# zhipeng-wei/Image-to-Video-I2V-attack

Hardware: AMD Instinct MI355X
Metric: adversarial frames/sec (10-step I2V, ResNet-50 layer3, 32x224^2 clips) (higher is better)
Workload: dtype f32

## Files before the change

### __graft_entry__.py

```python
import os
import subprocess
import sys

ROOT = os.path.dirname(os.path.abspath(__file__))
PKG_ROOT = os.path.join(ROOT, "image-to-video-i2v-attack_amd")
CSRC = os.path.join(PKG_ROOT, "csrc")
LIB = os.path.join(PKG_ROOT, "i2v_amd", "libi2v_hip.so")
for p in (PKG_ROOT, ROOT):
    if p not in sys.path:
        sys.path.insert(0, p)


def _stale(target, sources):
    return not os.path.exists(target) or any(os.path.getmtime(s) > os.path.getmtime(target) for s in sources)


ENGINE_UNITS = ["i2v_engine.cpp", "i2v_pack.cpp", "i2v_plan.cpp", "i2v_tune.cpp", "i2v_run.cpp", "i2v_loop_api.cpp"]
UNITS = ["i2v_kernels.hip", "i2v_conv_cfg0.hip", "i2v_conv_cfg1.hip", "i2v_conv_cfg2.hip", "i2v_conv_cfg3.hip", "i2v_conv_cfg4.hip",
         "i2v_conv_cfg5.hip", "i2v_conv_stems.hip", "i2v_fastblock.hip", "i2v_gconv.hip", "i2v_dwconv.hip", "i2v_se.hip", "i2v_loader.hip", "i2v_vit.hip", "i2v_vit.cpp", "i2v_swin.hip", "i2v_swin.cpp",
         "i2v_convnext.hip", "i2v_convnext.cpp", "i2v_mixer.hip", "i2v_mixer.cpp",
         ] + ENGINE_UNITS
HEADERS = ["i2v_kernels.h", "i2v_params.h", "i2v_be.h", "i2v_conv_tile.h", "i2v_conv_launch.h", "i2v_vit_kernels.h", "i2v_swin_kernels.h", "i2v_xf.h",
           "i2v_net.h", "i2v_se_host.h", "i2v_convnext_host.h", "i2v_xf_host.h", "i2v_hip_stub.h",
           "i2v_mixer_host.h", "i2v_gelu.h"]
FLAGS = ["--offload-arch=gfx950", "-O3", "-ffp-contract=off", "-std=c++20", "-fPIC", "-DI2V_SEPARATE_UNITS",
         "-DI2V_HAVE_GCONV", "-DI2V_HAVE_DWCONV",
         "-DI2V_HAVE_SE",
         "-DI2V_HAVE_CONVNEXT",
         "-DI2V_HAVE_MIXER"]


def build_lib(experimental: bool = False) -> str:
    from concurrent.futures import ThreadPoolExecutor
    hipcc = os.environ.get("HIPCC", "/opt/rocm/bin/hipcc")
    lib = LIB.replace(".so", "_exp.so") if experimental else LIB
    objdir = os.path.join(CSRC, "build", "exp" if experimental else "default")
    os.makedirs(objdir, exist_ok=True)
    units = UNITS + (["i2v_conv_exp.hip"] if experimental else [])
    hdrs = [os.path.join(CSRC, f) for f in HEADERS] + [os.path.join(ROOT, "include", h) for h in ("i2v_hip.h", "i2v_loader.h", "i2v_vit.h", "i2v_swin.h", "i2v_convnext.h", "i2v_mixer.h")]
    defs = ["-DI2V_EXPERIMENTAL"] if experimental else []
    if not _stale(lib, [os.path.join(CSRC, u) for u in units] + hdrs):
        return lib
    jobs = []
    for u in units:
        src, obj = os.path.join(CSRC, u), os.path.join(objdir, u + ".o")
        if _stale(obj, [src] + hdrs):
            jobs.append([hipcc] + FLAGS + defs + ["-c", "-x", "hip", src, "-o", obj])

    def run(cmd):
        print(" ".join(cmd), flush=True)
        subprocess.run(cmd, check=True)
    if jobs:
        with ThreadPoolExecutor(max_workers=min(len(jobs), max(1, (os.cpu_count() or 2)))) as ex:
            list(ex.map(run, jobs))
    objs = [os.path.join(objdir, u + ".o") for u in units]
    if jobs or _stale(lib, objs):
        run([hipcc, "--offload-arch=gfx950", "-shared", "-fPIC", "-o", lib] + objs)
    return lib


def build() -> None:
    build_lib(experimental=False)
    deps = [os.path.join(CSRC, f) for f in ENGINE_UNITS + ["i2v_net.h", "i2v_kernels.h", "i2v_params.h", "i2v_se_host.h", "i2v_convnext_host.h", "i2v_convnext.cpp", "i2v_mixer_host.h", "i2v_mixer.cpp", "i2v_gelu.h", "i2v_xf.h", "i2v_xf_host.h", "i2v_hip_stub.h",
                                                               "i2v_vit_kernels.h", "i2v_swin_kernels.h"]] + [os.path.join(ROOT, "include", "i2v_hip.h")]
    hs = os.path.join(ROOT, "tests", "hostsim")
    if _stale(os.path.join(hs, "libi2v_hostsim.so"), deps + [os.path.join(hs, "hostsim_backend.cpp")]):
        subprocess.run([os.path.join(hs, "build.sh")], check=True)
    import ctypes
    import i2v_amd
    from i2v_amd import lib
    cd = ctypes.CDLL(LIB) if not _has_gpu() else lib.load()
    missing = [n for n in lib.EXPORTS + lib.LOADER_EXPORTS + lib.VIT_EXPORTS + lib.SWIN_EXPORTS + lib.CONVNEXT_EXPORTS + lib.MIXER_EXPORTS if not hasattr(cd, n)]
    if missing:
        raise RuntimeError(f"libi2v_hip.so lacks symbols: {missing}")


def _has_gpu() -> bool:
    try:
        import torch
        return torch.cuda.is_available()
    except Exception:
        return False


def smoke() -> None:
    import numpy as np
    import torch
    build()
    from i2v_amd import attacks, graphs, weights
    from oracle import restate
    gen = torch.Generator().manual_seed(1234)
    u8 = torch.randint(0, 256, (1, 3, 4, 64, 64), generator=gen, dtype=torch.uint8)
    mean = torch.tensor(restate.MEAN).view(1, 3, 1, 1, 1)
    std = torch.tensor(restate.STD).view(1, 3, 1, 1, 1)
    vid = (u8.float() / 255 - mean) / std
    atk = attacks.ImageGuidedFMDirection_Adam(["resnet"], depth=3, step_size=0.005, steps=3,
                                              graph_builder=graphs.build_tiny, weight_seed=0)
    adv = atk(vid, torch.zeros(1, dtype=torch.long), ["smoke"])
    torch.cuda.synchronize()
    g = graphs.build_tiny("resnet", (64, 64))
    net = restate.OracleNet(g, weights.synthetic_state_dict(g, 0), [g.hooks[3]])
    ref = restate.run_attack([net], vid, steps=3, step_size=0.005)
    np.testing.assert_allclose(atk.last_costs, ref["costs"], rtol=2e-4)
    diff = (adv.cpu() - ref["adv"]).abs()
    assert float(diff.mean()) < 5e-3, float(diff.mean())
    print("smoke ok: costs", atk.last_costs, "mean|adv-oracle|", float(diff.mean()))


if __name__ == "__main__":
    if "--experimental" in sys.argv[1:]:
        print(build_lib(experimental=True))
    else:
        build()
        if _has_gpu():
            smoke()
```

### image-to-video-i2v-attack_amd/csrc/i2v_be.h

```cpp
#pragma once
#include <hip/hip_runtime.h>
#include <math.h>
#include <stdint.h>
#include <stdio.h>
#include <stdlib.h>
#include <string.h>

#include <type_traits>
#include <utility>

#include "i2v_kernels.h"

typedef float f32x16 __attribute__((ext_vector_type(16)));
typedef float f32x4 __attribute__((ext_vector_type(4)));

extern thread_local char g_be_err[256];
extern thread_local bool g_be_has_err;
int hip_fail(hipError_t e, const char* what);
#define HIPCHK(x) do { hipError_t e_ = (x); if (e_ != hipSuccess) return hip_fail(e_, #x); } while (0)
#define LAUNCH_CHECK(name) do { hipError_t e_ = hipGetLastError(); if (e_ != hipSuccess) return hip_fail(e_, name); } while (0)
extern long long g_stat_conv, g_stat_pws, g_stat_bf3, g_stat_igh, g_stat_sth, g_stat_fastblock, g_stat_vfma, g_stat_igv, g_stat_gconv, g_stat_dwconv, g_stat_se, g_stat_cndw, g_stat_mixtok;

__device__ __forceinline__ unsigned fastdiv(unsigned n, unsigned m, unsigned s) {
    return (unsigned)(((unsigned long long)n * m) >> s);
}
static inline void fastdiv_magic(unsigned d, uint32_t* m, uint32_t* s) {
    unsigned l = 0; while ((1ull << l) < d) ++l;
    *s = 31 + l;
    *m = (uint32_t)(((1ull << (31 + l)) / d) + 1);
}
typedef int i2v_v4i __attribute__((ext_vector_type(4)));
__device__ __forceinline__ I2VKEntry load_kentry(const I2VKEntry* tab, int k) {
#if defined(__HIP_DEVICE_COMPILE__)
    const i2v_v4i v = ((const __attribute__((address_space(4))) i2v_v4i*)tab)[k];
    return I2VKEntry{v.x, v.y, v.z, v.w};
#else
    return tab[k];
#endif
}

static inline void conv_magics(I2VConvParams& p) {
    fastdiv_magic((unsigned)(p.Hg * p.Wg), &p.dv_hw_m, &p.dv_hw_s);
    fastdiv_magic((unsigned)p.Wg, &p.dv_w_m, &p.dv_w_s);
    fastdiv_magic((unsigned)(p.Tg > 0 ? p.Tg : 1), &p.dv_t_m, &p.dv_t_s);
    fastdiv_magic((unsigned)(p.Wo > 0 ? p.Wo : 1), &p.dv_wo_m, &p.dv_wo_s);
}

static inline bool conv_wants_prefetch(const I2VConvParams& p) {
    return p.vec_epilogue && !p.gate_scale && !p.pre_scale && p.add0_stride == 1 && (p.add0 || p.add1 || p.mask || p.gate) && p.Kpad <= 256 && (p.pointwise || p.tap_uniform) && p.Cd > 32;
}

static inline int conv_tail_px_tiles(const I2VConvParams& p) {
    if (p.quad || p.pre_scale || p.temporal || !(p.pointwise || p.tap_uniform) || p.Cd % 16 != 0 || p.blk > 1) return 0;
    const int64_t P = (int64_t)p.N * p.Hg * p.Wg;
    const int64_t n_px = (P + 63) / 64; const int n_cd = (p.Cd + 63) / 64;
    const int64_t tiles = n_px * n_cd;
    if (tiles < 2 * 256) return 0;
    const int r = (int)(tiles % 256);
    if (r == 0 || r > 104) return 0;
    return r / n_cd;
}

static inline bool conv_halo_ok(const I2VConvParams& p) {
    return p.halo == 9 && p.tap_uniform && !p.temporal && !p.pre_scale && !p.quad && p.blk <= 1 && p.sh == 1 && p.sw == 1 && p.Hs == p.Hg &&
           p.Ws == p.Wg && (p.Ws == 14 || p.Ws == 28 || p.Ws == 56) && p.Kpad == p.K && (p.Kpad / I2V_KC) % 9 == 0;
}

static inline bool conv_dc_ok(const I2VConvParams& p) {
    return (p.pointwise || p.tap_uniform) && !p.temporal && !p.pre_scale && !p.quad && p.Cd > 32 && (p.Kpad / I2V_KC) % 2 == 0 && p.Kpad >= 4 * I2V_KC;
}

static inline bool conv_bf3_ok(const I2VConvParams& p) {
#ifdef I2V_EXPERIMENTAL
    return p.bf3 && p.wp3 && (p.pointwise || p.tap_uniform) && (!p.temporal || p.tap_uniform) && !p.pre_scale && !p.quad && p.blk <= 1 && p.blkt <= 1 && p.Cd > 32;
#else
    (void)p; return false;
#endif
}

int launch_conv_cfg0(const I2VConvParams& p, hipStream_t s);
int launch_conv_cfg1(const I2VConvParams& p, hipStream_t s);
int launch_conv_cfg2(const I2VConvParams& p, hipStream_t s);
int launch_conv_cfg3(const I2VConvParams& p, hipStream_t s);
int launch_conv_cfg4(const I2VConvParams& p, hipStream_t s);
int launch_conv_cfg5(const I2VConvParams& p, hipStream_t s);
bool conv_ighalo_ok(const I2VConvParams& p);
int launch_conv_ighalo(const I2VConvParams& p, hipStream_t s);
bool conv_igvfma_ok(const I2VConvParams& p);
int launch_conv_igvfma(const I2VConvParams& p, hipStream_t s);
bool conv_stemhalo_ok(const I2VConvParams& p);
int launch_conv_stemhalo(const I2VConvParams& p, hipStream_t s);
bool conv_vfma_ok(const I2VConvParams& p);
int launch_conv_vfma(const I2VConvParams& p, hipStream_t s);
#ifdef I2V_EXPERIMENTAL
#ifndef I2V_BF3_VARIANT
#define I2V_BF3_VARIANT 1
#endif
#endif
#ifdef I2V_EXPERIMENTAL
bool conv_stem64_ok(const I2VConvParams& p);
int launch_conv_stem64(const I2VConvParams& p, hipStream_t s);
int conv_pws_grid(const I2VConvParams& p);
int launch_conv_pws(const I2VConvParams& p, hipStream_t s);
int launch_conv_bf3(const I2VConvParams& p, hipStream_t s);
// ... 2 lines not shown
```

### image-to-video-i2v-attack_amd/csrc/i2v_conv_tile.h

```cpp
#pragma once
#include "i2v_be.h"

#ifndef I2V_PROBE_T
struct I2VNoProbe {
    __device__ __forceinline__ void entry() {}
    __device__ __forceinline__ void loop_begin() {}
    __device__ __forceinline__ void loop_end(int ) {}
    __device__ __forceinline__ void exit(int ) {}
};
#define I2V_PROBE_T I2VNoProbe
#endif

#ifndef I2V_PRIO_LEVELS
#define I2V_PRIO_LEVELS 3
#endif
#ifndef I2V_DEEP
#define I2V_DEEP 1
#endif
#ifndef I2V_DEEP_STAGES
#define I2V_DEEP_STAGES 3
#endif
#ifndef I2V_BF3_STAGES
#define I2V_BF3_STAGES 2
#endif
// ... 42 lines not shown
    const bool nt_store = true;
#else
    const bool nt_store = p.cfg > 0 && ((p.cfg - 1) & 128);
#endif
    constexpr int C4 = BP / 4, RSTEP = 1024 / BP, NQ = WD * FR / RSTEP;
    const int c4 = t % C4, rbase = t / C4;
    const int64_t pp = px0 + (int64_t)c4 * 4;
    const bool pok = pp < P;
    const int64_t n = pok ? fastdiv((unsigned)pp, p.dv_hw_m, p.dv_hw_s) : 0;
    const int64_t poff = pp - n * HWg;
    #pragma unroll
    for (int q = 0; q < NQ; ++q) {
        const int row = rbase + q * RSTEP;
        const int cd = cd0 + (row / FR) * (BD / WD) + i * FR + (row % FR);
        const bool valid = pok && cd < p.Cd;
        float4 v = make_float4(0.f, 0.f, 0.f, 0.f);
        if (valid) {
        v = *reinterpret_cast<const float4*>(&Cs[row][c4 * 4]);
        const int64_t o = (int64_t)cd * HoWo + poff;
        if (p.gate_scale) {
            const float4 m = *reinterpret_cast<const float4*>(p.mask + n * p.mask_nstride + o);
            const float gs = p.gate_scale[cd], gt = p.gate_shift[cd];
            if (!(fmaf(m.x, gs, gt) > 0.f)) v.x = 0.f;
            if (!(fmaf(m.y, gs, gt) > 0.f)) v.y = 0.f;
            if (!(fmaf(m.z, gs, gt) > 0.f)) v.z = 0.f;
            if (!(fmaf(m.w, gs, gt) > 0.f)) v.w = 0.f;
        }
        if (p.shift) { const float sh = p.shift[cd]; v.x += sh; v.y += sh; v.z += sh; v.w += sh; }
        if (PREF) {
            v.x += pre0[q].x; v.y += pre0[q].y; v.z += pre0[q].z; v.w += pre0[q].w;
        } else {
            if (p.add0 && p.add0_stride == 1) {
                const float4 a = *reinterpret_cast<const float4*>(p.add0 + n * p.add0_nstride + o);
                v.x += a.x; v.y += a.y; v.z += a.z; v.w += a.w;
            } else if (p.add0) {
                const int oh = (int)fastdiv((unsigned)poff, p.dv_wo_m, p.dv_wo_s), ow = (int)(poff - (int64_t)oh * p.Wo);
                if (!(oh & 1) && (oh >> 1) < p.add0_H) {
                    const float2 a = *reinterpret_cast<const float2*>(
                        p.add0 + n * p.add0_nstride + (int64_t)cd * p.add0_H * p.add0_W + (oh >> 1) * p.add0_W + (ow >> 1));
                    v.x += a.x; v.z += a.y;
                }
            }
        }
        if (p.add1) {
            const float4 a = *reinterpret_cast<const float4*>(p.add1 + n * p.add1_nstride + o);
            v.x += a.x; v.y += a.y; v.z += a.z; v.w += a.w;
        }
        if (p.relu) { v.x = fmaxf(v.x, 0.f); v.y = fmaxf(v.y, 0.f); v.z = fmaxf(v.z, 0.f); v.w = fmaxf(v.w, 0.f); }
        if (p.gate) {
            const unsigned w = PREF ? pregw[q] : p.gate[(int64_t)cd * p.gate_stride + ((p.gate_pix0 + pp) >> 5)];
            const unsigned g = w >> ((unsigned)(p.gate_pix0 + pp) & 31u);
            if (!(g & 1u)) v.x = 0.f;
            if (!(g & 2u)) v.y = 0.f;
            if (!(g & 4u)) v.z = 0.f;
            if (!(g & 8u)) v.w = 0.f;
        } else if (p.mask && !p.gate_scale) {
            const float4 m = *reinterpret_cast<const float4*>(p.mask + n * p.mask_nstride + o);
            if (!(m.x > 0.f)) v.x = 0.f;
            if (!(m.y > 0.f)) v.y = 0.f;
            if (!(m.z > 0.f)) v.z = 0.f;
            if (!(m.w > 0.f)) v.w = 0.f;
        }
        if constexpr (!FUSE) {
            if (nt_store) { typedef float nt4 __attribute__((ext_vector_type(4))); const nt4 w4 = {v.x, v.y, v.z, v.w};
                            __builtin_nontemporal_store(w4, reinterpret_cast<nt4*>(p.dst + n * p.dst_nstride + o)); }
            else *reinterpret_cast<float4*>(p.dst + n * p.dst_nstride + o) = v;
        }
        }
        if constexpr (FUSE)
            *reinterpret_cast<float4*>(mid + (cd - cd0) * BP + c4 * 4) = v;
        if (p.gate_out) {
            unsigned nib = valid ? ((v.x > 0.f ? 1u : 0u) | (v.y > 0.f ? 2u : 0u) | (v.z > 0.f ? 4u : 0u) | (v.w > 0.f ? 8u : 0u)) : 0u;
            nib <<= 4 * (lane & 7);
            nib |= (unsigned)__builtin_amdgcn_update_dpp(0, (int)nib, 0xB1, 0xF, 0xF, true);
            nib |= (unsigned)__builtin_amdgcn_update_dpp(0, (int)nib, 0x4E, 0xF, 0xF, true);
            nib |= (unsigned)__builtin_amdgcn_update_dpp(0, (int)nib, 0x141, 0xF, 0xF, true);
            if (valid && (lane & 7) == 0)
                p.gate_out[(int64_t)cd * p.gate_out_stride + ((p.gate_out_pix0 + pp) >> 5)] = nib;
        }
    }
}

#define I2V_FROW(r) (MF16 ? 4 * lk + (r) : ((r) & 3) + 8 * ((r) >> 2) + 4 * lk)
template <int BD, int BP, int WD, int WP, bool PREF, bool MF16, bool FUSE, typename ACC, typename PT>
__device__ __forceinline__ void conv_vec_epilogue(const PT& p, ACC (&acc)[BD / WD / (MF16 ? 16 : 32)][BP / WP / (MF16 ? 16 : 32)], const int cd0,
                                                  const int64_t px0, float* const smem, const float4* const pre0, const unsigned* const pregw,
                                                  float* const mid) {
    constexpr int FR = MF16 ? 16 : 32, NR = MF16 ? 4 : 16, TD = BD / WD / FR, TP = BP / WP / FR;
    const int t = threadIdx.x, lane = t & 63, wave = t >> 6;
    const int wd = wave / WP, wpx = wave % WP;
    const int l31 = MF16 ? (lane & 15) : (lane & 31), lk = MF16 ? (lane >> 4) : (lane >> 5);
    float (*Cs)[BP] = reinterpret_cast<float (*)[BP]>(smem);
#pragma unroll
    for (int i = 0; i < TD; ++i) {
        __syncthreads();
#pragma unroll
        for (int j = 0; j < TP; ++j)
#pragma unroll
            for (int r = 0; r < NR; ++r)
                Cs[wd * FR + I2V_FROW(r)][wpx * (BP / WP) + j * FR + l31] = acc[i][j][r];
        __syncthreads();
        conv_vec_rows<BD, BP, WD, PREF, MF16, FUSE>(p, i, cd0, px0, Cs, t, pre0, pregw, mid);
    }
}
#undef I2V_FROW

template <int BD, int BP, int WD, int WP, int MODE, bool PREF, bool PRE = false, bool VID = false, bool MF16 = false, int HWM = 0, int CPB = 1, int FUSE = 0, int BF3 = 0>
__device__ __forceinline__ void conv_tile(const I2VConvParams& p, const int n_cd_tiles, const int bid, const int nwg, const int64_t px_base,
                                          float* const smem, I2V_PROBE_T& probe, const int probe_slot, const int prio_arg = I2V_PRIO_LEVELS,
                                          float* const mid = nullptr) {
#if defined(__HIP_DEVICE_COMPILE__)
    constexpr int KC = I2V_KC;
    constexpr int FR = MF16 ? 16 : 32;
    constexpr int NR = MF16 ? 4 : 16;
    constexpr int TD = BD / WD / FR, TP = BP / WP / FR;
    static_assert(!(MF16 && (PRE || PREF)), "no pre-activation / prefetch variants of the 16x16 tile");
    constexpr bool DEEP = conv_deep(MODE, PREF) || (BF3 == 1 && I2V_BF3_STAGES > 2) || BF3 == 3;
    constexpr int NST = BF3 == 3 ? 3 : BF3 == 1 ? I2V_BF3_STAGES : DEEP ? I2V_DEEP_STAGES : 2, AHEAD = NST - 1;
    constexpr bool HALO = MODE == 5;
    constexpr int HS = HALO ? BP + 2 * HWM + 2 : 1, HQ = (HS + 63) / 64;
    static_assert(!HALO || (HWM > 0 && BD == 64 && BP == 64 && !PREF && !PRE && !VID && !MF16), "halo staging: the plain 64x64 image tile only");
    static_assert(CPB == 1 || (!HALO && !DEEP && !PREF && !PRE && MODE != 4 && MODE != 0), "several chunks per barrier: the plain pointwise / tap-uniform loops only");
    constexpr int KB = CPB * KC;
    static_assert(!BF3 || (!MF16 && !PRE && !PREF && !HALO && (MODE == 1 || MODE == 2) && FUSE == 0 && BD % 32 == 0), "split-bf16 K loop: the plain pointwise / tap-uniform tiles");
    constexpr int AF = BF3 == 2 ? 0 : BF3 ? CPB * (((BD / 32) * 3 + 3) / 4 * 4) * 256 : KB * BD;
    float (*As)[KB][BD] = reinterpret_cast<float (*)[KB][BD]>(smem);
    float* const As3 = smem;
    float (*Bs)[KB][BP] = reinterpret_cast<float (*)[KB][BP]>(smem + NST * AF);

    const int t = threadIdx.x, lane = t & 63, wave = t >> 6;
    const int wd = wave / WP, wpx = wave % WP;

    const int q8 = nwg >> 3, r8 = nwg & 7, xcd = bid & 7;
    const int lid = (xcd < r8 ? xcd * (q8 + 1) : r8 * (q8 + 1) + (xcd - r8) * q8) + (bid >> 3);
    const int cd_tile = lid % n_cd_tiles;
    const int64_t px0 = px_base + (int64_t)(lid / n_cd_tiles) * BP;
    const int cd0 = cd_tile * BD;

    const int HWg = p.Hg * p.Wg;
    const int64_t P = (int64_t)p.N * HWg;

    constexpr bool PW = MODE == 1;
    constexpr bool QUAD = MODE == 4;
    typedef __attribute__((address_space(3))) void* lds_ptr_t;
    constexpr unsigned OOB = 0x80000000u;
    const int wv = __builtin_amdgcn_readfirstlane(wave);
    const __amdgpu_buffer_rsrc_t rs_w = BF3 ? __builtin_amdgcn_make_buffer_rsrc((void*)p.wp3, 0, (p.Kpad / KC) * (p.Cdpad / 32) * 3072, 0x00020000)
                                            : __builtin_amdgcn_make_buffer_rsrc((void*)p.wp, 0, p.Kpad * p.Cdpad * 4, 0x00020000);
    constexpr unsigned XB = QUAD ? 64u : 0u;
    const __amdgpu_buffer_rsrc_t rs_x = __builtin_amdgcn_make_buffer_rsrc((void*)((const char*)p.src - XB), 0, p.src_span_bytes + 2 * XB, 0x00020000);
    constexpr int NA = BF3 == 2 ? 0 : BF3 ? (BD / 32) * 3 : KC * BD / 256, NAQ = (NA + 3) / 4;
    constexpr int BPER = (PW || QUAD) ? 256 : 64;
    constexpr int NB = HALO ? 0 : KC * BP / BPER, NBQ = (NB + 3) / 4;
    const int bcol = PW ? (lane * 4) % BP : (BP >= 64 ? ((wave * 64) % BP) + lane : lane % BP);
    const int64_t ppix = px0 + bcol;
    const bool pvalid = ppix < P;
    const int64_t pn = pvalid ? fastdiv((unsigned)ppix, p.dv_hw_m, p.dv_hw_s) : 0;
    const int prem = (int)(ppix - pn * HWg);
    const int HWs = p.Hs * p.Ws;
    int h0 = 0, w0 = 0, t0 = 0;
    int64_t pns = pn;
    if (VID) {
        const int64_t clip = fastdiv((unsigned)pn, p.dv_t_m, p.dv_t_s);
        t0 = (int)(pn - clip * p.Tg) * p.st;
        pns = clip * p.Ts + t0;
    }
    const int nstr = (int)p.src_nstride;
    unsigned xoff;
    if (PW) xoff = (unsigned)((pns * p.src_nstride + prem) * 4);
    else {
        const int gi = (int)fastdiv((unsigned)prem, p.dv_w_m, p.dv_w_s), gj = prem - gi * p.Wg;
        h0 = gi * p.sh; w0 = gj * p.sw;
        xoff = (unsigned)((pns * p.src_nstride + (int64_t)h0 * p.Ws + w0) * 4) + XB;
    }
    if (!pvalid) xoff = OOB;
    unsigned aoff[NAQ ? NAQ : 1];
#pragma unroll
    for (int q = 0; q < NAQ; ++q) {
        const int f = (wave + 4 * q) * 256 + lane * 4;
        aoff[q] = BF3 ? (unsigned)(((cd0 / 32) * 3 + wave + 4 * q) * 1024 + lane * 16) : (unsigned)(((f / BD) * p.Cdpad + f % BD + cd0) * 4);
    }
    unsigned boff[PW ? NBQ : 1];
    if (PW) {
#pragma unroll
        for (int q = 0; q < NBQ; ++q) boff[q] = pvalid ? xoff + (unsigned)((((wave + 4 * q) * 256 + lane * 4) / BP) * HWs * 4) : OOB;
    }

#define I2V_ISSUE_PIECE(j_, k0_, buf_, vb_) I2V_ISSUE_PIECE_SUB(j_, k0_, buf_, vb_, 0)
#define I2V_ISSUE_PIECE_SUB(j_, k0_, buf_, vb_, sub_)                                                     \
    {                                                                                                     \
        constexpr int jj = (j_);                                                                          \
        const int k0 = (k0_);                                                                             \
        if constexpr (jj < NAQ) {                                                                         \
            const int ins = wv + 4 * jj;                                                                  \
            if constexpr (BF3) {    \
                __builtin_amdgcn_raw_ptr_buffer_load_lds(rs_w, (lds_ptr_t)(As3 + (buf_) * AF + (sub_) * (AF / CPB) + ins * 256), 16, ins < NA ? aoff[jj] : OOB, \
                                                         (k0 / KC) * (p.Cdpad / 32) * 3072, 0, 0);       \
            } else if (NA % 4 == 0 || ins < NA) {                                                         \
                if constexpr (false)                                                                      \
                    ;                                                                                     \
                else                                                                                      \
                    __builtin_amdgcn_raw_ptr_buffer_load_lds(rs_w, (lds_ptr_t)(&As[buf_][(sub_) * KC][0] + ins * 256), 16, aoff[jj],  \
                                                             k0 * p.Cdpad * 4, 0, 0);                     \
            }                                                                                             \
        } else {                                                                                          \
            constexpr int q = jj - NAQ;                                                                   \
            const int ins = wv + 4 * q;                                                                   \
            float* const bbuf = &Bs[buf_][(sub_) * KC][0];                                                \
            if (NB % 4 == 0 || ins < NB) {                                                                \
                if constexpr (PW) {                                                                       \
                    unsigned v = boff[q];                                                                 \
                    if (k0 + KC > p.K)             \
                        v = (k0 + ((wave + 4 * q) * 256 + lane * 4) / BP < p.K) ? v : OOB;                \
                    __builtin_amdgcn_raw_ptr_buffer_load_lds(rs_x, (lds_ptr_t)(bbuf + ins * 256), 16, v,         \
                                                             k0 * HWs * 4, 0, 0);                         \
                } else if constexpr (QUAD) {                                                              \
                     \
                    const I2VKEntry e = load_kentry(p.ktab, k0 + 4 * ((ins * 64) / BP));                  \
                    const int hs = h0 + e.dh, dtk = VID ? (e.valid >> 1) : 0;                             \
                    const bool ok = pvalid && (unsigned)hs < (unsigned)p.Hs && (!VID || (unsigned)(t0 + dtk) < (unsigned)p.Ts); \
                    const unsigned v = ok ? xoff + (unsigned)((e.chan_off + dtk * nstr + e.dh * p.Ws + e.dw) * 4) : OOB; \
                    __builtin_amdgcn_raw_ptr_buffer_load_lds(rs_x, (lds_ptr_t)(bbuf + ins * 256), 16, v, 0, 0, 0); \
                } else if constexpr (MODE == 2) {                                                         \
                    __builtin_amdgcn_raw_ptr_buffer_load_lds(rs_x, (lds_ptr_t)(bbuf + ins * 64), 4, vb_,         \
                                                             ((ins * 64) / BP) * HWs * 4, 0, 0);          \
                } else {                                                                                  \
                    const I2VKEntry e = load_kentry(p.ktab, k0 + (ins * 64) / BP);                        \
                    const int hs = h0 + e.dh, ws = w0 + e.dw, dtk = VID ? (e.valid >> 1) : 0;             \
                    const bool ok = pvalid && (e.valid & 1) && (unsigned)hs < (unsigned)p.Hs &&           \
                                    (unsigned)ws < (unsigned)p.Ws && (!VID || (unsigned)(t0 + dtk) < (unsigned)p.Ts); \
                    const unsigned v = ok ? xoff + (unsigned)((e.chan_off + dtk * nstr + e.dh * p.Ws + e.dw) * 4) : OOB; \
                    __builtin_amdgcn_raw_ptr_buffer_load_lds(rs_x, (lds_ptr_t)(bbuf + ins * 64), 4, v, 0, 0, 0); \
                }                                                                                         \
            }                                                                                             \
        }                                                                                                 \
    }
#define I2V_CHUNK_VB(e_)                                                                                  \
    ([&]() -> unsigned {                                                                                  \
        const int hs = h0 + (e_).dh, ws = w0 + (e_).dw, dtk = VID ? ((e_).valid >> 1) : 0;                \
        const bool ok = pvalid && (unsigned)hs < (unsigned)p.Hs && (unsigned)ws < (unsigned)p.Ws &&       \
                        (!VID || (unsigned)(t0 + dtk) < (unsigned)p.Ts);                                  \
        return ok ? xoff + (unsigned)(((e_).chan_off + dtk * nstr + (e_).dh * p.Ws + (e_).dw) * 4) : OOB; \
    }())

    constexpr int E_C4 = BP / 4, E_RSTEP = 1024 / BP, E_NQ = WD * FR / E_RSTEP;
    static_assert(!PREF || TD == 1, "PREF needs a single epilogue pass");
    float4 pre0[PREF ? E_NQ : 1];
    unsigned pregw[PREF ? E_NQ : 1];
    if (PREF) {
        const int e_c4 = t % E_C4, e_rbase = t / E_C4;
        const int64_t e_pp = px0 + (int64_t)e_c4 * 4;
        const bool e_ok = e_pp < P;
        const int64_t e_n = e_ok ? fastdiv((unsigned)e_pp, p.dv_hw_m, p.dv_hw_s) : 0;
        const int64_t e_poff = e_pp - e_n * HWg;
        const int e_HoWo = p.Ho * p.Wo;
#pragma unroll
        for (int q = 0; q < E_NQ; ++q) {
            const int row = e_rbase + q * E_RSTEP;
            const int cd = cd0 + (row >> 5) * (BD / WD) + (row & 31);
            const bool ok = e_ok && cd < p.Cd;
            const int64_t o = (int64_t)cd * e_HoWo + e_poff;
            pre0[q] = (ok && p.add0) ? *reinterpret_cast<const float4*>(p.add0 + e_n * p.add0_nstride + o) : make_float4(0.f, 0.f, 0.f, 0.f);
            pregw[q] = (ok && p.gate) ? p.gate[(int64_t)cd * p.gate_stride + ((p.gate_pix0 + e_pp) >> 5)] : 0xffffffffu;
        }
    }

    probe.loop_begin();
    typedef short bf8 __attribute__((ext_vector_type(8)));
    typedef float f4 __attribute__((ext_vector_type(4)));
    constexpr int TD_ = BD / WD / (MF16 ? 16 : 32);
    bf8 wcur[BF3 == 2 ? CPB : 1][BF3 == 2 ? TD_ : 1][3];
    const char* const w3lane = BF3 ? (const char*)p.wp3 + (size_t)lane * 16 + (size_t)(cd0 / 32 + (wave / WP) * TD_) * 3072 : nullptr;
    const size_t w3chunk = BF3 ? (size_t)(p.Cdpad / 32) * 3072 : 0;
    auto load_w3 = [&](const int chunk, const int i, const int pl) {
        return __builtin_bit_cast(bf8, *reinterpret_cast<const f4*>(w3lane + (size_t)chunk * w3chunk + (i * 3 + pl) * 1024));
    };
    if constexpr (BF3 == 2) {
#pragma unroll
        for (int sb = 0; sb < CPB; ++sb)
#pragma unroll
            for (int i = 0; i < TD_; ++i)
#pragma unroll
                for (int pl = 0; pl < 3; ++pl) wcur[sb][i][pl] = load_w3(sb, i, pl);
    }
    (void)wcur; (void)w3lane; (void)w3chunk;
    constexpr int TP_ = BP / WP / (MF16 ? 16 : 32);
    bf8 xcur[BF3 == 3 ? TP_ : 1][3];
    (void)xcur;
    auto bf3_split2 = [](const float lo, const float hi, unsigned& p1, unsigned& p2, unsigned& p3) {
        typedef __bf16 bf2 __attribute__((ext_vector_type(2)));
        typedef float f2 __attribute__((ext_vector_type(2)));
        const unsigned a = __builtin_bit_cast(unsigned, __builtin_convertvector((f2){lo, hi}, bf2));
        const float rl = lo - __builtin_bit_cast(float, a << 16), rh = hi - __builtin_bit_cast(float, a & 0xffff0000u);
        const unsigned b = __builtin_bit_cast(unsigned, __builtin_convertvector((f2){rl, rh}, bf2));
        const float sl = rl - __builtin_bit_cast(float, b << 16), sh = rh - __builtin_bit_cast(float, b & 0xffff0000u);
        const unsigned c = __builtin_bit_cast(unsigned, __builtin_convertvector((f2){sl, sh}, bf2));
        p1 = a; p2 = b; p3 = c;
    };
    auto bf3_split_frag = [&](const float (&x)[8], bf8 (&out)[3]) {
        typedef unsigned u4 __attribute__((ext_vector_type(4)));
        unsigned q1[4], q2[4], q3[4];
#pragma unroll
        for (int e = 0; e < 4; ++e) bf3_split2(x[2 * e], x[2 * e + 1], q1[e], q2[e], q3[e]);
        out[0] = __builtin_bit_cast(bf8, (u4){q1[0], q1[1], q1[2], q1[3]});
        out[1] = __builtin_bit_cast(bf8, (u4){q2[0], q2[1], q2[2], q2[3]});
        out[2] = __builtin_bit_cast(bf8, (u4){q3[0], q3[1], q3[2], q3[3]});
    };
    (void)bf3_split_frag;
    typedef typename std::conditional<MF16, f32x4, f32x16>::type acc_t;
    acc_t acc[TD][TP];
#pragma unroll
    for (int a = 0; a < TD; ++a)
#pragma unroll
        for (int b = 0; b < TP; ++b)
#pragma unroll
            for (int r = 0; r < NR; ++r) acc[a][b][r] = 0.f;

    const int nchunks = p.Kpad / KC;
    const int l31 = MF16 ? (lane & 15) : (lane & 31), lk = MF16 ? (lane >> 4) : (lane >> 5);
#define I2V_FROW(r) (MF16 ? 4 * lk + (r) : ((r) & 3) + 8 * ((r) >> 2) + 4 * lk)
    constexpr int NL = NAQ + NBQ;
    constexpr int KR = MF16 ? 4 : 2;
    constexpr int KS = KC / KR;
    constexpr int PPS = (NL + KS - 1) / KS;
    I2VKEntry e_next[CPB];
#pragma unroll
    for (int h = 0; h < CPB; ++h) e_next[h] = I2VKEntry{0, 0, 0, 0};
    const int nsuper = nchunks / CPB;
    bool qok[QUAD ? TP : 1][2][MF16 ? 1 : 2];
    if constexpr (QUAD) {
#pragma unroll
        for (int j = 0; j < TP; ++j) {
            const int64_t fp = px0 + wpx * (BP / WP) + j * FR + l31;
            const unsigned fr = fp < P ? (unsigned)fp - fastdiv((unsigned)fp, p.dv_hw_m, p.dv_hw_s) * (unsigned)HWg : 0u;
            const int fj = (int)(fr - fastdiv(fr, p.dv_w_m, p.dv_w_s) * (unsigned)p.Wg);
#pragma unroll
            for (int qi = 0; qi < 2; ++qi)
#pragma unroll
                for (int hf = 0; hf < (MF16 ? 1 : 2); ++hf) {
                    const int el = MF16 ? lk : 2 * hf + lk;
                    qok[j][qi][hf] = 4 * qi + el < p.quad_kw && (unsigned)(fj * p.sw + p.quad_dw0 + 4 * qi + el) < (unsigned)p.Ws;
                }
        }
    }
    if constexpr (HALO) {
        constexpr int NT = 9, HPW = 4 * HQ, PPC = (HPW + NT - 1) / NT;
        float* const Hb = smem + NST * KC * BD;
        const int W_ = HWM;
        int tsh[NT], tdh[NT], tdw[NT];
#pragma unroll
        for (int t = 0; t < NT; ++t) {
            const I2VKEntry e = load_kentry(p.ktab, t * KC);
            tdh[t] = e.dh; tdw[t] = e.dw; tsh[t] = e.dh * W_ + e.dw + W_ + 1;
        }
        const int chan0 = load_kentry(p.ktab, 0).chan_off;
        const int ngroups = nchunks / NT;
        const int gstride = ngroups > 1 ? load_kentry(p.ktab, NT * KC).chan_off - chan0 : 0;
        const int64_t fp = px0 + wpx * (BP / WP) + l31;
        const bool fpv = fp < P;
        const unsigned fr = fpv ? (unsigned)fp - fastdiv((unsigned)fp, p.dv_hw_m, p.dv_hw_s) * (unsigned)HWg : 0u;
        const int fh = (int)fastdiv(fr, p.dv_w_m, p.dv_w_s), fw = (int)fr - fh * p.Wg;
        unsigned tmask = 0;
#pragma unroll
        for (int t = 0; t < NT; ++t)
            tmask |= (fpv && (unsigned)(fh + tdh[t]) < (unsigned)p.Hs && (unsigned)(fw + tdw[t]) < (unsigned)p.Ws) ? (1u << t) : 0u;
        const int lbase = lk * HS + wpx * (BP / WP) + l31;
        unsigned hoff[HQ];
#pragma unroll
        for (int q = 0; q < HQ; ++q) {
            const int64_t vp = px0 - (W_ + 1) + 64 * q + lane;
            const bool ok = vp >= 0 && vp < P;
            const int64_t vn = ok ? fastdiv((unsigned)vp, p.dv_hw_m, p.dv_hw_s) : 0;
            hoff[q] = ok ? (unsigned)((vn * p.src_nstride + (vp - vn * HWg)) * 4) : OOB;
        }
        auto halo_piece = [&]<int IDX>(std::integral_constant<int, IDX>, const int gb, const int chan_off) {
            constexpr int chl = IDX / HQ, q = IDX % HQ;
            float* const dst = Hb + ((gb * KC + wv * 4 + chl) * HS + 64 * q);
            const int so = (chan_off + (wv * 4 + chl) * HWs) * 4;
            if constexpr (chl == 3 && q == HQ - 1) {
                if (lane < HS - 64 * q) __builtin_amdgcn_raw_ptr_buffer_load_lds(rs_x, (lds_ptr_t)dst, 4, hoff[q], so, 0, 0);
            } else
                __builtin_amdgcn_raw_ptr_buffer_load_lds(rs_x, (lds_ptr_t)dst, 4, hoff[q], so, 0, 0);
        };
        if (ngroups > 0) {
            [&]<int... I>(std::integer_sequence<int, I...>) { ((halo_piece(std::integral_constant<int, I>{}, 0, chan0)), ...); }
            (std::make_integer_sequence<int, HPW>{});
            I2V_ISSUE_PIECE(0, 0, 0, OOB);
        }
        int gbuf = 0;
        for (int g = 0; g < ngroups; ++g) {
            const bool more_g = g + 1 < ngroups;
            const int chan_next = chan0 + (g + 1) * gstride;
            [&]<int... T>(std::integer_sequence<int, T...>) {
                (([&] {
                    constexpr int t = T;
                    const int abuf = (g + t) & 1;
                    asm volatile("s_waitcnt vmcnt(0)" ::: "memory");
                    asm volatile("s_waitcnt lgkmcnt(0)" ::: "memory");
                    __builtin_amdgcn_s_barrier();
                    const int hidx = lbase + gbuf * KC * HS + tsh[t];
                    const bool ok = (tmask >> t) & 1u;
                    float fa[2], fb[2];
                    auto rd = [&](const int s_, const int set) {
// ... 192 lines not shown
#pragma unroll
                    for (int i = 0; i < TD; ++i)
#pragma unroll
                        for (int pl = 0; pl < 3; ++pl) wcur[sb][i][pl] = wnxt[sb][i][pl];
            }
            return;
        }
        float fa[2][TD], fb[2][TP];
        auto read_frags = [&](const int s, const int set) {
#pragma unroll
            for (int i = 0; i < TD; ++i) fa[set][i] = As[buf][KR * s + lk][wd * (BD / WD) + i * FR + l31];
            if constexpr (QUAD) {
                const float* const bq = &Bs[buf][0][0];
#pragma unroll
                for (int j = 0; j < TP; ++j) {
                    const int px = wpx * (BP / WP) + j * FR + l31;
                    const int qd = MF16 ? s : (s >> 1), el = MF16 ? lk : 2 * (s & 1) + lk;
                    const float v = bq[(qd * BP + px) * 4 + el];
                    const bool m = ((qd & 1) && p.quad == 2) ? qok[j][1][MF16 ? 0 : (s & 1)] : qok[j][0][MF16 ? 0 : (s & 1)];
                    fb[set][j] = m ? v : 0.f;
                }
            } else {
#pragma unroll
                for (int j = 0; j < TP; ++j) fb[set][j] = Bs[buf][KR * s + lk][wpx * (BP / WP) + j * FR + l31];
            }
        };
        read_frags(0, 0);
        [&]<int... S>(std::integer_sequence<int, S...>) {
            (([&] {
                constexpr int s = S, set = S & 1;
                if constexpr (s + 1 < CPB * KS) read_frags(s + 1, set ^ 1);
                __builtin_amdgcn_sched_barrier(0);
                if constexpr (PRE) {
                    typedef const __attribute__((address_space(4))) float* cfp;
                    const int kr = c * KB + 2 * s;
                    const float sc = lk ? ((cfp)p.pre_scale)[kr + 1] : ((cfp)p.pre_scale)[kr];
                    const float sh = lk ? ((cfp)p.pre_shift)[kr + 1] : ((cfp)p.pre_shift)[kr];
#pragma unroll
                    for (int j = 0; j < TP; ++j) fb[set][j] = fmaxf(fmaf(fb[set][j], sc, sh), 0.f);
                }
#pragma unroll
                for (int i = 0; i < TD; ++i)
#pragma unroll
                    for (int j = 0; j < TP; ++j) {
                        if constexpr (MF16) acc[i][j] = __builtin_amdgcn_mfma_f32_16x16x4f32(fa[set][i], fb[set][j], acc[i][j], 0, 0, 0);
                        else acc[i][j] = __builtin_amdgcn_mfma_f32_32x32x2f32(fa[set][i], fb[set][j], acc[i][j], 0, 0, 0);
                    }
                if constexpr (MORE) {
                    [&]<int... Q>(std::integer_sequence<int, Q...>) {
                        (([&] {
                            constexpr int jp = s * PPS + Q;
                            if constexpr (jp < CPB * NL) {
                                constexpr int sub = jp / NL;
                                I2V_ISSUE_PIECE_SUB(jp % NL, ((c + AHEAD) * CPB + sub) * KC, DEEP ? (buf + AHEAD) % NST : (buf ^ 1), vb[sub], sub);
                            }
                        }()), ...);
                    }(std::make_integer_sequence<int, PPS>{});
                }
            }()), ...);
        }(std::make_integer_sequence<int, CPB * KS>{});
    };
    if constexpr (BF3 == 3) {
        asm volatile("s_waitcnt vmcnt(0)" ::: "memory");
        __builtin_amdgcn_s_barrier();
        const int l31_ = lane & 31, lk_ = lane >> 5;
#pragma unroll
        for (int j = 0; j < TP_; ++j) {
            float x[8];
#pragma unroll
            for (int e = 0; e < 8; ++e) x[e] = Bs[0][8 * lk_ + e][(wave % WP) * (BP / WP) + j * 32 + l31_];
            bf3_split_frag(x, xcur[j]);
        }
    }
    if constexpr (!HALO) {
        int c = 0, buf = 0;
        for (; c + AHEAD < nsuper; ++c) { chunk_body(c, buf, std::true_type{}); buf = buf + 1 == NST ? 0 : buf + 1; }
        for (; c < nsuper; ++c) { chunk_body(c, buf, std::false_type{}); buf = buf + 1 == NST ? 0 : buf + 1; }
    }
#undef I2V_ISSUE_PIECE
#undef I2V_ISSUE_PIECE_SUB
#undef I2V_CHUNK_VB
    if (prio_hi > 0) __builtin_amdgcn_s_setprio(0);
    probe.loop_end(probe_slot);

    const int HoWo = p.Ho * p.Wo;
    if (p.vec_epilogue) {
        conv_vec_epilogue<BD, BP, WD, WP, PREF, MF16, FUSE != 0>(p, acc, cd0, px0, smem, pre0, pregw, mid);
        return;
    }
    if (p.blk > 1 || (VID && p.blkt > 1)) {
        const int bb = p.blk * p.blk, Creal = p.Cd / ((VID ? p.blkt : 1) * bb);
#pragma unroll
        for (int j = 0; j < TP; ++j) {
            const int64_t pp = px0 + wpx * (BP / WP) + j * FR + l31;
            if (pp >= P) continue;
            const int64_t ng = fastdiv((unsigned)pp, p.dv_hw_m, p.dv_hw_s);
            const int rem = (int)(pp - ng * HWg);
            const int gi = (int)fastdiv((unsigned)rem, p.dv_w_m, p.dv_w_s), gj = rem - gi * p.Wg;
            const int64_t clip = VID ? fastdiv((unsigned)ng, p.dv_t_m, p.dv_t_s) : ng;
            const int otb = VID ? (int)(ng - clip * p.Tg) * p.ost + p.ot0 : 0;
#pragma unroll
            for (int i = 0; i < TD; ++i)
#pragma unroll
                for (int r = 0; r < NR; ++r) {
                    const int cd = cd0 + wd * (BD / WD) + i * FR + I2V_FROW(r);
                    if (cd >= p.Cd) continue;
                    const int cls3 = cd / Creal, c = cd - cls3 * Creal;
                    const int ct = VID ? cls3 / bb : 0, cls = cls3 - ct * bb;
                    const int oh = gi * p.osh + cls / p.blk + p.oh0, ow = gj * p.osw + cls % p.blk + p.ow0;
                    if (oh >= p.Ho || ow >= p.Wo || (VID && otb + ct * p.oct >= p.To)) continue;
                    const int64_t n = VID ? clip * p.To + otb + ct * p.oct : ng;
                    const int64_t o = (int64_t)c * HoWo + oh * p.Wo + ow;
                    float v = acc[i][j][r];
                    if (p.shift) v += p.shift[c];
                    if (p.add1) v += p.add1[n * p.add1_nstride + o];
                    if (p.relu) v = fmaxf(v, 0.f);
                    if (p.mask && !(p.mask[n * p.mask_nstride + o] > 0.f)) v = 0.f;
                    p.dst[n * p.dst_nstride + o] = v;
                }
        }
        return;
    }
#pragma unroll
    for (int j = 0; j < TP; ++j) {
        const int64_t pp = px0 + wpx * (BP / WP) + j * FR + l31;
        const bool pin = pp < P;
        const int64_t ng = pin ? fastdiv((unsigned)pp, p.dv_hw_m, p.dv_hw_s) : 0;
        const int rem = (int)(pin ? pp - ng * HWg : 0);
        const int gi = (int)fastdiv((unsigned)rem, p.dv_w_m, p.dv_w_s), gj = rem - gi * p.Wg;
        const int oh = gi * p.osh + p.oh0, ow = gj * p.osw + p.ow0;
        bool ok = pin && oh < p.Ho && ow < p.Wo;
        int64_t n = ng;
        if (VID) {
            const int64_t clip = fastdiv((unsigned)ng, p.dv_t_m, p.dv_t_s);
            const int ot = (int)(ng - clip * p.Tg) * p.ost + p.ot0;
            if (ot >= p.To) ok = false;
            n = clip * p.To + ot;
        }
        const int opix = oh * p.Wo + ow;
        float* dstn = p.dst + n * p.dst_nstride + opix;
        const float* a0 = nullptr; int a0_plane = HoWo;
        if (p.add0 && ok) {
            if (p.add0_stride == 1) a0 = p.add0 + n * p.add0_nstride + opix;
            else {
                const int s = p.add0_stride, qh = oh / s, qw = ow / s;
                if (qh * s == oh && qw * s == ow && qh < p.add0_H && qw < p.add0_W) {
                    a0 = p.add0 + n * p.add0_nstride + qh * p.add0_W + qw;
                    a0_plane = p.add0_H * p.add0_W;
                }
            }
        }
        const float* a1 = p.add1 ? p.add1 + n * p.add1_nstride + opix : nullptr;
        const float* mk = p.mask ? p.mask + n * p.mask_nstride + opix : nullptr;
        const int64_t gidx = (int64_t)p.gate_pix0 + n * HoWo + opix;
#pragma unroll
        for (int i = 0; i < TD; ++i) {
#pragma unroll
            for (int r = 0; r < NR; ++r) {
                const int cd = cd0 + wd * (BD / WD) + i * FR + I2V_FROW(r);
                const bool okc = ok && cd < p.Cd;
                float v = 0.f;
                if (okc) {
                    v = acc[i][j][r];
                    if (p.gate_scale && !(fmaf(mk[(int64_t)cd * HoWo], p.gate_scale[cd], p.gate_shift[cd]) > 0.f)) v = 0.f;
                    if (p.shift) v += p.shift[cd];
                    if (a0) v += a0[(int64_t)cd * a0_plane];
                    if (a1) v += a1[(int64_t)cd * HoWo];
// ... 72 lines not shown
```

### image-to-video-i2v-attack_amd/csrc/i2v_engine.cpp

```cpp
#include "i2v_net.h"

#include <math.h>
#include <stdarg.h>
#include <stdio.h>
#include <stdlib.h>
#include <string.h>

using namespace eng;

#define I2V_MAX_NETS 4096
thread_local std::string eng::g_err;

int eng::fail(const char* fmt, ...) {
    char buf[512];
    va_list ap;
    va_start(ap, fmt);
    vsnprintf(buf, sizeof buf, fmt, ap);
    va_end(ap);
    g_err = buf;
    return 1;
}

int i2v_api_fail(const char* msg) { return fail("%s", msg); }

// ... 331 lines not shown
            if (pack_gconv(n, nd)) return 1;
            continue;
        }
        if (nd.groups > 1 || nd.dw) expand_grouped(nd);
        if (pack_fwd(n, nd)) return 1;
        if (nd.preact()) {
            std::vector<float> ps(nd.fwd.Kpad > nd.fwd.Cdpad ? nd.fwd.Kpad : nd.fwd.Cdpad, 0.f), pt(ps.size(), 0.f);
            for (int c = 0; c < nd.cd.cin; ++c) { ps[c] = nd.pre_scale[c]; pt[c] = nd.pre_shift[c]; }
            if (upload(n, ps, &nd.pre_scale_d) || upload(n, pt, &nd.pre_shift_d)) return 1;
        }
        if (nd.cd.src == n.input) { if (pack_img(n, nd)) return 1; }
        else if (pack_bwd(n, nd)) return 1;
        if (nd.groups > 1 || nd.dw) std::vector<float>().swap(nd.w);
    }
    size_t off = 64;
    for (const Node& nd : n.nodes) if (nd.type == 0 && nd.cd.src == n.input && nd.fwd.quad) n.stage_input = true;
    if (n.stage_input) {
        const Buffer& ib = n.bufs[n.tens[n.input].buf];
        n.in_stage_off = off; off = align_up(off + N * ib.C * ib.H * ib.W, 64) + 64;
    }
    for (Buffer& b : n.bufs) {
        if (b.is_input) continue;
        size_t sz = N / Tin * b.T * b.C * b.H * b.W;
        b.act_off = off; off = align_up(off + sz, 64);
        b.grad_off = off; off = align_up(off + sz, 64);
    }
    const char* gates_env = getenv("I2V_GATES");
    const bool use_gates = !(gates_env && gates_env[0] == '0');
    for (const Node& nd : n.nodes)
        if (use_gates && nd.type == 0 && nd.cd.relu && !nd.fwd.tpair) n.bufs[n.tens[nd.cd.dst].buf].gated = true;
    for (const Node& nd : n.nodes)
        if (use_gates && nd.type == 4 && nd.sd.relu) n.bufs[n.tens[nd.sd.dst].buf].gated = true;
    for (Buffer& b : n.bufs) {
        if (!b.gated) continue;
        const size_t pix = N / Tin * b.T * b.H * b.W;
        if (pix + 64 >= (1ull << 31)) return fail("gate rows of more than 2^31 bits are not supported");
        b.gate_words = (int)((pix + 31) / 32 + 2);
        b.gate_off = off; off = align_up(off + (size_t)b.C * b.gate_words, 64);
    }
    for (Node& nd : n.nodes)
        if (nd.type == 1) {
            const Buffer& db = n.bufs[n.tens[nd.pd.dst].buf];
            nd.idx_off = off; off = align_up(off + (N / Tin * db.T * n.tens[nd.pd.dst].C * db.H * db.W + 3) / 4, 64);
        }
    for (Node& nd : n.nodes)
        if (nd.type == 3) {
            const Buffer& tb = n.bufs[n.tens[nd.ad.theta].buf]; const Buffer& pb = n.bufs[n.tens[nd.ad.phi].buf];
            nd.p_off = off; off = align_up(off + N / Tin * ((size_t)tb.T * tb.H * tb.W) * ((size_t)pb.T * pb.H * pb.W), 64);
        }
    for (Node& nd : n.nodes)
        if (nd.type == 4) {
            const size_t C = (size_t)nd.sd.C, rd = (size_t)nd.sd.rd;
            nd.se_off = off; nd.se_floats = 4 * align_up(N * C, 64) + align_up(N * rd, 64);
            off += nd.se_floats;
        }
    std::string err;
    size_t end = 0;
    if (!plan_pass(n, true, off, N, &end, &err)) return fail("plan: %s", err.c_str());
    n.arena_floats = end + 64;
    n.arena = (float*)be_malloc(n.arena_floats * sizeof(float));
    if (!n.arena) return fail("arena allocation of %zu bytes failed", n.arena_floats * sizeof(float));
    CHECK_BE(be_memset0(n.arena, n.arena_floats * sizeof(float), nullptr));
    if (!plan_pass(n, false, off, N, &end, &err)) return fail("plan: %s", err.c_str());
    mark_fusable(n);
    if (autotune(n)) return 1;
    mark_overlap(n);
    CHECK_BE(be_stream_sync(nullptr));
    n.planned = true;
    return 0;
}

extern "C" int i2v_net_fusion_info(i2v_handle h, int net, int32_t out[4]) {
    Net* n = get_net(h, net); if (!n) return 1;
    if (!n->planned || !out) return fail("i2v_net_fusion_info: net not planned");
    out[0] = out[1] = out[2] = out[3] = 0;
    int k = 0;
    for (const std::vector<Launch>* L : {&n->fwd, &n->bwd}) {
        for (const Launch& l : *L) { out[k] += l.fuse_ok ? 1 : 0; out[2 + k] += (l.fuse_ok && l.fuse_b[0]) ? 1 : 0; }
        ++k;
    }
    return 0;
}

extern "C" size_t i2v_net_workspace_bytes(i2v_handle h, int net) {
    Net* n = get_net(h, net); if (!n) return 0;
    return n->arena_floats * sizeof(float) + n->weight_bytes;
}

#ifndef I2V_SEPARATE_UNITS
#include "i2v_pack.cpp"
#include "i2v_plan.cpp"
#include "i2v_tune.cpp"
#include "i2v_run.cpp"
#include "i2v_loop_api.cpp"
#define fail xf_fail
#include "i2v_convnext.cpp"
#include "i2v_mixer.cpp"
#undef fail
#endif
```

### image-to-video-i2v-attack_amd/csrc/i2v_kernels.h

```cpp
#pragma once
#include <initializer_list>
#include "i2v_params.h"

typedef void* i2v_stream_t;

const char* be_name();
long long be_stat(const char* name);
int  be_set_device(int device);
void* be_malloc(size_t bytes);
void be_free(void* p);
int  be_h2d(void* dst, const void* src, size_t bytes);
int  be_d2d_2d(void* dst, size_t dpitch, const void* src, size_t spitch, size_t width, size_t rows,
               i2v_stream_t s);
int  be_memset0(void* p, size_t bytes, i2v_stream_t s);
const char* be_error();
int  i2v_api_fail(const char* msg);
void* be_event_create();
void be_event_destroy(void* ev);
int  be_event_record(void* ev, i2v_stream_t s);
int  be_event_elapsed_ms(void* start, void* stop, float* ms);
int  be_stream_sync(i2v_stream_t s);
i2v_stream_t be_stream_create();
void be_stream_destroy(i2v_stream_t s);
int  be_stream_wait_event(i2v_stream_t s, void* ev);
int  be_device_sync();

int k_conv(const I2VConvParams& p, i2v_stream_t s);
int k_conv_fusable(const I2VConvParams& a, const I2VConvParams& b);
inline bool i2v_conv_pair_fusable(const I2VConvParams& a, const I2VConvParams& b) {
    if (a.pointwise || !a.tap_uniform || a.temporal || a.quad || a.pre_scale || a.gate_scale || a.blk > 1 || a.blkt > 1) return false;
    for (const I2VConvParams* q : {&a, &b})
        if (!(q->Tg == q->Ts && q->Ts == q->To && q->st == 1 && q->ost == 1 && q->ot0 == 0 && q->blkt <= 1)) return false;
    if (a.sh != 1 || a.sw != 1 || a.Hs != a.Hg || a.Ws != a.Wg || a.Hg != a.Ho || a.Wg != a.Wo || a.osh != 1 || a.osw != 1 || a.oh0 || a.ow0) return false;
    if ((a.Cd != 64 && a.Cd != 128) || a.Kpad != a.K || a.add0_stride > 1) return false;
    if (!b.pointwise || b.temporal || b.quad || b.pre_scale || b.gate_scale || b.blk > 1 || b.blkt > 1 || b.add0_stride > 1) return false;
    if (b.K != a.Cd || b.Kpad != b.K || b.Cs != a.Cd || b.src != a.dst || b.src_nstride != a.dst_nstride) return false;
    if (b.Hs != a.Ho || b.Ws != a.Wo || b.Hg != a.Hg || b.Wg != a.Wg || b.Ho != a.Ho || b.Wo != a.Wo || b.sh != 1 || b.sw != 1 || b.osh != 1 || b.osw != 1 ||
        b.oh0 || b.ow0 || b.Cd < 64 || b.Tg != a.Tg) return false;
    return true;
}
int k_conv_fused(const I2VConvParams& a, const I2VConvParams& b, int halo, i2v_stream_t s);
int k_conv_candidates(const I2VConvParams& p, int* out);
inline int i2v_fastblock_rows(const I2VConvParams& a, const I2VConvParams& b, const I2VConvParams* c, const I2VConvParams* d) {
    auto plain = [](const I2VConvParams& q) {
        return !q.pre_scale && !q.gate_scale && q.blk <= 1 && q.blkt <= 1 && q.sh == 1 && q.sw == 1 && q.osh == 1 && q.osw == 1 && q.oh0 == 0 &&
               q.ow0 == 0 && q.Hs == q.Hg && q.Hg == q.Ho && q.Ws == q.Wg && q.Wg == q.Wo && q.Tg == q.Ts && q.Ts == q.To && q.st == 1 && q.ost == 1 && q.ot0 == 0 &&
               !q.add1 && !q.mask && q.Kpad % 8 == 0 && q.Kpad <= 512 && q.gate_pix0 == 0 && q.gate_out_pix0 == 0;
    };
    if (!plain(a) || !plain(b) || a.quad || a.add0 || b.add0) return 0;
    const int CM = a.Cd;
    if ((CM != 4 && CM != 8) || b.Cd != CM || b.Cs != CM || b.src != a.dst || b.src_nstride != a.dst_nstride) return 0;
    if (b.Hg != a.Hg || b.Wg != a.Wg || b.Tg != a.Tg || b.N != a.N) return 0;
    const int H = a.Hg, W = a.Wg;
    if ((H * W) % 32 != 0 || (int64_t)a.N * a.src_nstride * 4 >= (1ll << 31)) return 0;
    if (c) {
        if (!plain(*c) || c->quad || !a.relu || !b.relu || a.gate || b.gate || c->gate || !c->relu || !a.shift || !b.shift || !c->shift || !a.gate_out || !b.gate_out || !c->gate_out) return 0;
        if (c->src != b.dst || c->src_nstride != b.dst_nstride || c->Cs != CM || c->K != CM || c->Cd != 4 * CM || c->Hg != H || c->Wg != W || c->Tg != a.Tg || c->N != a.N) return 0;
        if (!c->add0 || c->add0_stride != 1) return 0;
        if (d) {
            if (!plain(*d) || d->quad || d->relu || d->add0 || d->gate || d->gate_out || !d->shift || d->src != a.src || d->src_nstride != a.src_nstride || d->Cs != a.Cs ||
                d->K != a.Cs || d->K != CM || d->Cd != c->Cd || d->Hg != H || d->Wg != W || d->Tg != a.Tg || d->N != a.N || c->add0 != d->dst || c->add0_nstride != d->dst_nstride) return 0;
        }
    } else {
        if (d || a.relu || b.relu || a.gate_out || b.gate_out || a.shift || b.shift || !a.gate || !b.gate || a.K != a.Cs || a.K > 64) return 0;
    }
    int g = W, r32 = 32; while (r32) { const int t = g % r32; g = r32; r32 = t; }
    const int Rq = 32 / g;
    if (H % Rq != 0) return 0;
    int R = Rq;
    while (R * W < 192 && R * 2 <= H && H % (R * 2) == 0) R *= 2;
    if ((size_t)CM * (R + 2) * (W + 2) * 4 > 60 * 1024) return 0;
    return R;
}
int k_fastblock(const I2VConvParams& a, const I2VConvParams& b, const I2VConvParams* c, const I2VConvParams* d, i2v_stream_t s);
int k_gconv_plan(I2VGConvParams* p);
int k_gconv(const I2VGConvParams& p, i2v_stream_t s);
int k_dwconv_plan(I2VDwConvParams* p);
int k_dwconv(const I2VDwConvParams& p, i2v_stream_t s);
int k_se_plan(I2VSeParams* p);
int k_se_squeeze(const I2VSeParams& p, i2v_stream_t s);
int k_se_excite(const I2VSeParams& p, i2v_stream_t s);
int k_se_scale(const I2VSeParams& p, i2v_stream_t s);
int k_convnext_dw_plan(I2VCnDwParams* p);
int k_convnext_dw(const I2VCnDwParams& p, i2v_stream_t s);
int k_mixer_tokens_plan(I2VMixTokParams* p);
int k_mixer_tokens(const I2VMixTokParams& p, i2v_stream_t s);
int k_pool_fwd(const I2VPoolParams& p, i2v_stream_t s);
int k_pool_bwd(const I2VPoolParams& p, i2v_stream_t s);
int k_pool3d_fwd(const I2VPoolParams& p, i2v_stream_t s);
int k_pool3d_bwd(const I2VPoolParams& p, i2v_stream_t s);
int k_avgpool_fwd(const I2VPoolParams& p, i2v_stream_t s);
int k_avgpool_bwd(const I2VPoolParams& p, i2v_stream_t s);
int k_addmask(const I2VAddMaskParams& p, i2v_stream_t s);
int k_cos(const I2VCosParams& p, i2v_stream_t s);
int k_std_reduce(const I2VStdParams& p, i2v_stream_t s);
int k_std_grad(const I2VStdParams& p, i2v_stream_t s);
int k_ilaf_reduce(const I2VIlafParams& p, i2v_stream_t s);
int k_ilaf_grad(const I2VIlafParams& p, i2v_stream_t s);
int k_head_ce(const I2VHeadParams& p, i2v_stream_t s);
int k_clip_from_u8(const uint8_t* frames, float* video, int b, int t, int h, int w, i2v_stream_t s);
int k_clip_resize_crop(const uint8_t* frames, float* video, const int32_t* xtab, const int32_t* ytab, int b, int t, int H, int W,
                       int cy, int cx, int oh, int ow, i2v_stream_t s);
int k_frames_from_video(const float* video, float* x, float* u, int b, int f, int h, int w, i2v_stream_t s);
int k_compose(const float* u, const float* delta, float* x, int b, int f, int h, int w, float eps,
              int video_layout, i2v_stream_t s);
int k_adam(float* delta, float* m, float* v, const float* gx, const float* u, int64_t n, int hw,
           float eps, float step_size, float bc2_sqrt, float w1, float beta2, float w2, float adam_eps,
           i2v_stream_t s);
int k_sign_bim(float* adv, const float* u, const float* grad, int64_t n, int64_t chan_stride,
               float step, float eps, i2v_stream_t s);
int k_sign_delta(float* delta, const float* grad, int64_t n, float step, i2v_stream_t s);
int k_sign_delta_gx(float* delta, const float* gx, const float* u, int64_t n, float eps, float step,
                    i2v_stream_t s);
int k_clip_resample_crop(const uint8_t* frames, float* video, const int32_t* xb, const int32_t* xk, int kx, const int32_t* yb, const int32_t* yk,
                         int ky, int b, int t, int H, int W, int cy, int cx, int oh, int ow, i2v_stream_t s);
int k_tt_grad_mix(const float* grads, float* out, const float* kern , const int* moves , int D, int64_t NC, int T,
                  int HW, float w1, float w, i2v_stream_t s);
int k_attn_gemm(const I2VAttnGemm& p, i2v_stream_t s);
int k_softmax_rows(const I2VSoftmaxRows& p, i2v_stream_t s);
int k_resample_nearest(const float* src, float* dst, int64_t planes, int Hs, int Ws, int Hd, int Wd, const int32_t* map_y,
                       const int32_t* map_x, i2v_stream_t s);
int k_resample_nearest_bwd(const float* g, float* gsrc, int64_t planes, int Hd, int Wd, int Hs, int Ws, const int32_t* ylo,
                           const int32_t* yhi, const int32_t* xlo, const int32_t* xhi, i2v_stream_t s);
int k_grad_post_groups(int b, int c, int f, int h, int w, int mode, int64_t* group_elems);
// ... 12 lines not shown
```

### image-to-video-i2v-attack_amd/csrc/i2v_kernels.hip

```cpp
#include "i2v_be.h"

thread_local char g_be_err[256];
thread_local bool g_be_has_err = false;

int hip_fail(hipError_t e, const char* what) {
    snprintf(g_be_err, sizeof g_be_err, "%s: %s", what, hipGetErrorString(e));
    g_be_has_err = true;
    return 1;
}

const char* be_name() { return "hip:gfx950"; }
long long g_stat_conv = 0, g_stat_pws = 0, g_stat_bf3 = 0, g_stat_igh = 0, g_stat_sth = 0;
long long be_stat(const char* name) {
    if (!strcmp(name, "conv_launches")) return __atomic_load_n(&g_stat_conv, __ATOMIC_RELAXED);
    if (!strcmp(name, "pws_launches")) return __atomic_load_n(&g_stat_pws, __ATOMIC_RELAXED);
    if (!strcmp(name, "bf3_launches")) return __atomic_load_n(&g_stat_bf3, __ATOMIC_RELAXED);
    if (!strcmp(name, "ighalo_launches")) return __atomic_load_n(&g_stat_igh, __ATOMIC_RELAXED);
    if (!strcmp(name, "stemhalo_launches")) return __atomic_load_n(&g_stat_sth, __ATOMIC_RELAXED);
    if (!strcmp(name, "fastblock_launches")) return __atomic_load_n(&g_stat_fastblock, __ATOMIC_RELAXED);
    if (!strcmp(name, "vfma_launches")) return __atomic_load_n(&g_stat_vfma, __ATOMIC_RELAXED);
    if (!strcmp(name, "igvfma_launches")) return __atomic_load_n(&g_stat_igv, __ATOMIC_RELAXED);
    if (!strcmp(name, "gconv_launches")) return __atomic_load_n(&g_stat_gconv, __ATOMIC_RELAXED);
    if (!strcmp(name, "dwconv_launches")) return __atomic_load_n(&g_stat_dwconv, __ATOMIC_RELAXED);
    if (!strcmp(name, "se_launches")) return __atomic_load_n(&g_stat_se, __ATOMIC_RELAXED);
    if (!strcmp(name, "convnext_dw_launches")) return __atomic_load_n(&g_stat_cndw, __ATOMIC_RELAXED);
    if (!strcmp(name, "mixer_tokens_launches")) return __atomic_load_n(&g_stat_mixtok, __ATOMIC_RELAXED);
#ifdef I2V_EXPERIMENTAL
    if (!strcmp(name, "experimental")) return 1;
#else
    if (!strcmp(name, "experimental")) return 0;
#endif
    return -1;
}
const char* be_error() { return g_be_has_err ? g_be_err : nullptr; }
int be_set_device(int device) { HIPCHK(hipSetDevice(device)); return 0; }
void* be_malloc(size_t bytes) { void* p = nullptr; if (hipMalloc(&p, bytes) != hipSuccess) return nullptr; return p; }
void be_free(void* p) { (void)hipFree(p); }
int be_h2d(void* dst, const void* src, size_t bytes) { HIPCHK(hipMemcpy(dst, src, bytes, hipMemcpyHostToDevice)); return 0; }
int be_d2d_2d(void* dst, size_t dpitch, const void* src, size_t spitch, size_t width, size_t rows, i2v_stream_t s) {
    HIPCHK(hipMemcpy2DAsync(dst, dpitch, src, spitch, width, rows, hipMemcpyDeviceToDevice, (hipStream_t)s));
    return 0;
}
int be_memset0(void* p, size_t bytes, i2v_stream_t s) { HIPCHK(hipMemsetAsync(p, 0, bytes, (hipStream_t)s)); return 0; }

void* be_event_create() { hipEvent_t e = nullptr; if (hipEventCreate(&e) != hipSuccess) return nullptr; return (void*)e; }
void be_event_destroy(void* ev) { (void)hipEventDestroy((hipEvent_t)ev); }
int be_event_record(void* ev, i2v_stream_t s) { HIPCHK(hipEventRecord((hipEvent_t)ev, (hipStream_t)s)); return 0; }
int be_event_elapsed_ms(void* a, void* b, float* ms) { HIPCHK(hipEventElapsedTime(ms, (hipEvent_t)a, (hipEvent_t)b)); return 0; }
int be_stream_sync(i2v_stream_t s) { HIPCHK(hipStreamSynchronize((hipStream_t)s)); return 0; }
int be_device_sync() { HIPCHK(hipDeviceSynchronize()); return 0; }
i2v_stream_t be_stream_create() { hipStream_t s = nullptr; if (hipStreamCreateWithFlags(&s, hipStreamNonBlocking) != hipSuccess) return nullptr; return (i2v_stream_t)s; }
void be_stream_destroy(i2v_stream_t s) { if (s) (void)hipStreamDestroy((hipStream_t)s); }
int be_stream_wait_event(i2v_stream_t s, void* ev) { HIPCHK(hipStreamWaitEvent((hipStream_t)s, (hipEvent_t)ev, 0)); return 0; }

__constant__ float c_mean[3] = {0.485f, 0.456f, 0.406f};
__constant__ float c_std[3] = {0.229f, 0.224f, 0.225f};

static int conv_pick(const I2VConvParams& p) {
    const char* force = getenv("I2V_FORCE_CFG");
    if (force && *force) { const int f = atoi(force); return (p.pre_scale && f != 0 && f != 3) ? 3 : f; }
    if (p.Cd <= 16 && !p.pre_scale) return 5;
    if (conv_bf3_ok(p)) return p.Cd > 64 ? 2 : 3;
    if (conv_wants_prefetch(p)) return 3;
    if (p.pre_scale) {
        const double blocks128 = ceil(p.Cd / 128.0) * ceil((double)p.N * p.Hg * p.Wg / 128.0);
        return (p.Cd > 64 && blocks128 >= 256.0 * 6) ? 0 : 3;
    }
    static const struct { int BD, BP, occ; double ineff; } C[5] = {
        {128, 128, 3, 1.00}, {64, 128, 5, 1.05}, {128, 64, 5, 1.04}, {64, 64, 7, 1.10}, {32, 256, 4, 1.08}};
    const double P = (double)p.N * p.Hg * p.Wg;
    const int nchunks = p.Kpad / I2V_KC;
    int best = 0; double best_t = 1e300;
    for (int i = 0; i < 5; ++i) {
        if (C[i].BD > 32 && p.Cd <= C[i].BD / 2) continue;
        if (C[i].BD == 32 && p.Cd > 32) continue;
        const double blocks = ceil(p.Cd / (double)C[i].BD) * ceil(P / C[i].BP);
        const double rounds = ceil(blocks / 256.0);
        const double fill = blocks / (256.0 * C[i].occ);
        const double mfma = (double)nchunks * (C[i].BD / 32) * (C[i].BP / 32) / 4 * 8 * 64 * C[i].ineff *
                            (1.0 + 0.15 * (fill < 1.0 ? 1.0 - fill : 0.0));
        const double overhead = 1500.0 + (C[i].BD * C[i].BP / 256) * 10.0;
        const double t = rounds * mfma + ceil(rounds / C[i].occ) * overhead;
        if (t < best_t) { best_t = t; best = i; }
    }
    return best;
}

int k_conv_candidates(const I2VConvParams& p, int* out) {
    int n = 0;
    if (p.pre_scale) { if (p.Cd > 64) out[n++] = 0; out[n++] = 3; return n; }
#ifdef I2V_EXPERIMENTAL
    if (conv_bf3_ok(p)) {
        static const int BD3[4] = {128, 64, 128, 64};
        for (int i = 0; i < 4; ++i) {
            if (p.Cd <= BD3[i] / 2) continue;
            out[n++] = i;
            if (I2V_BF3_VARIANT == 2 && (p.Kpad / I2V_KC) % 2 == 0) out[n++] = i | 64;
            if (I2V_BF3_VARIANT == 1 && i == 0 && !p.temporal) out[n++] = 0 | 64;
        }
        return n;
    }
#endif
    static const int BD[5] = {128, 64, 128, 64, 32};
    for (int i = 0; i < 5; ++i) {
        if (BD[i] > 32 && p.Cd <= BD[i] / 2) continue;
        if (BD[i] == 32 && p.Cd > 32) continue;
        out[n++] = i;
    }
    if (conv_wants_prefetch(p)) out[n++] = 3 | 8;
// ... 1306 lines not shown
```

### image-to-video-i2v-attack_amd/csrc/i2v_net.h

```cpp
#pragma once
#include "../../include/i2v_hip.h"
#include "i2v_kernels.h"

#include <stdint.h>

#include <deque>
#include <mutex>
#include <string>
#include <vector>

namespace eng {

#pragma GCC visibility push(hidden)
extern thread_local std::string g_err;
int fail(const char* fmt, ...);
#pragma GCC visibility pop

#define CHECK_BE(expr)                                                            \
    do {                                                                          \
        if ((expr) != 0) return fail("%s: %s", #expr, be_error() ? be_error() : "backend error"); \
    } while (0)

struct Buffer { int C, H, W; int T = 1; size_t act_off = 0, grad_off = 0; bool is_input = false;
                size_t gate_off = 0; int gate_words = 0; bool gated = false; };
struct Tensor { int buf, c_off, C; bool post_relu; float bwd_gain = 1.f; };

struct Packed {
    float* wp = nullptr; I2VKEntry* ktab = nullptr;
    float* wpc = nullptr;
    uint16_t* wp3 = nullptr;
    int K = 0, Kpad = 0, Cd = 0, Cdpad = 0, tap_uniform = 0;
    int halo = 0;
    int ph = 0, pw = 0, Hg = 0, Wg = 0;
    int pt = 0, Tg = 1;
    int has_dt = 0;
    int quad = 0, quad_kw = 0, quad_dw0 = 0;
    int tpair = 0;
    int ig_tt = 0, ig_th = 0, ig_tw = 0;
    int ig_p77 = 0;
};

struct Node {
    int type;
    i2v_se_desc sd{};
    std::vector<float> se_w1, se_b1, se_w2t, se_b2;
    float* se_w1_d = nullptr; float* se_b1_d = nullptr; float* se_w2t_d = nullptr; float* se_b2_d = nullptr;
    size_t se_off = 0, se_floats = 0;
    i2v_attn_desc ad{};
    size_t p_off = 0;
    int src0() const { return type == 0 ? cd.src : type == 3 ? ad.theta : type == 4 ? sd.src : pd.src; }
    int dst0() const { return type == 0 ? cd.dst : type == 3 ? ad.dst : type == 4 ? sd.dst : pd.dst; }
    int residual0() const { return type == 0 ? cd.residual : type == 4 ? sd.residual : -1; }
    i2v_conv3d_desc cd; i2v_pool3d_desc pd;
    std::vector<float> w;
    std::vector<float> shift;
    std::vector<float> pre_scale, pre_shift;
    float* shift_d = nullptr; float* pre_scale_d = nullptr; float* pre_shift_d = nullptr;
    bool preact() const { return !pre_scale.empty(); }
    Packed fwd; std::vector<Packed> bwd;
    int groups = 1; std::vector<float> wg; bool gconv = false;
    float* gw_fwd = nullptr; float* gw_bwd = nullptr; int gw_tapmask[4] = {0, 0, 0, 0};
    int dw = 0; bool dwconv = false;
    struct ImgGrad {
        Packed P; int blk = 0, sh = 1, blkt = 1;
        int ost = 1, ot0 = 0;
        int st = 1, oct = 1; bool skips = false;
        double flop_share = 1.0;
    };
    std::vector<ImgGrad> imgs;
    size_t idx_off = 0;
};

enum Kind { L_CONV, L_IMGGRAD, L_POOLF, L_POOLB, L_ADDMASK, L_AVGF, L_AVGB, L_MEMSET, L_POOL3F, L_POOL3B, L_AGEMM, L_SOFTMAX, L_GCONV, L_DWCONV,
            L_SE_SQUEEZE, L_SE_EXCITE, L_SE_SCALE };
struct Launch {
    Kind kind;
    I2VConvParams conv; I2VPoolParams pool; I2VAddMaskParams am; I2VGConvParams gc; I2VDwConvParams dc; I2VSeParams se;
    I2VAttnGemm ag; I2VSoftmaxRows sm; int sm_rows_per_clip = 0;
    int T = 1;
    bool src_is_input = false;
    bool img_accumulate = false;
    float* ms_ptr = nullptr; size_t ms_floats_per_frame = 0;
    float* se_vec = nullptr; size_t se_vec_floats = 0;
    double se_bytes_per_frame = 0;
    bool ms_gx = false;
    double alg_flops_per_frame = 0;
    int cfg_b[4] = {0, 0, 0, 0};
    int fuse_ok = 0;
    int fuse_b[4] = {0, 0, 0, 0};
    int node = -1;
    int fb_ok = 0;
    int fb_b[4] = {0, 0, 0, 0};
    int ov_after = -2, ov_join = -1;
};
inline int cfg_bucket(int clips, int max_clips) {
    int b = 0;
    while (b < 3 && (max_clips >> (b + 1)) >= clips && (max_clips >> (b + 1)) >= 1) ++b;
    return b;
}

struct Addend { const float* p; int64_t nstride; int stride, H, W; };

struct Net {
    std::vector<Buffer> bufs; std::vector<Tensor> tens; std::vector<Node> nodes;
    int input = -1; std::vector<int> hooks; int maxN = 0; bool planned = false;
    float* arena = nullptr; size_t arena_floats = 0; std::vector<void*> dev_allocs;
    std::vector<Launch> fwd, bwd;
    int frames = 0;
    int Tin() const { return bufs[tens[input].buf].T; }
    size_t weight_bytes = 0;
    std::vector<float*> hook_tmp;
    size_t in_stage_off = 0; bool stage_input = false;
    i2v_stream_t side = nullptr; std::vector<void*> ov_ev; size_t ov_used = 0;
    std::vector<std::vector<int>> ov_at[2]; int ov_max_frames = 0;
};

struct TimedLaunch { void* start; void* stop; int kind; double flops; int Cd, K, HWg, frames, pw; void* chain_from; double bytes; int count = 1; };

}

struct i2v_ctx {
    int device; std::vector<eng::Net*> nets; std::mutex nets_mu;
    int timing = 0;
    std::deque<eng::TimedLaunch> timed; size_t timed_used = 0; std::mutex timing_mu;
};

namespace eng {
#pragma GCC visibility push(hidden)

inline size_t align_up(size_t v, size_t a) { return (v + a - 1) / a * a; }

inline Net* get_net(i2v_handle h, int id) {
    if (!h || id < 0 || id >= (int)h->nets.size() || !h->nets[id]) { fail("bad net id %d", id); return nullptr; }
    return h->nets[id];
}

template <typename T>
int upload(Net& n, const std::vector<T>& host, T** dev) {
    size_t bytes = host.size() * sizeof(T);
    void* d = be_malloc(bytes ? bytes : 16);
    if (!d) return fail("device allocation of %zu bytes failed", bytes);
    n.dev_allocs.push_back(d);
    n.weight_bytes += bytes;
    if (bytes) CHECK_BE(be_h2d(d, host.data(), bytes));
    *dev = (T*)d;
    return 0;
}

bool math_bf16x3();
int pack_fwd(Net& n, Node& nd);
int pack_bwd(Net& n, Node& nd);
int pack_img(Net& n, Node& nd);
bool gconv_enabled();
int pack_gconv(Net& n, Node& nd);
bool dwconv_enabled();
int pack_dwconv(Net& n, Node& nd);

struct View { float* p; int64_t nstride; int C, H, W; int T = 1; };
View view_of(Net& n, int t, bool grad);
bool plan_pass(Net& n, bool dry, size_t off, size_t N, size_t* end, std::string* err);

void mark_fusable(Net& n);
void mark_overlap(Net& n);
int autotune(Net& n);

I2VConvParams conv_prep(const Launch& l, const float* x, float* gx, int accumulate);
int conv_run(const Launch& l, int frames, const float* x, float* gx, int accumulate, i2v_stream_t s);
bool fused_fits(const Launch& a, const Launch& b, int frames);
int fused_run(const Launch& a, const Launch& b, int frames, const float* x, int halo, i2v_stream_t s);
int fast_run(const std::vector<Launch>& L, size_t li, int frames, const float* x, i2v_stream_t s);
extern long long g_overlap_launches;

#pragma GCC visibility pop
}
```

### image-to-video-i2v-attack_amd/csrc/i2v_run.cpp

```cpp
#include "i2v_net.h"
#ifndef I2V_HAVE_SE
#include "i2v_se_host.h"
#endif

#include <stdio.h>
#include <stdlib.h>

#include <algorithm>

using namespace eng;

namespace eng {

I2VConvParams conv_prep(const Launch& l, const float* x, float* gx, int accumulate) {
    I2VConvParams p = l.conv;
    if (l.src_is_input) p.src = x;
    if (l.kind == L_IMGGRAD) { p.dst = gx; if (accumulate || l.img_accumulate) { p.add1 = gx; p.add1_nstride = p.dst_nstride; } }
    p.vec_epilogue = (p.blk <= 1 && p.osh == 1 && p.osw == 1 && p.oh0 == 0 && p.ow0 == 0 && p.Hg == p.Ho &&
                      p.Wg == p.Wo && p.Tg == p.To && p.ost == 1 && p.ot0 == 0 &&
                      (p.Ho * p.Wo) % 4 == 0 && p.dst_nstride % 4 == 0 &&
                      (p.add0_stride == 1 || (p.add0_stride == 2 && p.Wo % 4 == 0 && p.add0_W * 2 == p.Wo &&
                                              p.add0_W % 2 == 0 && (p.add0_H * p.add0_W) % 2 == 0)) &&
                      p.add0_nstride % 4 == 0 && p.add1_nstride % 4 == 0 && p.mask_nstride % 4 == 0 &&
                      (((uintptr_t)p.dst | (uintptr_t)p.add0 | (uintptr_t)p.add1 | (uintptr_t)p.mask) & 15) == 0)
                         ? 1 : 0;
    if (!(p.Tg == p.Ts && p.Ts == p.To && p.st == 1 && p.ost == 1 && p.ot0 == 0 && p.blkt == 1)) p.temporal = 1;
    return p;
}

bool fused_fits(const Launch& a, const Launch& b, int frames) {
    for (const Launch* l : {&a, &b}) {
        const I2VConvParams& p = l->conv;
        const int64_t span = ((int64_t)frames * p.Ts / p.Tg - 1) * p.src_nstride * 4 + (int64_t)p.Cs * p.Hs * p.Ws * 4;
        if (span >= (1ll << 31)) return false;
    }
    return true;
}
int fused_run(const Launch& a, const Launch& b, int frames, const float* x, int halo, i2v_stream_t s) {
    I2VConvParams pa = conv_prep(a, x, nullptr, 0), pb = conv_prep(b, x, nullptr, 0);
    for (I2VConvParams* p : {&pa, &pb}) {
        p->N = frames;
        p->src_span_bytes = (int32_t)(((int64_t)frames * p->Ts / p->Tg - 1) * p->src_nstride * 4 + (int64_t)p->Cs * p->Hs * p->Ws * 4);
    }
    CHECK_BE(k_conv_fused(pa, pb, halo, s));
    return 0;
}

int fast_run(const std::vector<Launch>& L, size_t li, int frames, const float* x, i2v_stream_t s) {
    const int g = L[li].fb_ok;
    I2VConvParams q[4];
    for (int j = 0; j < g; ++j) { q[j] = conv_prep(L[li + j], x, nullptr, 0); q[j].N = frames; }
    const I2VConvParams* c = g == 3 ? &q[2] : g == 4 ? &q[3] : nullptr;
    const I2VConvParams* d = g == 4 ? &q[2] : nullptr;
    if (i2v_fastblock_rows(q[0], q[1], c, d) <= 0) return 2;
    if (k_fastblock(q[0], q[1], c, d, s)) { fail("k_fastblock: %s", be_error() ? be_error() : "backend error"); return 1; }
    return 0;
}

int conv_run(const Launch& l, int frames, const float* x, float* gx, int accumulate, i2v_stream_t s) {
    I2VConvParams p = conv_prep(l, x, gx, accumulate);
    const int clips = frames / p.Tg;
    const int64_t plane_bytes = (int64_t)p.Cs * p.Hs * p.Ws * 4, stride_bytes = p.src_nstride * 4;
    const int64_t clip_bytes = (int64_t)(p.Ts - 1) * stride_bytes + plane_bytes;
    int64_t per = clip_bytes >= (1ll << 31) ? 0 : 1 + ((1ll << 31) - 1 - clip_bytes) / (stride_bytes * p.Ts);
    if (per < 1) return fail("one clip of a convolution input exceeds 2 GiB");
    if (per < clips && (p.gate || p.gate_out)) {
        per -= per % 32;
        if (per < 1) return fail("a sliced convolution launch cannot keep its gate rows word-aligned");
    }
    for (int c0 = 0; c0 < clips; c0 += (int)per) {
        I2VConvParams q = p;
        const int nc = clips - c0 < per ? clips - c0 : (int)per;
        q.N = nc * p.Tg;
        q.src += (int64_t)c0 * p.Ts * p.src_nstride; q.dst += (int64_t)c0 * p.To * p.dst_nstride;
        if (q.add0) q.add0 += (int64_t)c0 * p.To * p.add0_nstride;
        if (q.add1) q.add1 += (int64_t)c0 * p.To * p.add1_nstride;
        if (q.mask) q.mask += (int64_t)c0 * p.To * p.mask_nstride;
        q.gate_pix0 = p.gate_pix0 + (int32_t)((int64_t)c0 * p.To * p.Ho * p.Wo);
        q.gate_out_pix0 = p.gate_out_pix0 + (int32_t)((int64_t)c0 * p.To * p.Ho * p.Wo);
        q.src_span_bytes = (int32_t)((int64_t)(nc * p.Ts - 1) * stride_bytes + plane_bytes);
        CHECK_BE(k_conv(q, s));
    }
    return 0;
}

}

long long eng::g_overlap_launches = 0;

static TimedLaunch* timing_begin(i2v_ctx* h, int kind, double flops, i2v_stream_t s, TimedLaunch* prev) {
    if (!h->timing) return nullptr;
    TimedLaunch* t;
    {
        std::lock_guard<std::mutex> lock(h->timing_mu);
        if (h->timed_used == h->timed.size()) {
            TimedLaunch fresh{be_event_create(), be_event_create(), 0, 0.0, 0, 0, 0, 0, 0, nullptr, 0.0, 1};
            if (!fresh.start || !fresh.stop) return nullptr;
            h->timed.push_back(fresh);
        }
        t = &h->timed[h->timed_used++];
    }
    t->kind = kind; t->flops = flops; t->Cd = t->K = t->HWg = t->frames = t->pw = 0; t->bytes = 0.0; t->count = 1;
    t->chain_from = prev ? prev->stop : nullptr;
    if (!t->chain_from) be_event_record(t->start, s);
    return t;
}

static double launch_flops(const std::vector<Launch>& L, size_t li, int fb, int fuse, int frames, int clips) {
    const Launch& l = L[li];
    double flops = 0.0;
    if (fb) { for (int j = 0; j < fb; ++j) { const Launch& m = L[li + j]; flops += m.alg_flops_per_frame > 0 ? m.alg_flops_per_frame * frames : 2.0 * frames * m.conv.Hg * m.conv.Wg * (double)m.conv.Cd * m.conv.K; } }
    else if ((l.kind == L_CONV || l.kind == L_GCONV || l.kind == L_DWCONV) && l.alg_flops_per_frame > 0) flops = l.alg_flops_per_frame * frames;
    else if (l.kind == L_CONV) flops = 2.0 * frames * l.conv.Hg * l.conv.Wg * ((double)l.conv.Cd * l.conv.K + (fuse ? (double)L[li + 1].conv.Cd * L[li + 1].conv.K : 0.0));
    else if (l.kind == L_IMGGRAD) flops = l.alg_flops_per_frame * frames;
    else if (l.kind == L_AGEMM) flops = 2.0 * clips * (double)l.ag.Cc * l.ag.M * l.ag.N;
    else if (l.kind == L_SE_SQUEEZE || l.kind == L_SE_EXCITE || l.kind == L_SE_SCALE) flops = l.alg_flops_per_frame * frames;
    return flops;
}

static int launch_timing_kind(const Launch& l, bool backward_pass) {
    switch (l.kind) {
        case L_CONV: case L_AGEMM: case L_GCONV: case L_DWCONV: return backward_pass ? 5 : 0;
        case L_IMGGRAD: return 1;
        case L_POOLF: case L_AVGF: case L_POOL3F: return 2;
        case L_POOLB: case L_AVGB: case L_POOL3B: return 3;
        case L_ADDMASK: case L_MEMSET: case L_SOFTMAX: return 4;
        case L_SE_SQUEEZE: case L_SE_EXCITE: case L_SE_SCALE: return 4;
    }
    return 4;
}

static double launch_bytes(const std::vector<Launch>& L, size_t li, int fb, int fuse, int frames, int clips, int accumulate) {
    const Launch& l = L[li];
    const I2VConvParams& q = l.conv;
    const double out = (double)frames * q.Hg * q.Wg * q.Cd;
    const double src = (double)clips * q.Ts * q.Cs * q.Hs * q.Ws;
    double b = 4.0 * (src + (double)q.K * q.Cd + out);
    if (q.add0) b += 4.0 * out / (q.add0_stride * q.add0_stride);
    if (q.add1 || l.kind == L_IMGGRAD) b += (q.add1 || accumulate || l.img_accumulate) ? 4.0 * out : 0.0;
    if (q.mask) b += 4.0 * out;
    if (q.gate) b += out / 8.0;
    if (q.gate_out) b += out / 8.0;
    if (fb) {
        const I2VConvParams& last = L[li + fb - 1].conv;
        const double outl = (double)frames * last.Hg * last.Wg * last.Cd;
        b = 4.0 * (src + outl);
        for (int j = 0; j < fb; ++j) {
            const I2VConvParams& r = L[li + j].conv;
            const double o = (double)frames * r.Hg * r.Wg * r.Cd;
            b += 4.0 * (double)r.K * r.Cd + (r.gate ? o / 8.0 : 0.0) + (r.gate_out ? o / 8.0 : 0.0);
        }
        if (fb == 3) b += 4.0 * outl;
    }
    if (fuse) {
        const I2VConvParams& r = L[li + 1].conv;
        const double out2 = (double)frames * r.Hg * r.Wg * r.Cd;
        b += 4.0 * ((double)r.K * r.Cd + out2) - 4.0 * out;
        if (r.add0) b += 4.0 * out2;
        if (r.add1) b += 4.0 * out2;
        if (r.mask) b += 4.0 * out2;
        if (r.gate) b += out2 / 8.0;
        if (r.gate_out) b += out2 / 8.0;
    }
    return b;
}

namespace {

struct ListTiming {
    i2v_ctx* h; i2v_stream_t s; bool backward_pass;
    TimedLaunch* prev = nullptr;
    TimedLaunch* seg = nullptr;

    TimedLaunch* open(const std::vector<Launch>& L, size_t li, int fb, int fuse, int frames, int clips, int accumulate) {
        const Launch& l = L[li];
        const int kind = launch_timing_kind(l, backward_pass);
        const double flops = launch_flops(L, li, fb, fuse, frames, clips);
        const bool conv = l.kind == L_CONV || l.kind == L_IMGGRAD || l.kind == L_GCONV || l.kind == L_DWCONV;
        if (h->timing == 2) {
            if (!seg || seg->kind != kind) {
                close();
                seg = timing_begin(h, kind, 0.0, s, seg);
                if (seg) seg->count = 0;
            }
            if (seg) { seg->flops += flops; seg->count += 1; if (conv) seg->bytes += launch_bytes(L, li, fb, fuse, frames, clips, accumulate); else seg->bytes += l.se_bytes_per_frame * frames; }
            return prev = nullptr;
        }
        TimedLaunch* const tl = prev = timing_begin(h, kind, flops, s, prev);
        if (tl && conv) {
            tl->Cd = l.conv.Cd; tl->K = l.conv.K; tl->HWg = l.conv.Hg * l.conv.Wg; tl->frames = frames; tl->pw = l.conv.pointwise;
            tl->bytes = launch_bytes(L, li, fb, fuse, frames, clips, accumulate);
        }
        if (tl && l.kind == L_AGEMM) {
            const I2VAttnGemm& q = l.ag;
            tl->Cd = q.Cc; tl->K = q.form == 1 ? q.Cc : (q.form == 2 ? q.N : q.M); tl->HWg = q.form == 2 ? q.M : q.N; tl->frames = frames; tl->pw = 10 + q.form;
            tl->bytes = 4.0 * clips * ((double)q.M * q.N + (double)q.Cc * q.M + (double)q.Cc * q.N);
        }
        if (tl && (l.kind == L_SE_SQUEEZE || l.kind == L_SE_EXCITE || l.kind == L_SE_SCALE)) {
            tl->Cd = l.se.C; tl->K = l.se.rd; tl->HWg = l.se.HW; tl->frames = frames;
            tl->pw = 20 + (l.kind == L_SE_SQUEEZE ? 0 : l.kind == L_SE_EXCITE ? 1 : 2) + 3 * l.se.backward;
            tl->bytes = l.se_bytes_per_frame * frames;
        }
        return tl;
    }
    void close() { if (seg) be_event_record(seg->stop, s); }
};

struct SideStream {
    Net& n; std::vector<Launch>& L; const std::vector<std::vector<int>>& at; i2v_stream_t main;
    int clips; const float* x; float* gx; int accumulate;
    struct Pending { int join; void* done; };
    std::vector<Pending> pending;

    void* event() {
        if (n.ov_used == n.ov_ev.size()) { void* e = be_event_create(); if (!e) return nullptr; n.ov_ev.push_back(e); }
        return n.ov_ev[n.ov_used++];
    }
    int issue(int p) {
        for (int i : at[p + 1]) {
            void* ready = event(); void* done = event();
            if (!ready || !done) return fail("launch overlap: event creation failed");
            CHECK_BE(be_event_record(ready, main)); CHECK_BE(be_stream_wait_event(n.side, ready));
            Launch& m = L[i];
            const int fr = clips * m.T;
            if (fr * m.conv.Hg * m.conv.Wg != 0) {
                const int cb = m.cfg_b[cfg_bucket(clips, n.maxN / n.Tin())];
                if (cb) m.conv.cfg = cb;
                if (conv_run(m, fr, x, gx, accumulate, n.side)) return 1;
                __atomic_fetch_add(&g_overlap_launches, 1, __ATOMIC_RELAXED);
            }
            CHECK_BE(be_event_record(done, n.side));
            pending.push_back(Pending{m.ov_join, done});
        }
        return 0;
    }
    int join(int upto) {
        for (size_t i = 0; i < pending.size();) {
            if (pending[i].join <= upto) { CHECK_BE(be_stream_wait_event(main, pending[i].done)); pending[i] = pending.back(); pending.pop_back(); }
            else ++i;
        }
        return 0;
    }
};

}

static int run_list(i2v_ctx* h, Net& n, std::vector<Launch>& L, int in_frames, const float* x, float* gx, int accumulate,
                    i2v_stream_t s, bool backward_pass) {
    const int clips = in_frames / n.Tin();
    const int bucket = cfg_bucket(clips, n.maxN / n.Tin());
    ListTiming timing{h, s, backward_pass};
    SideStream side{n, L, n.ov_at[backward_pass ? 1 : 0], s, clips, x, gx, accumulate};
    const bool overlap = !h->timing && n.side && !side.at.empty() && in_frames <= n.ov_max_frames;
    if (overlap) n.ov_used = 0;
    if (overlap && side.issue(-1)) return 1;
    for (size_t li = 0; li < L.size(); ++li) {
        Launch& l = L[li];
        const int frames = clips * l.T;
        const size_t li0 = li;
        if (overlap && l.ov_after != -2) continue;
        const int fuse = (l.kind == L_CONV && l.fuse_ok && li + 1 < L.size() && frames * l.conv.Hg * l.conv.Wg > 0 && fused_fits(l, L[li + 1], frames))
                             ? l.fuse_b[bucket] : 0;
        const int fb = (l.kind == L_CONV && l.fb_ok && li + l.fb_ok <= L.size() && frames * l.conv.Hg * l.conv.Wg > 0) ? l.fb_b[bucket] * l.fb_ok : 0;
        if (overlap && side.join((int)li + (fb ? fb - 1 : fuse ? 1 : 0))) return 1;
        TimedLaunch* const tl = h->timing ? timing.open(L, li, fb, fuse, frames, clips, accumulate) : nullptr;
        struct Stop { TimedLaunch* t; i2v_stream_t s; ~Stop() { if (t) be_event_record(t->stop, s); } } stop{tl, s};
        switch (l.kind) {
            case L_CONV:
            case L_IMGGRAD: {
                if (frames * l.conv.Hg * l.conv.Wg == 0) break;
                if (fuse) { if (fused_run(l, L[li + 1], frames, x, fuse == 2, s)) return 1; ++li; break; }
                if (fb) {
                    const int rc = fast_run(L, li, frames, x, s);
                    if (rc == 1) return 1;
                    if (rc == 0) { li += fb - 1; break; }
                }
                const int cb = l.cfg_b[bucket];
                if (cb) l.conv.cfg = cb;
                if (conv_run(l, frames, x, gx, accumulate, s)) return 1;
            } break;
            case L_GCONV: {
#ifdef I2V_HAVE_GCONV
                I2VGConvParams p = l.gc; p.N = frames; CHECK_BE(k_gconv(p, s));
#else
                return fail("this build has no grouped-convolution kernel");
#endif
            } break;
            case L_DWCONV: {
#ifdef I2V_HAVE_DWCONV
                I2VDwConvParams p = l.dc; p.N = frames; CHECK_BE(k_dwconv(p, s));
#else
                return fail("this build has no depthwise-convolution kernel");
#endif
            } break;
#ifdef I2V_HAVE_SE
            case L_SE_SQUEEZE: { I2VSeParams p = l.se; p.N = frames; CHECK_BE(k_se_squeeze(p, s)); } break;
            case L_SE_EXCITE: { I2VSeParams p = l.se; p.N = frames; CHECK_BE(k_se_excite(p, s)); } break;
            case L_SE_SCALE: { I2VSeParams p = l.se; p.N = frames; CHECK_BE(k_se_scale(p, s)); } break;
#else
            case L_SE_SQUEEZE: { I2VSeParams p = l.se; p.N = frames; if (se_host::squeeze(p)) return fail("squeeze-and-excitation: squeeze failed"); } break;
            case L_SE_EXCITE: { I2VSeParams p = l.se; p.N = frames; if (se_host::excite(p)) return fail("squeeze-and-excitation: excite failed"); } break;
            case L_SE_SCALE: { I2VSeParams p = l.se; p.N = frames; if (se_host::scale(p)) return fail("squeeze-and-excitation: scale failed"); } break;
#endif
            case L_POOLF: { I2VPoolParams p = l.pool; p.N = frames; CHECK_BE(k_pool_fwd(p, s)); } break;
            case L_POOL3F: {
                I2VPoolParams p = l.pool; p.N = frames;
                if (p.kt == 1 && p.pad_t == 0 && p.Ts == p.stride_t * p.To) { p.x_nstride *= p.stride_t; CHECK_BE(k_pool_fwd(p, s)); }
                else CHECK_BE(k_pool3d_fwd(p, s));
            } break;
            case L_POOL3B: {
                I2VPoolParams p = l.pool; p.N = frames;
                if (p.kt == 1 && p.pad_t == 0 && p.Ts == p.stride_t * p.To && p.gx_nstride == (int64_t)p.C * p.Hs * p.Ws) {
                    CHECK_BE(be_memset0(p.gx, (size_t)frames * p.stride_t * p.gx_nstride * sizeof(float), s));
                    p.x_nstride *= p.stride_t; p.gx_nstride *= p.stride_t;
                    CHECK_BE(k_pool_bwd(p, s));
                } else CHECK_BE(k_pool3d_bwd(p, s));
            } break;
            case L_AVGF: { I2VPoolParams p = l.pool; p.N = frames; CHECK_BE(k_avgpool_fwd(p, s)); } break;
            case L_AVGB: { I2VPoolParams p = l.pool; p.N = frames; CHECK_BE(k_avgpool_bwd(p, s)); } break;
            case L_MEMSET:
                if (!l.ms_gx) CHECK_BE(be_memset0(l.ms_ptr, l.ms_floats_per_frame * frames * sizeof(float), s));
                else if (!accumulate) CHECK_BE(be_memset0(gx, l.ms_floats_per_frame * frames * sizeof(float), s));
                break;
            case L_POOLB: { I2VPoolParams p = l.pool; p.N = frames; CHECK_BE(k_pool_bwd(p, s)); } break;
            case L_ADDMASK: { I2VAddMaskParams p = l.am; p.N = frames; CHECK_BE(k_addmask(p, s)); } break;
            case L_AGEMM: { I2VAttnGemm p = l.ag; p.clips = clips; CHECK_BE(k_attn_gemm(p, s)); } break;
            case L_SOFTMAX: { I2VSoftmaxRows p = l.sm; p.rows = (int64_t)clips * l.sm_rows_per_clip; CHECK_BE(k_softmax_rows(p, s)); } break;
        }
        if (overlap) for (size_t p = li0; p <= li; ++p) if (side.issue((int)p)) return 1;
    }
    if (overlap && side.join((int)L.size())) return 1;
    timing.close();
    return 0;
}

extern "C" int i2v_net_forward(i2v_handle h, int net, const float* x, int frames, void* stream) {
    Net* n = get_net(h, net); if (!n) return 1;
    if (!n->planned) return fail("net not planned");
    if (frames <= 0 || frames > n->maxN) return fail("frames=%d outside 1..%d", frames, n->maxN);
    if (frames % n->Tin()) return fail("frames=%d is not a multiple of the input's %d frames per clip", frames, n->Tin());
    if (!x) return fail("null input");
    n->frames = frames;
    if (n->stage_input) {
        static const bool always = [] { const char* e = getenv("I2V_STAGE_COPY"); return e && e[0] == '1'; }();
        bool need = always || ((uintptr_t)x & 15) != 0;
        const int bucket = cfg_bucket(frames / n->Tin(), n->maxN / n->Tin());
        for (const Launch& l : n->fwd)
            if (l.kind == L_CONV && l.src_is_input && l.conv.quad && !(l.cfg_b[bucket] > 0 && ((l.cfg_b[bucket] - 1) & 1024))) need = true;
        if (need) {
            const Buffer& ib = n->bufs[n->tens[n->input].buf];
            const size_t bytes = (size_t)frames * ib.C * ib.H * ib.W * sizeof(float);
            float* staged = n->arena + n->in_stage_off;
            CHECK_BE(be_d2d_2d(staged, bytes, x, bytes, bytes, 1, stream));
// ... 16 lines not shown
    return 0;
}

#define I2V_TIMING_FIELDS 8
extern "C" int i2v_timing_collect_ex(i2v_handle h, double* out, int n_kinds, int n_fields) {
    if (!h || !out || n_kinds < 6 || n_fields < I2V_TIMING_FIELDS) return fail("i2v_timing_collect_ex: bad argument");
    for (int i = 0; i < n_kinds * n_fields; ++i) out[i] = 0.0;
    if (h->timed_used) CHECK_BE(be_device_sync());
    const char* dump_path = getenv("I2V_TIMING_DUMP");
    FILE* dump = dump_path ? fopen(dump_path, "a") : nullptr;
    for (size_t i = 0; i < h->timed_used; ++i) {
        const TimedLaunch& t = h->timed[i];
        float ms = 0.f;
        CHECK_BE(be_event_elapsed_ms(t.chain_from ? t.chain_from : t.start, t.stop, &ms));
        if (dump && h->timing != 2) fprintf(dump, "%d %d %d %d %d %d %.4f %.3f %.3f\n", t.kind, t.Cd, t.K, t.HWg, t.frames, t.pw, ms, t.flops * 1e-9, t.bytes * 1e-6);
        if (t.kind < 0 || t.kind >= n_kinds) continue;
        double* o = out + (size_t)t.kind * n_fields;
        o[0] += ms; o[1] += t.flops; o[2] += t.count; o[3] += t.bytes;
        if (h->timing != 2 && t.bytes > 0 && t.flops < 19.7 * t.bytes) { o[4] += ms; o[5] += t.bytes; o[6] += 1; o[7] += t.flops; }
    }
    if (dump) fclose(dump);
    h->timed_used = 0;
    return 0;
}

extern "C" int i2v_timing_collect(i2v_handle h, double* ms_by_kind, double* flops_by_kind, int64_t* launches_by_kind,
                                  int n_kinds) {
    if (!h || !ms_by_kind || !flops_by_kind || !launches_by_kind || n_kinds < 6 || n_kinds > 16) return fail("i2v_timing_collect: bad argument");
    double tmp[16 * I2V_TIMING_FIELDS];
    if (i2v_timing_collect_ex(h, tmp, n_kinds, I2V_TIMING_FIELDS)) return 1;
    for (int i = 0; i < n_kinds; ++i) {
        ms_by_kind[i] = tmp[i * I2V_TIMING_FIELDS]; flops_by_kind[i] = tmp[i * I2V_TIMING_FIELDS + 1];
        launches_by_kind[i] = (int64_t)tmp[i * I2V_TIMING_FIELDS + 2];
    }
    return 0;
}

extern "C" int i2v_net_hook_info(i2v_handle h, int net, int hook, float** act, int64_t* act_stride,
                                 float** grad, int64_t* grad_stride, int64_t* D, int32_t* post_relu) {
    Net* n = get_net(h, net); if (!n) return 1;
    if (!n->planned) return fail("net not planned");
    if (hook < 0 || hook >= (int)n->hooks.size()) return fail("bad hook index");
    int t = n->hooks[hook];
    View a = view_of(*n, t, false), g = view_of(*n, t, true);
    int64_t d = (int64_t)a.C * a.H * a.W;
    if (act) *act = a.p;
    if (act_stride) *act_stride = a.nstride;
    if (grad_stride) *grad_stride = n->hook_tmp[hook] ? d : g.nstride;
    if (grad) *grad = n->hook_tmp[hook] ? n->hook_tmp[hook] : g.p;
    if (D) *D = d;
    if (post_relu) *post_relu = n->tens[t].post_relu ? 1 : 0;
    return 0;
}

extern "C" int i2v_net_read_tensor(i2v_handle h, int net, int tensor, int which, float* out, int frames,
                                   void* stream) {
    Net* n = get_net(h, net); if (!n) return 1;
    if (!n->planned) return fail("net not planned");
    if (tensor < 0 || tensor >= (int)n->tens.size() || tensor == n->input) return fail("bad tensor id");
    View v = view_of(*n, tensor, which != 0);
    if (frames <= 0 || frames > n->maxN / n->Tin() * v.T) return fail("bad frame count");
    for (const std::vector<Launch>* L : {&n->fwd, &n->bwd})
        for (const Launch& l : *L) {
            if (l.kind != L_CONV || !l.fuse_ok || !(l.fuse_b[0] | l.fuse_b[1] | l.fuse_b[2] | l.fuse_b[3])) continue;
            const float* lo = l.conv.dst; const float* hi = lo + (int64_t)(n->maxN / n->Tin() * std::max(1, l.conv.To) - 1) * l.conv.dst_nstride + (int64_t)l.conv.Cd * l.conv.Ho * l.conv.Wo;
            const float* vlo = v.p; const float* vhi = v.p + (int64_t)(frames - 1) * v.nstride + (int64_t)v.C * v.H * v.W;
            if (vlo < hi && lo < vhi)
                return fail("i2v_net_read_tensor: this tensor is the intermediate of a fused 3x3 -> pointwise pair and is never stored "
                            "(plan without I2V_FUSE / I2V_FORCE_FUSE to read it)");
        }
    for (const std::vector<Launch>* L : {&n->fwd, &n->bwd})
        for (size_t i = 0; i < L->size(); ++i) {
            const Launch& l = (*L)[i];
            if (l.kind != L_CONV || !l.fb_ok || !(l.fb_b[0] | l.fb_b[1] | l.fb_b[2] | l.fb_b[3])) continue;
            for (int j = 0; j + 1 < l.fb_ok && i + j < L->size(); ++j) {
                const I2VConvParams& q = (*L)[i + j].conv;
                const float* lo = q.dst; const float* hi = lo + (int64_t)(n->maxN / n->Tin() * std::max(1, q.To) - 1) * q.dst_nstride + (int64_t)q.Cd * q.Ho * q.Wo;
                const float* vlo = v.p; const float* vhi = v.p + (int64_t)(frames - 1) * v.nstride + (int64_t)v.C * v.H * v.W;
                if (vlo < hi && lo < vhi)
                    return fail("i2v_net_read_tensor: this tensor is an intermediate of a fused fast-pathway block and is never stored "
                                "(plan with I2V_FASTBLOCK=0 to read it)");
            }
        }
    size_t row = (size_t)v.C * v.H * v.W * sizeof(float);
    CHECK_BE(be_d2d_2d(out, row, v.p, (size_t)v.nstride * sizeof(float), row, frames, stream));
    return 0;
}
```

### image-to-video-i2v-attack_amd/csrc/i2v_tune.cpp

```cpp
#include "i2v_net.h"

#include <stdio.h>
#include <stdlib.h>
#include <string.h>

#include <algorithm>

namespace eng {

void mark_fusable(Net& n) {
    const int64_t frames = n.maxN, clips = n.maxN / n.Tin();
    typedef std::pair<const float*, const float*> Range;
    auto rng = [](const void* q, int64_t fr, int64_t ns, int64_t plane) {
        const float* f = (const float*)q;
        return f ? Range(f, f + (fr > 0 ? (fr - 1) * ns : 0) + std::max<int64_t>(plane, 1)) : Range(nullptr, nullptr);
    };
    auto meet = [](const Range& a, const Range& b) { return a.first && b.first && a.first < b.second && b.first < a.second; };
    auto touches = [&](const Launch& c, const Range& w, bool skip_src, bool skip_dst) {
        if (c.kind == L_CONV || c.kind == L_IMGGRAD || c.kind == L_GCONV || c.kind == L_DWCONV) {
            const I2VConvParams& q = c.conv;
            const int64_t fs = clips * std::max(1, q.Ts), fo = clips * std::max(1, q.To), dplane = (int64_t)(q.blk > 1 ? q.Cd / (q.blk * q.blk) : q.Cd) * q.Ho * q.Wo;
            return (!skip_src && meet(w, rng(q.src, fs, q.src_nstride, (int64_t)q.Cs * q.Hs * q.Ws))) ||
                   meet(w, rng(q.add0, fo, q.add0_nstride, dplane)) || meet(w, rng(q.add1, fo, q.add1_nstride, dplane)) ||
                   meet(w, rng(q.mask, fo, q.mask_nstride, dplane)) || (!skip_dst && meet(w, rng(q.dst, fo, q.dst_nstride, dplane)));
// ... 39 lines not shown
    for (std::vector<Launch>* L : {&n.fwd, &n.bwd})
        for (size_t i = 0; i + 1 < L->size(); ++i) {
            Launch& a = (*L)[i]; Launch& b = (*L)[i + 1];
            a.fuse_ok = 0;
            if (a.kind != L_CONV || b.kind != L_CONV || a.src_is_input || b.src_is_input || a.T != b.T) continue;
            const int ok = k_conv_fusable(a.conv, b.conv);
            if (!ok) continue;
            const Range w = dst_of(a);
            bool other = false;
            for (auto& hk : hooked) other |= meet(hk, w);
            for (std::vector<Launch>* M : {&n.fwd, &n.bwd})
                for (size_t j = 0; j < M->size() && !other; ++j)
                    other |= touches((*M)[j], w, M == L && j == i + 1, M == L && j == i);
            if (!other) a.fuse_ok = ok;
            if (getenv("I2V_FUSE_DEBUG"))
                fprintf(stderr, "[i2v fuse] %s pair %zu: 3x3 Cd=%d K=%d %dx%d -> 1x1 Cd=%d K=%d: eligible=%d other_reader=%d\n", L == &n.fwd ? "fwd" : "bwd", i,
                        a.conv.Cd, a.conv.K, a.conv.Hg, a.conv.Wg, b.conv.Cd, b.conv.K, ok, (int)other);
        }
    {
        const bool fb_off = [] { const char* e = getenv("I2V_FASTBLOCK"); return e && e[0] == '0'; }();
        auto cd_of = [&](const Launch& l) -> const i2v_conv3d_desc* { return (l.kind == L_CONV && l.node >= 0 && n.nodes[l.node].type == 0 && !n.nodes[l.node].preact()) ? &n.nodes[l.node].cd : nullptr; };
        auto unit = [](const i2v_conv3d_desc& c) { return c.stride == 1 && c.stride_t == 1 && c.dil_t == 1; };
        auto is_pw = [&](const i2v_conv3d_desc& c) { return unit(c) && c.kt == 1 && c.kh == 1 && c.kw == 1 && c.pad == 0 && c.pad_t == 0; };
        auto is_t = [&](const i2v_conv3d_desc& c) { return unit(c) && c.kh == 1 && c.kw == 1 && c.pad == 0 && (c.kt & 1) && 2 * c.pad_t == c.kt - 1; };
        auto is_33 = [&](const i2v_conv3d_desc& c) { return unit(c) && c.kt == 1 && c.kh == 3 && c.kw == 3 && c.pad == 1 && c.pad_t == 0; };
        auto private_to = [&](std::vector<Launch>* L, size_t first, size_t last, const Launch& w) {
            const Range r = dst_of(w);
            for (auto& hk : hooked) if (meet(hk, r)) return false;
            for (std::vector<Launch>* M : {&n.fwd, &n.bwd})
                for (size_t j = 0; j < M->size(); ++j) {
                    if (M == L && j >= first && j <= last) continue;
                    if (touches((*M)[j], r, false, false)) return false;
                }
            return true;
        };
        for (Launch& l : n.fwd) l.fb_ok = 0;
        for (Launch& l : n.bwd) l.fb_ok = 0;
        for (size_t i = 0; !fb_off && i + 2 < n.bwd.size(); ++i) {
            Launch& a = n.bwd[i]; Launch& x = n.bwd[i + 1]; Launch& b = n.bwd[i + 2];
            const i2v_conv3d_desc* ca = cd_of(a); const i2v_conv3d_desc* cb = cd_of(b);
            if (!ca || !cb || !is_pw(*ca) || !is_33(*cb) || b.conv.src != a.conv.dst || x.kind != L_CONV) continue;
            const I2VConvParams& px = x.conv;
            const bool dep = touches(x, dst_of(a), false, false) || touches(a, dst_of(x), false, false) || touches(x, dst_of(b), false, false) || touches(b, dst_of(x), false, false) ||
                             (px.gate_out && (px.gate_out == a.conv.gate || px.gate_out == b.conv.gate));
            if (!dep) { Launch t = x; n.bwd[i + 1] = n.bwd[i]; n.bwd[i] = t; }
        }
        for (size_t i = 0; !fb_off && i + 1 < n.bwd.size(); ++i) {
            Launch& a = n.bwd[i]; Launch& b = n.bwd[i + 1];
            const i2v_conv3d_desc* ca = cd_of(a); const i2v_conv3d_desc* cb = cd_of(b);
            if (!ca || !cb || !is_pw(*ca) || !is_33(*cb) || a.T != b.T || b.conv.src != a.conv.dst) continue;
            if (i2v_fastblock_rows(a.conv, b.conv, nullptr, nullptr) <= 0) continue;
            if (!private_to(&n.bwd, i, i + 1, a)) continue;
            a.fb_ok = 2;
        }
        for (size_t i = 0; !fb_off && i + 2 < n.fwd.size(); ++i) {
            Launch& a = n.fwd[i]; Launch& b = n.fwd[i + 1];
            const i2v_conv3d_desc* ca = cd_of(a); const i2v_conv3d_desc* cb = cd_of(b);
            if (!ca || !cb || a.src_is_input || !(is_t(*ca) || is_pw(*ca)) || !is_33(*cb) || !ca->relu || !cb->relu || ca->residual >= 0 || cb->residual >= 0 || cb->src != ca->dst) continue;
            Launch& c3 = n.fwd[i + 2];
            const i2v_conv3d_desc* cc = cd_of(c3);
            if (!cc || !is_pw(*cc)) continue;
            if (cc->src == cb->dst && cc->residual >= 0 && cc->relu && a.T == b.T && a.T == c3.T) {
                if (i2v_fastblock_rows(a.conv, b.conv, &c3.conv, nullptr) <= 0) continue;
                if (!private_to(&n.fwd, i, i + 2, a) || !private_to(&n.fwd, i, i + 2, b)) continue;
                a.fb_ok = 3;
            } else if (i + 3 < n.fwd.size() && cc->src == ca->src && !cc->relu && cc->residual < 0) {
                Launch& c4 = n.fwd[i + 3];
                const i2v_conv3d_desc* c4d = cd_of(c4);
                if (!c4d || !is_pw(*c4d) || c4d->src != cb->dst || c4d->residual != cc->dst || !c4d->relu || a.T != b.T || a.T != c3.T || a.T != c4.T) continue;
                if (i2v_fastblock_rows(a.conv, b.conv, &c4.conv, &c3.conv) <= 0) continue;
                if (!private_to(&n.fwd, i, i + 3, a) || !private_to(&n.fwd, i, i + 3, b) || !private_to(&n.fwd, i, i + 3, c3)) continue;
                a.fb_ok = 4;
            }
        }
        const bool fb_force = [] { const char* e = getenv("I2V_FORCE_FASTBLOCK"); return e && e[0] == '1'; }();
        for (std::vector<Launch>* L : {&n.fwd, &n.bwd})
            for (Launch& a : *L)
                for (int bk = 0; bk < 4; ++bk) a.fb_b[bk] = (a.fb_ok && fb_force) ? 1 : 0;
        if (getenv("I2V_FUSE_DEBUG"))
            for (std::vector<Launch>* L : {&n.fwd, &n.bwd})
                for (size_t i = 0; i < L->size(); ++i)
                    if ((*L)[i].fb_ok) fprintf(stderr, "[i2v fastblock] %s launch %zu: group of %d (Cs %d -> %d mid channels, %dx%d)\n", L == &n.fwd ? "fwd" : "bwd", i, (*L)[i].fb_ok,
                                               (*L)[i].conv.Cs, (*L)[i].conv.Cd, (*L)[i].conv.Hg, (*L)[i].conv.Wg);
    }
    const char* force = getenv("I2V_FORCE_FUSE");
    const int f = force ? atoi(force) : 0;
    for (std::vector<Launch>* L : {&n.fwd, &n.bwd})
        for (Launch& a : *L)
            for (int b = 0; b < 4; ++b) a.fuse_b[b] = (a.fuse_ok && f) ? ((f == 2 && (a.fuse_ok & 2)) ? 2 : 1) : 0;
}

void mark_overlap(Net& n) {
    for (int k = 0; k < 2; ++k) n.ov_at[k].clear();
    for (std::vector<Launch>* L : {&n.fwd, &n.bwd}) for (Launch& l : *L) { l.ov_after = -2; l.ov_join = -1; }
    const char* e = getenv("I2V_OVERLAP_MAX_FRAMES");
    n.ov_max_frames = e ? atoi(e) : 0;
    if (n.ov_max_frames <= 0) return;
    const int64_t clips = n.maxN / n.Tin();
    typedef std::pair<const char*, const char*> Range;
    struct RW { std::vector<Range> r, w; bool barrier = false; };
    static const char gx_tag[16] = {0};
    const Range GX(gx_tag, gx_tag + 16);
    auto rng = [](const void* q, int64_t fr, int64_t stride_bytes, int64_t plane_bytes) {
        const char* f = (const char*)q;
        return f ? Range(f, f + (fr > 0 ? (fr - 1) * stride_bytes : 0) + std::max<int64_t>(plane_bytes, 1)) : Range(nullptr, nullptr);
    };
    auto rw_of = [&](const Launch& c) {
        RW o;
        auto rd = [&](const Range& x) { if (x.first) o.r.push_back(x); };
        auto wr = [&](const Range& x) { if (x.first) o.w.push_back(x); };
        if (c.kind == L_CONV || c.kind == L_IMGGRAD || c.kind == L_GCONV || c.kind == L_DWCONV) {
            const I2VConvParams& q = c.conv;
            const int64_t fs = clips * std::max(1, q.Ts), fo = clips * std::max(1, q.To);
            const int64_t dplane = 4ll * (q.blk > 1 ? q.Cd / (q.blk * q.blk) : q.Cd) * q.Ho * q.Wo;
            if (!c.src_is_input) rd(rng(q.src, fs, 4 * q.src_nstride, 4ll * q.Cs * q.Hs * q.Ws));
            rd(rng(q.add0, fo, 4 * q.add0_nstride, dplane)); rd(rng(q.add1, fo, 4 * q.add1_nstride, dplane)); rd(rng(q.mask, fo, 4 * q.mask_nstride, dplane));
            rd(rng(q.gate, 1, 0, 4ll * q.Cd * q.gate_stride)); wr(rng(q.gate_out, 1, 0, 4ll * q.Cd * q.gate_out_stride));
            if (c.kind == L_IMGGRAD) { wr(GX); rd(GX); } else wr(rng(q.dst, fo, 4 * q.dst_nstride, dplane));
        } else if (c.kind == L_ADDMASK) {
            const int64_t fr = clips * std::max(1, c.T), pl = 4ll * c.am.C * c.am.HW;
            wr(rng(c.am.out, fr, 4 * c.am.out_nstride, pl));
            for (int i = 0; i < 3; ++i) rd(rng(c.am.a[i], fr, 4 * c.am.a_nstride[i], pl));
            rd(rng(c.am.mask, fr, 4 * c.am.mask_nstride, pl)); rd(rng(c.am.gate, 1, 0, 4ll * c.am.C * c.am.gate_stride));
        } else if (c.kind == L_MEMSET) {
            if (c.ms_gx) wr(GX); else wr(rng(c.ms_ptr, 1, 0, 4ll * (int64_t)c.ms_floats_per_frame * clips * std::max(1, c.T)));
        } else if (c.kind == L_AGEMM || c.kind == L_SOFTMAX) {
            o.barrier = true;
        } else if (c.kind == L_SE_SQUEEZE || c.kind == L_SE_EXCITE || c.kind == L_SE_SCALE) {
            const I2VSeParams& q = c.se;
            const int64_t fr = clips * std::max(1, c.T), pl = 4ll * q.C * q.HW;
            const Range vec = rng(c.se_vec, 1, 0, 4ll * (int64_t)c.se_vec_floats);
            rd(vec); wr(vec);
            if (c.kind != L_SE_EXCITE) { rd(rng(q.x, fr, 4 * q.x_nstride, pl)); rd(rng(q.g, fr, 4 * q.g_nstride, pl)); }
            if (c.kind == L_SE_SCALE) {
                rd(rng(q.r, fr, 4 * q.r_nstride, pl)); wr(rng(q.dst, fr, 4 * q.dst_nstride, pl));
                wr(rng(q.gate_out, 1, 0, 4ll * q.C * q.gate_out_stride));
            }
        } else {
            const I2VPoolParams& q = c.pool;
            const int64_t fr = clips * std::max(std::max(1, c.T), std::max(q.Ts, q.To)), pin = 4ll * q.C * q.Hs * q.Ws, pout = 4ll * q.C * q.Ho * q.Wo;
            const Range idx = rng(q.idx, 1, 0, fr * (int64_t)q.C * q.Ho * q.Wo);
            const bool fwd = c.kind == L_POOLF || c.kind == L_POOL3F || c.kind == L_AVGF;
            if (fwd) { rd(rng(q.x, fr, 4 * q.x_nstride, pin)); wr(rng(q.y, fr, 4 * q.y_nstride, pout)); wr(idx); }
            else { rd(rng(q.x, fr, 4 * q.x_nstride, pin)); rd(rng(q.y, fr, 4 * q.y_nstride, pout)); rd(rng(q.yact, fr, 4 * q.yact_nstride, pout)); rd(idx);
                   wr(rng(q.gx, fr * std::max(1, q.stride_t), 4 * q.gx_nstride, pin)); }
        }
        return o;
    };
    auto meet = [](const std::vector<Range>& A, const std::vector<Range>& B) {
        for (const Range& a : A) for (const Range& b : B) if (a.first < b.second && b.first < a.second) return true;
        return false;
    };
    auto conflict = [&](const RW& a, const RW& b) { return a.barrier || b.barrier || meet(a.r, b.w) || meet(a.w, b.w) || meet(a.w, b.r); };
    int k = 0;
    for (std::vector<Launch>* L : {&n.fwd, &n.bwd}) {
        const int M = (int)L->size();
        std::vector<RW> rw; rw.reserve(M);
        for (const Launch& l : *L) rw.push_back(rw_of(l));
        std::vector<char> member(M, 0);
        for (int i = 0; i < M; ++i) {
            const Launch& l = (*L)[i];
            for (int j = 0; j < l.fb_ok && i + j < M; ++j) member[i + j] = 1;
            if (l.fuse_ok) { member[i] = 1; if (i + 1 < M) member[i + 1] = 1; }
        }
        n.ov_at[k].assign(M + 1, {});
        int hoisted = 0;
// ... 85 lines not shown
                for (int ci = 0; ci < nc; ++ci) {
                    float ms = 0.f;
                    if (time_cfg(cand[ci] + 1, &ms)) return 1;
                    if ((cand[ci] & 2048) && getenv("I2V_FUSE_DEBUG"))
                        fprintf(stderr, "[i2v vfma] %s launch Cd %d K %d (%dx%d) at %d frames: conv_vfma %.1f us, best tile so far %.1f us\n", list_name(n, L),
                                l.conv.Cd, l.conv.K, l.conv.Hg, l.conv.Wg, lf, 1e3f * ms, 1e3f * best);
                    if (ms < best) { best = ms; best_c = cand[ci]; }
                }
                static const bool no_nt = [] { const char* e = getenv("I2V_NT"); return e && e[0] == '0'; }();
                if (best_c >= 0 && l.kind == L_CONV && !no_nt) {
                    float ms = 0.f;
                    if (time_cfg((best_c | 128) + 1, &ms)) return 1;
                    if (ms < 0.98f * best) { best = ms; best_c |= 128; }
                }
                l.cfg_b[b] = best_c >= 0 ? best_c + 1 : 0;
                return 0;
            });
            l.conv.cfg = l.cfg_b[0] ? l.cfg_b[0] : planned_cfg;
            if (rc) return 1;
        }
    return 0;
}

int tune_fastblocks(Net& n, Probe& pr, int max_clips) {
    const bool fb_force = [] { const char* e = getenv("I2V_FORCE_FASTBLOCK"); return e && e[0] == '1'; }();
    for (std::vector<Launch>* L : {&n.fwd, &n.bwd})
        for (size_t i = 0; i < L->size(); ++i) {
            Launch& a = (*L)[i];
            if (!a.fb_ok || i + a.fb_ok > L->size()) continue;
            for (int bk = 0; bk < 4; ++bk) a.fb_b[bk] = 0;
            const int rc = for_each_bucket(max_clips, a.conv.Tg, [&](int bk, int lf) -> int {
                auto run_sep = [&]() { for (int j = 0; j < a.fb_ok; ++j) { Launch& m = (*L)[i + j]; if (m.cfg_b[bk]) m.conv.cfg = m.cfg_b[bk]; if (conv_run(m, lf, pr.x, pr.gx, 0, nullptr)) return 1; } return 0; };
                auto run_fb = [&]() { return fast_run(*L, i, lf, pr.x, nullptr); };
                float t_sep = 0.f, t_fb = 0.f;
                if (run_fb() != 0) return 0;
                if (pr.time(run_sep, 3, &t_sep) || pr.time(run_fb, 3, &t_fb)) return 1;
                a.fb_b[bk] = (fb_force || t_fb < 0.97f * t_sep) ? 1 : 0;
                if (getenv("I2V_FUSE_DEBUG"))
                    fprintf(stderr, "[i2v fastblock] %s group %zu (%d launches, %d -> %d mid channels) at %d frames: separate %.1f us, fused %.1f us -> %s\n",
                            list_name(n, L), i, a.fb_ok, a.conv.Cs, a.conv.Cd, lf, 1e3f * t_sep, 1e3f * t_fb, a.fb_b[bk] ? "fused" : "separate");
                return 0;
            });
            for (int j = 0; j < a.fb_ok; ++j) { Launch& m = (*L)[i + j]; m.conv.cfg = m.cfg_b[0] ? m.cfg_b[0] : m.conv.cfg; }
            if (rc) return 1;
        }
    return 0;
}

int tune_pairs(Net& n, Probe& pr, int max_clips) {
    for (std::vector<Launch>* L : {&n.fwd, &n.bwd})
        for (size_t i = 0; i + 1 < L->size(); ++i) {
            Launch& a = (*L)[i]; Launch& b = (*L)[i + 1];
            if (!a.fuse_ok) continue;
            for (int bk = 0; bk < 4; ++bk) a.fuse_b[bk] = 0;
            const int rc = for_each_bucket(max_clips, a.conv.Tg, [&](int bk, int lf) -> int {
                if (!fused_fits(a, b, lf)) return 0;
                const int ca = a.conv.cfg, cb = b.conv.cfg;
                if (a.cfg_b[bk]) a.conv.cfg = a.cfg_b[bk];
                if (b.cfg_b[bk]) b.conv.cfg = b.cfg_b[bk];
                float best = 1e30f; int best_v = 0, rc = 0;
                for (int v = 0; v <= ((a.fuse_ok & 2) ? 2 : 1); ++v) {
                    auto once = [&]() { return v == 0 ? (conv_run(a, lf, pr.x, pr.gx, 0, nullptr) || conv_run(b, lf, pr.x, pr.gx, 0, nullptr))
                                                      : fused_run(a, b, lf, pr.x, v == 2, nullptr); };
                    if (v > 0 && once()) {
                        if (getenv("I2V_FUSE_DEBUG")) fprintf(stderr, "[i2v fuse] pair %zu variant %d does not launch: %s\n", i, v, g_err.c_str());
                        g_err.clear(); continue;
                    }
                    float ms = 0.f;
                    if (pr.time(once, 2, &ms, v == 0)) { rc = 1; break; }
                    if ((v == 0 ? ms : ms * 1.03f) < best) { best = v == 0 ? ms : ms * 1.03f; best_v = v; }
                    if (getenv("I2V_FUSE_DEBUG"))
                        fprintf(stderr, "[i2v fuse] %s pair %zu (Cd %d -> %d, %dx%d) at %d frames: variant %d = %.1f us\n", list_name(n, L), i,
                                a.conv.Cd, b.conv.Cd, a.conv.Hg, a.conv.Wg, lf, v, 1e3f * ms);
                }
                a.fuse_b[bk] = best_v;
                a.conv.cfg = ca; b.conv.cfg = cb;
                return rc;
            });
            if (rc) return 1;
        }
    return 0;
}

}

int autotune(Net& n) {
    const char* off = getenv("I2V_AUTOTUNE");
    if (off && off[0] == '0') return 0;
    int rc;
    {
        Probe pr;
        if (pr.init(n)) return 1;
        const int max_clips = n.maxN / n.Tin();
        const bool on_device = strncmp(be_name(), "hip", 3) == 0;
        rc = tune_tiles(n, pr, max_clips);
        if (!rc && on_device) rc = tune_fastblocks(n, pr, max_clips);
        static const bool fuse_on = [] { const char* e = getenv("I2V_FUSE"); return e && e[0] == '1'; }();
        if (!rc && fuse_on && on_device) rc = tune_pairs(n, pr, max_clips);
    }
    if (rc) return g_err.empty() ? fail("autotune failed") : 1;
    CHECK_BE(be_memset0(n.arena, n.arena_floats * sizeof(float), nullptr));
    return 0;
}

}
```

### image-to-video-i2v-attack_amd/i2v_amd/engine.py

```python
import ctypes as C
import sys
import threading
import time
from typing import List, Sequence

import torch

from . import lib as _lib
from .graphs import ConvNextSpec, Graph, MixerSpec, SwinSpec, VitSpec
from .weights import fold_affine, fold_pre_affine


_DEVICE_TYPES = {}


def _ptr(t: torch.Tensor, eng: "Engine" = None):
    assert t.is_contiguous() and t.dtype == torch.float32, (t.dtype, t.is_contiguous())
    ok = t.device.type == eng.device.type if eng is not None else _DEVICE_TYPES.get(t.device.type, 0) > 0
    if not ok:
        where = eng.device if eng is not None else sorted(k for k, v in _DEVICE_TYPES.items() if v > 0)
        raise _lib.I2VError(f"tensor on {t.device} passed to an engine on {where}: move it to the engine's device")
    return C.c_void_p(t.data_ptr())


# ... 312 lines not shown
            if nd.op == "conv":
                w = sd[nd.weight].float().cpu().contiguous()
                scale, shift = fold_affine(nd, sd)
                scale, shift = scale.contiguous(), shift.contiguous()
                if g.video:
                    d = _lib.Conv3dDesc(self.ten_id[nd.src], self.ten_id[nd.dst], nd.cin, nd.cout, nd.kt, nd.kh, nd.kw,
                                        nd.stride_t, nd.stride, nd.pad_t, nd.pad, nd.dil_t, 1 if nd.relu else 0,
                                        -1 if nd.residual is None else self.ten_id[nd.residual])
                    _lib.check(capi, capi.i2v_net_add_conv3d(h, self.id, C.byref(d), _hptr(w), _hptr(scale), _hptr(shift)))
                    continue
                d = _lib.ConvDesc(self.ten_id[nd.src], self.ten_id[nd.dst], nd.cin, nd.cout, nd.kh, nd.kw,
                                  nd.stride, nd.pad, 1 if nd.relu else 0,
                                  -1 if nd.residual is None else self.ten_id[nd.residual])
                if nd.pre_bn:
                    ps, pt = fold_pre_affine(nd, sd)
                    ps, pt = ps.contiguous(), pt.contiguous()
                    _lib.check(capi, capi.i2v_net_add_conv_preact(h, self.id, C.byref(d), _hptr(w), _hptr(scale), _hptr(shift),
                                                                  _hptr(ps), _hptr(pt)))
                elif getattr(nd, "groups", 1) > 1 and nd.groups == nd.cin == nd.cout:
                    _lib.check(capi, capi.i2v_net_add_conv_depthwise(h, self.id, C.byref(d), _hptr(w), _hptr(scale), _hptr(shift)))
                elif getattr(nd, "groups", 1) > 1:
                    _lib.check(capi, capi.i2v_net_add_conv_grouped(h, self.id, C.byref(d), nd.groups, _hptr(w), _hptr(scale), _hptr(shift)))
                else:
                    _lib.check(capi, capi.i2v_net_add_conv(h, self.id, C.byref(d), _hptr(w), _hptr(scale), _hptr(shift)))
            elif nd.op == "se":
                w1 = sd[nd.fc1 + ".weight"].float().cpu().reshape(nd.rd, nd.C).contiguous()
                w2 = sd[nd.fc2 + ".weight"].float().cpu().reshape(nd.C, nd.rd).contiguous()
                b1, b2 = sd[nd.fc1 + ".bias"].float().cpu().contiguous(), sd[nd.fc2 + ".bias"].float().cpu().contiguous()
                d = _lib.SeDesc(self.ten_id[nd.src], self.ten_id[nd.dst], -1 if nd.residual is None else self.ten_id[nd.residual],
                                nd.C, nd.rd, 1 if nd.relu else 0)
                _lib.check(capi, capi.i2v_net_add_se(h, self.id, C.byref(d), _hptr(w1), _hptr(b1), _hptr(w2), _hptr(b2)))
            elif nd.op == "attention":
                d = _lib.AttnDesc(self.ten_id[nd.src], self.ten_id[nd.phi], self.ten_id[nd.g], self.ten_id[nd.dst], float(nd.scale))
                _lib.check(capi, capi.i2v_net_add_attention(h, self.id, C.byref(d)))
            elif g.video:
                d = _lib.Pool3dDesc(self.ten_id[nd.src], self.ten_id[nd.dst], nd.kt, nd.k, nd.stride_t, nd.stride, nd.pad_t, nd.pad)
                _lib.check(capi, capi.i2v_net_add_maxpool3d(h, self.id, C.byref(d)))
            else:
                d = _lib.PoolDesc(self.ten_id[nd.src], self.ten_id[nd.dst], nd.k, nd.stride, nd.pad)
                add = capi.i2v_net_add_avgpool if nd.op == "avgpool" else capi.i2v_net_add_maxpool
                _lib.check(capi, add(h, self.id, C.byref(d)))
        for t, gain in (relu_gain or {}).items():
            if t in self.ten_id:
                _lib.check(capi, capi.i2v_net_set_relu_gain(h, self.id, self.ten_id[t], float(gain)))
        hooks = (C.c_int * len(hook_tensors))(*[self.ten_id[t] for t in hook_tensors])
        _lib.check(capi, capi.i2v_net_plan(h, self.id, hooks, len(hook_tensors), max_frames))
        self.hook_tensors = hook_tensors
        self.hooks = [self._hook_info(i) for i in range(len(hook_tensors))]

    def _hook_info(self, i) -> HookInfo:
        act, grad = C.c_void_p(), C.c_void_p()
        a_s, g_s, D, pr = C.c_int64(), C.c_int64(), C.c_int64(), C.c_int32()
        _lib.check(self.eng.capi, self.eng.capi.i2v_net_hook_info(
            self.eng.h, self.id, i, C.byref(act), C.byref(a_s), C.byref(grad), C.byref(g_s), C.byref(D), C.byref(pr)))
        hi = HookInfo()
        hi.act, hi.act_stride, hi.grad, hi.grad_stride = act.value, a_s.value, grad.value, g_s.value
        hi.D, hi.post_relu = D.value, pr.value
        ts = self.graph.tensors[self.hook_tensors[i]]
        hi.shape = (ts.C, ts.H, ts.W)
        hi.T = ts.T
        return hi

    def close(self):
        if self.id is not None and self.eng.h:
            with self.eng.plan_lock:
                self.eng.capi.i2v_net_destroy(self.eng.h, self.id)
        self.id = None

    def __del__(self):
        try:
            if not sys.is_finalizing():
                self.close()
        except Exception:
            pass

    def workspace_bytes(self) -> int:
        return self.eng.capi.i2v_net_workspace_bytes(self.eng.h, self.id)

    def fusion_info(self):
        out = (C.c_int32 * 4)()
        _lib.check(self.eng.capi, self.eng.capi.i2v_net_fusion_info(self.eng.h, self.id, out))
        return tuple(int(v) for v in out)

    def forward(self, x: torch.Tensor):
        _lib.check(self.eng.capi, self.eng.capi.i2v_net_forward(self.eng.h, self.id, _ptr(x, self.eng), x.shape[0], self.eng.stream()))

    def backward(self, gx: torch.Tensor, accumulate=False):
        _lib.check(self.eng.capi, self.eng.capi.i2v_net_backward(self.eng.h, self.id, _ptr(gx, self.eng), 1 if accumulate else 0,
                                                                 self.eng.stream()))

    def read_tensor(self, tid: int, frames: int, grad=False) -> torch.Tensor:
        ts = self.graph.tensors[tid]
        out = torch.empty(frames, ts.C, ts.H, ts.W, dtype=torch.float32, device=self.eng.device)
        _lib.check(self.eng.capi, self.eng.capi.i2v_net_read_tensor(self.eng.h, self.id, self.ten_id[tid], 1 if grad else 0,
                                                                    _ptr(out, self.eng), frames, self.eng.stream()))
        return out

    def save_hook(self, i: int, frames: int) -> torch.Tensor:
        return self.read_tensor(self.hook_tensors[i], frames)

    def cossim(self, i: int, init: torch.Tensor, cos_out: torch.Tensor, scratch: torch.Tensor, frames: int,
               coef_dev=None, coef_index=0, coef_host=1.0):
        hi = self.hooks[i]
        capi = self.eng.capi
        _lib.check(capi, capi.i2v_cossim_fwd_bwd_f32(
            C.c_void_p(hi.act), hi.act_stride, _ptr(init, self.eng), hi.D, hi.D, frames,
            C.c_void_p(coef_dev.data_ptr()) if coef_dev is not None else C.c_void_p(0), coef_index, coef_host,
            hi.post_relu, 0, C.c_void_p(cos_out.data_ptr()), C.c_void_p(hi.grad), hi.grad_stride,
            C.c_void_p(scratch.data_ptr()), self.eng.stream()))

    def stdloss(self, i: int, std_out: torch.Tensor, scratch: torch.Tensor, frames: int, exchange=None):
        hi = self.hooks[i]
        capi = self.eng.capi
        _lib.check(capi, capi.i2v_std_reduce_f32(C.c_void_p(hi.act), hi.act_stride, hi.D, frames,
                                                 C.c_void_p(scratch.data_ptr()), self.eng.stream()))
        total = frames * hi.D
        if exchange is not None:
            total = exchange(scratch[:16].view(torch.float64), total)
        _lib.check(capi, capi.i2v_std_grad_f32(
            C.c_void_p(hi.act), hi.act_stride, hi.D, frames, total, hi.post_relu, 0, C.c_void_p(std_out.data_ptr()),
            C.c_void_p(hi.grad), hi.grad_stride, C.c_void_p(scratch.data_ptr()), self.eng.stream()))

    def hook_frames(self, i: int, in_frames: int) -> int:
        return in_frames // self.graph.tensors[self.graph.input].T * self.hooks[i].T

    def ilaf_scratch_bytes(self, i: int, frames: int, frames_per_seg: int = 0) -> int:
        return self.eng.capi.i2v_ilaf_scratch_bytes(self.hooks[i].D, frames, frames_per_seg)

    def ilaf_reduce(self, i: int, ori: torch.Tensor, adv0: torch.Tensor, scratch: torch.Tensor, frames: int, act=None,
                    frames_per_seg: int = 0):
        hi = self.hooks[i]
        capi = self.eng.capi
        a, a_s = (C.c_void_p(hi.act), hi.act_stride) if act is None else (_ptr(act, self.eng), hi.D)
        if frames_per_seg:
            _lib.check(capi, capi.i2v_ilaf_reduce_seg_f32(a, a_s, _ptr(ori, self.eng), _ptr(adv0, self.eng), hi.D, frames, frames_per_seg,
                                                          C.c_void_p(scratch.data_ptr()), self.eng.stream()))
            return
        _lib.check(capi, capi.i2v_ilaf_reduce_f32(a, a_s, _ptr(ori, self.eng), _ptr(adv0, self.eng), hi.D, frames,
                                                  C.c_void_p(scratch.data_ptr()), self.eng.stream()))

    def ilaf_grad(self, i: int, ori, adv0, init_norm, loss_out: torch.Tensor, scratch: torch.Tensor, frames: int,
                  frames_per_seg: int = 0):
        hi = self.hooks[i]
        capi = self.eng.capi
        if frames_per_seg:
            assert init_norm.dtype == torch.float64 and init_norm.numel() == frames // frames_per_seg
            _lib.check(capi, capi.i2v_ilaf_grad_seg_f32(C.c_void_p(hi.act), hi.act_stride, _ptr(ori, self.eng), _ptr(adv0, self.eng), hi.D, frames,
                                                        frames_per_seg, C.c_void_p(init_norm.data_ptr()), hi.post_relu, 0,
                                                        C.c_void_p(loss_out.data_ptr()), C.c_void_p(hi.grad), hi.grad_stride,
                                                        C.c_void_p(scratch.data_ptr()), self.eng.stream()))
            return
        _lib.check(capi, capi.i2v_ilaf_grad_f32(C.c_void_p(hi.act), hi.act_stride, _ptr(ori, self.eng), _ptr(adv0, self.eng), hi.D, frames,
                                                init_norm, hi.post_relu, 0, C.c_void_p(loss_out.data_ptr()),
                                                C.c_void_p(hi.grad), hi.grad_stride, C.c_void_p(scratch.data_ptr()),
                                                self.eng.stream()))

    def tap_distance(self, i: int, clean: torch.Tensor, coef: float, dist_out: torch.Tensor, scratch: torch.Tensor, frames: int,
                     frames_per_seg: int):
        hi = self.hooks[i]
        _lib.check(self.eng.capi, self.eng.capi.i2v_tap_distance_f32(
            C.c_void_p(hi.act), hi.act_stride, _ptr(clean, self.eng), hi.D, frames, frames_per_seg, float(coef), hi.post_relu, 0,
            C.c_void_p(dist_out.data_ptr()), C.c_void_p(hi.grad), hi.grad_stride, C.c_void_p(scratch.data_ptr()), self.eng.stream()))

    def head_ce(self, i, W: torch.Tensor, bias, labels: torch.Tensor, in_frames: int, scale: float, logits: torch.Tensor,
                loss_each: torch.Tensor, scratch: torch.Tensor):
        capi = self.eng.capi
# ... 185 lines not shown
```

### image-to-video-i2v-attack_amd/i2v_amd/lib.py

```python
import ctypes as C
import os

_HERE = os.path.dirname(os.path.abspath(__file__))
LIB_PATH = os.path.join(_HERE, "libi2v_hip.so")
HIP_BACKEND = b"hip:gfx950"


class ConvDesc(C.Structure):
    _fields_ = [(n, C.c_int32) for n in
                ("src", "dst", "cin", "cout", "kh", "kw", "stride", "pad", "relu", "residual")]


class PoolDesc(C.Structure):
    _fields_ = [(n, C.c_int32) for n in ("src", "dst", "k", "stride", "pad")]


class Conv3dDesc(C.Structure):
    _fields_ = [(n, C.c_int32) for n in
                ("src", "dst", "cin", "cout", "kt", "kh", "kw", "stride_t", "stride", "pad_t", "pad", "dil_t",
                 "relu", "residual")]


class AttnDesc(C.Structure):
    _fields_ = [(n, C.c_int32) for n in ("theta", "phi", "g", "dst")] + [("scale", C.c_float)]


class SeDesc(C.Structure):
    _fields_ = [(n, C.c_int32) for n in ("src", "dst", "residual", "C", "rd", "relu")]


class Pool3dDesc(C.Structure):
    _fields_ = [(n, C.c_int32) for n in ("src", "dst", "kt", "k", "stride_t", "stride", "pad_t", "pad")]


class I2VError(RuntimeError):
    pass


_P, _I, _L, _F = C.c_void_p, C.c_int, C.c_int64, C.c_float
_PROTOS = {
    "i2v_create": ([_I, C.POINTER(_P)], _I),
    "i2v_destroy": ([_P], _I),
    "i2v_last_error": ([], C.c_char_p),
    "i2v_abi_version": ([], _I),
    "i2v_backend": ([], C.c_char_p),
    "i2v_backend_stat": ([C.c_char_p], C.c_longlong),
    "i2v_net_create": ([_P, C.POINTER(_I)], _I),
    "i2v_net_destroy": ([_P, _I], _I),
    "i2v_net_add_buffer": ([_P, _I, _I, _I, _I, C.POINTER(_I)], _I),
    "i2v_net_add_tensor": ([_P, _I, _I, _I, _I, _I, C.POINTER(_I)], _I),
    "i2v_net_set_input": ([_P, _I, _I], _I),
    "i2v_net_set_relu_gain": ([_P, _I, _I, _F], _I),
    "i2v_net_add_conv": ([_P, _I, C.POINTER(ConvDesc), _P, _P, _P], _I),
    "i2v_net_add_conv_grouped": ([_P, _I, C.POINTER(ConvDesc), _I, _P, _P, _P], _I),
    "i2v_net_add_conv_depthwise": ([_P, _I, C.POINTER(ConvDesc), _P, _P, _P], _I),
    "i2v_net_add_maxpool": ([_P, _I, C.POINTER(PoolDesc)], _I),
    "i2v_net_add_conv_preact": ([_P, _I, C.POINTER(ConvDesc), _P, _P, _P, _P, _P], _I),
    "i2v_net_add_avgpool": ([_P, _I, C.POINTER(PoolDesc)], _I),
    "i2v_net_add_buffer3d": ([_P, _I, _I, _I, _I, _I, C.POINTER(_I)], _I),
    "i2v_net_add_conv3d": ([_P, _I, C.POINTER(Conv3dDesc), _P, _P, _P], _I),
    "i2v_net_add_maxpool3d": ([_P, _I, C.POINTER(Pool3dDesc)], _I),
    "i2v_net_add_attention": ([_P, _I, C.POINTER(AttnDesc)], _I),
    "i2v_net_add_se": ([_P, _I, C.POINTER(SeDesc), _P, _P, _P, _P], _I),
    "i2v_net_tensor_frames": ([_P, _I, _I, C.POINTER(_I)], _I),
    "i2v_net_plan": ([_P, _I, C.POINTER(_I), _I, _I], _I),
    "i2v_net_workspace_bytes": ([_P, _I], C.c_size_t),
    "i2v_net_fusion_info": ([_P, _I, _P], _I),
    "i2v_net_forward": ([_P, _I, _P, _I, _P], _I),
    "i2v_net_hook_info": ([_P, _I, _I, C.POINTER(_P), C.POINTER(_L), C.POINTER(_P), C.POINTER(_L),
                           C.POINTER(_L), C.POINTER(C.c_int32)], _I),
    "i2v_net_backward": ([_P, _I, _P, _I, _P], _I),
    "i2v_net_read_tensor": ([_P, _I, _I, _I, _P, _I, _P], _I),
    "i2v_timing_enable": ([_P, _I], _I),
    "i2v_timing_collect": ([_P, C.POINTER(C.c_double), C.POINTER(C.c_double), C.POINTER(_L), _I], _I),
    "i2v_timing_collect_ex": ([_P, C.POINTER(C.c_double), _I, _I], _I),
    "i2v_clip_from_u8_f32": ([_P, _P, _I, _I, _I, _I, _P], _I),
    "i2v_clip_resize_crop_u8_f32": ([_P, _P, _P, _P, _I, _I, _I, _I, _I, _I, _I, _I, _I, _I, _P], _I),
    "i2v_frames_from_video_f32": ([_P, _P, _P, _I, _I, _I, _I, _P], _I),
    "i2v_compose_f32": ([_P, _P, _P, _I, _I, _I, _I, _F, _I, _P], _I),
    "i2v_cossim_scratch_bytes": ([_L, _I], C.c_size_t),
    "i2v_cossim_fwd_bwd_f32": ([_P, _L, _P, _L, _L, _I, _P, _I, _F, _I, _I, _P, _P, _L, _P, _P], _I),
    "i2v_std_fwd_bwd_f32": ([_P, _L, _L, _I, _I, _I, _P, _P, _L, _P, _P], _I),
    "i2v_std_reduce_f32": ([_P, _L, _L, _I, _P, _P], _I),
    "i2v_std_grad_f32": ([_P, _L, _L, _I, _L, _I, _I, _P, _P, _L, _P, _P], _I),
    "i2v_adam_step_f32": ([_P, _P, _P, _P, _P, _L, _I, _F, C.c_double, C.c_double, C.c_double, C.c_double, _I, _P], _I),
    "i2v_sign_step_f32": ([_P, _P, _P, _L, _L, _F, _F, _P], _I),
    "i2v_sign_step_delta_f32": ([_P, _P, _L, _F, _P], _I),
    "i2v_sign_step_delta_gx_f32": ([_P, _P, _P, _L, _F, _F, _P], _I),
    "i2v_ilaf_reduce_f32": ([_P, _L, _P, _P, _L, _I, _P, _P], _I),
    "i2v_ilaf_grad_f32": ([_P, _L, _P, _P, _L, _I, C.c_double, _I, _I, _P, _P, _L, _P, _P], _I),
    "i2v_ilaf_scratch_bytes": ([_L, _I, _I], C.c_size_t),
    "i2v_ilaf_reduce_seg_f32": ([_P, _L, _P, _P, _L, _I, _I, _P, _P], _I),
    "i2v_ilaf_grad_seg_f32": ([_P, _L, _P, _P, _L, _I, _I, _P, _I, _I, _P, _P, _L, _P, _P], _I),
    "i2v_tap_distance_f32": ([_P, _L, _P, _L, _I, _I, C.c_double, _I, _I, _P, _P, _L, _P, _P], _I),
    "i2v_head_scratch_bytes": ([_I, _I], C.c_size_t),
    "i2v_head_ce_f32": ([_P, _L, _I, _I, _I, _I, _P, _P, _I, _P, _F, _I, _I, _P, _P, _P, _L, _P, _P], _I),
    "i2v_clip_resample_crop_u8_f32": ([_P, _P, _P, _P, _I, _P, _P, _I, _I, _I, _I, _I, _I, _I, _I, _I, _I, _I, _P], _I),
    "i2v_tt_grad_mix_f32": ([_P, _P, _P, _P, _I, _L, _I, _I, _F, _P], _I),
    "i2v_resample_nearest_f32": ([_P, _P, _L, _I, _I, _I, _I, _P, _P, _P], _I),
    "i2v_resample_nearest_bwd_f32": ([_P, _P, _L, _I, _I, _I, _I, _P, _P, _P, _P, _P], _I),
    "i2v_dwconv1d_f32": ([_P, _P, _L, _I, _L, _P, _I, _P], _I),
    "i2v_tap_scratch_bytes": ([_L], _L),
    "i2v_tap_perts_f32": ([_P, _P, _P, _I, _I, _I, _I, _I, _P], _I),
    "i2v_tap_sign_abs_f32": ([_P, _P, _P, _L, _P, _P], _I),
    "i2v_tap_grad_f32": ([_P, _P, _P, _I, _I, _I, _I, _I, _F, _P], _I),
    "i2v_grad_post_scratch_bytes": ([_I, _I, _I, _I, _I, _I], _L),
    "i2v_grad_post_f32": ([_P, _P, _P, _I, _I, _I, _I, _I, _I, _I, _F, _P, _P], _I),
    "i2v_head_pool_f32": ([_P, _L, _I, _I, _I, _I, _I, _I, _P, _P], _I),
    "i2v_head_logits_ce_f32": ([_I, _I, _P, _P, _I, _P, _F, _P, _P, _P, _P], _I),
    "i2v_head_grad_f32": ([_P, _L, _I, _I, _I, _I, _I, _I, _I, _I, _P, _L, _P, _P], _I),
    "i2v_aens_coeffs_f32": ([_P, _P, _F, _I, _P], _I),
    "i2v_aens_reduce_f32": ([_P, _P, _I, _I, _P, _P, _P], _I),
}
EXPORTS = tuple(_PROTOS)
_LOADER_PROTOS = {
    "i2v_clip_gather_scratch_bytes": ([_I, _I, _I, _I], _L),
    "i2v_clip_gather_resize_crop_u8_f32": ([_P, _L, _P, _P, _I, _I, _P, _I, _P, _I, _I, _I, _P, _P, _L, _P], _I),
}
LOADER_EXPORTS = tuple(_LOADER_PROTOS)


class VitConfig(C.Structure):
    _fields_ = [(n, C.c_int32) for n in ("img", "patch", "in_chans", "dim", "heads", "mlp", "blocks")] + [("ln_eps", C.c_float)]


_VIT_PROTOS = {
    "i2v_vit_create": ([_I, C.POINTER(VitConfig), C.POINTER(_P), _I, C.POINTER(C.c_int32), _I, _I, C.POINTER(_P)], _I),
    "i2v_vit_create_ex": ([_I, C.POINTER(VitConfig), _I, C.POINTER(_P), _I, C.POINTER(C.c_int32), _I, _I, C.POINTER(_P)], _I),
    "i2v_vit_destroy": ([_P], _I),
    "i2v_vit_workspace_bytes": ([_P], _L),
    "i2v_vit_forward": ([_P, _P, _I, _P], _I),
    "i2v_vit_backward": ([_P, _P, _I, _P], _I),
    "i2v_vit_hook_info": ([_P, _I, C.POINTER(_P), C.POINTER(_L), C.POINTER(_P), C.POINTER(_L), C.POINTER(_L)], _I),
    "i2v_vit_read_hook": ([_P, _I, _I, _P, _I, _P], _I),
    "i2v_vit_linear_f32": ([_P, _I, _I, _P, _P, _I, _P, _P, _P, _P], _I),
    "i2v_vit_linear_bwd_f32": ([_P, _I, _I, _P, _I, _P, _P, _P], _I),
    "i2v_vit_layernorm_f32": ([_P, _L, _I, _P, _P, _F, _P, _P, _P, _P], _I),
    "i2v_vit_layernorm_bwd_f32": ([_P, _P, _P, _P, _P, _L, _I, _P, _P, _P, _P], _I),
    "i2v_vit_probs_ld": ([_I], _I),
    "i2v_vit_attention_f32": ([_P, _I, _I, _I, _I, _F, _P, _P, _P], _I),
    "i2v_vit_attention_bwd_f32": ([_P, _P, _P, _I, _I, _I, _I, _F, _P, _P, _P], _I),
    "i2v_vit_embed_f32": ([_P, _I, _I, _I, _I, _P, _P, _P, _P, _I, _P, _P, _P, _P], _I),
    "i2v_vit_embed_bwd_f32": ([_P, _I, _I, _I, _I, _P, _I, _P, _P, _I, _P], _I),
    "i2v_vit_embed_ex_f32": ([_P, _I, _I, _I, _I, _P, _P, _P, _I, _P, _I, _P, _P, _P, _P], _I),
    "i2v_vit_embed_bwd_ex_f32": ([_P, _I, _I, _I, _I, _P, _I, _I, _P, _P, _I, _P], _I),
}
VIT_EXPORTS = tuple(_VIT_PROTOS)


class SwinConfig(C.Structure):
# ... 92 lines not shown
```

### include/i2v_hip.h

```cpp
#ifndef I2V_HIP_H
#define I2V_HIP_H
#include <stddef.h>
#include <stdint.h>

#ifdef __cplusplus
extern "C" {
#endif

typedef struct i2v_ctx* i2v_handle;

int i2v_create(int device, i2v_handle* out);
int i2v_destroy(i2v_handle h);
const char* i2v_last_error(void);
int i2v_abi_version(void);
const char* i2v_backend(void);
long long i2v_backend_stat(const char* name);

typedef struct {
    int32_t src, dst;
    int32_t cin, cout, kh, kw, stride, pad;
    int32_t relu;
    int32_t residual;
} i2v_conv_desc;

typedef struct {
    int32_t src, dst;
    int32_t k, stride, pad;
} i2v_pool_desc;

int i2v_net_create(i2v_handle h, int* net);
int i2v_net_destroy(i2v_handle h, int net);
int i2v_net_add_buffer(i2v_handle h, int net, int C, int H, int W, int* buf);
int i2v_net_add_tensor(i2v_handle h, int net, int buf, int c_off, int C, int post_relu, int* tensor);
int i2v_net_set_input(i2v_handle h, int net, int tensor);
int i2v_net_set_relu_gain(i2v_handle h, int net, int tensor, float gain);
int i2v_net_add_conv(i2v_handle h, int net, const i2v_conv_desc* d, const float* weight,
                     const float* scale, const float* shift);
int i2v_net_add_conv_grouped(i2v_handle h, int net, const i2v_conv_desc* d, int groups, const float* weight,
                             const float* scale, const float* shift);
int i2v_net_add_conv_depthwise(i2v_handle h, int net, const i2v_conv_desc* d, const float* weight,
                               const float* scale, const float* shift);
int i2v_net_add_maxpool(i2v_handle h, int net, const i2v_pool_desc* d);
int i2v_net_add_conv_preact(i2v_handle h, int net, const i2v_conv_desc* d, const float* weight,
                            const float* scale, const float* shift, const float* pre_scale,
                            const float* pre_shift);
int i2v_net_add_avgpool(i2v_handle h, int net, const i2v_pool_desc* d);
typedef struct {
    int32_t src, dst;
    int32_t cin, cout, kt, kh, kw;
    int32_t stride_t, stride, pad_t, pad, dil_t;
    int32_t relu, residual;
} i2v_conv3d_desc;
typedef struct {
    int32_t src, dst;
    int32_t kt, k, stride_t, stride, pad_t, pad;
} i2v_pool3d_desc;
int i2v_net_add_buffer3d(i2v_handle h, int net, int C, int T, int H, int W, int* buf);
int i2v_net_add_conv3d(i2v_handle h, int net, const i2v_conv3d_desc* d, const float* weight,
                       const float* scale, const float* shift);
int i2v_net_add_maxpool3d(i2v_handle h, int net, const i2v_pool3d_desc* d);
typedef struct {
    int32_t theta, phi, g, dst;
    float scale;
} i2v_attn_desc;
int i2v_net_add_attention(i2v_handle h, int net, const i2v_attn_desc* d);
typedef struct {
    int32_t src, dst, residual;
    int32_t C, rd, relu;
} i2v_se_desc;
int i2v_net_add_se(i2v_handle h, int net, const i2v_se_desc* d, const float* W1, const float* b1, const float* W2, const float* b2);
int i2v_net_tensor_frames(i2v_handle h, int net, int tensor, int* T);
int i2v_net_plan(i2v_handle h, int net, const int* hook_tensors, int n_hooks, int max_frames);
size_t i2v_net_workspace_bytes(i2v_handle h, int net);
int i2v_net_fusion_info(i2v_handle h, int net, int32_t out[4]);

int i2v_net_forward(i2v_handle h, int net, const float* x, int frames, void* stream);
int i2v_net_hook_info(i2v_handle h, int net, int hook, float** act, int64_t* act_stride,
                      float** grad, int64_t* grad_stride, int64_t* D, int32_t* post_relu);
int i2v_net_backward(i2v_handle h, int net, float* gx, int accumulate, void* stream);
int i2v_net_read_tensor(i2v_handle h, int net, int tensor, int which, float* out, int frames,
                        void* stream);

int i2v_timing_enable(i2v_handle h, int enable);
int i2v_timing_collect(i2v_handle h, double* ms_by_kind, double* flops_by_kind,
                       int64_t* launches_by_kind, int n_kinds);
int i2v_timing_collect_ex(i2v_handle h, double* out, int n_kinds, int n_fields);

int i2v_clip_from_u8_f32(const uint8_t* frames, float* video, int b, int t, int h, int w, void* stream);
int i2v_clip_resize_crop_u8_f32(const uint8_t* frames, float* video, const int32_t* xtab, const int32_t* ytab, int b, int t,
                                int H, int W, int rh, int rw, int crop_y, int crop_x, int out_h, int out_w, void* stream);
int i2v_clip_resample_crop_u8_f32(const uint8_t* frames, float* video, const int32_t* xbounds, const int32_t* xcoef, int kx,
                                  const int32_t* ybounds, const int32_t* ycoef, int ky, int b, int t, int H, int W, int rh, int rw,
                                  int crop_y, int crop_x, int out_h, int out_w, void* stream);
int i2v_frames_from_video_f32(const float* video, float* x, float* u, int b, int f, int h, int w,
                              void* stream);
int i2v_compose_f32(const float* u, const float* delta, float* x, int b, int f, int h, int w,
                    float eps, int video_layout, void* stream);
size_t i2v_cossim_scratch_bytes(int64_t D, int frames);
int i2v_cossim_fwd_bwd_f32(const float* a, int64_t a_stride, const float* b, int64_t b_stride,
                           int64_t D, int frames, const float* coef_dev, int coef_index,
                           float coef_host, int mask_relu, int accumulate, float* cos_out,
                           float* grad, int64_t grad_stride, void* scratch, void* stream);
int i2v_std_fwd_bwd_f32(const float* a, int64_t a_stride, int64_t D, int frames, int mask_relu,
                        int accumulate, float* std_out, float* grad, int64_t grad_stride,
                        void* scratch, void* stream);
int i2v_std_reduce_f32(const float* a, int64_t a_stride, int64_t D, int frames, void* scratch, void* stream);
int i2v_std_grad_f32(const float* a, int64_t a_stride, int64_t D, int frames, int64_t total_count,
                     int mask_relu, int accumulate, float* std_out, float* grad, int64_t grad_stride,
                     void* scratch, void* stream);
int i2v_adam_step_f32(float* delta, float* m, float* v, const float* gx, const float* u,
                      int64_t frames, int hw, float eps, double lr, double beta1, double beta2,
                      double adam_eps, int step_t, void* stream);
int i2v_sign_step_f32(float* adv, const float* u, const float* grad, int64_t n, int64_t chan_stride,
                      float step, float eps, void* stream);
int i2v_sign_step_delta_f32(float* delta, const float* grad, int64_t n, float step, void* stream);
int i2v_sign_step_delta_gx_f32(float* delta, const float* gx, const float* u, int64_t n, float eps,
                               float step, void* stream);
int i2v_ilaf_reduce_f32(const float* a, int64_t a_stride, const float* ori, const float* adv0, int64_t D,
                        int frames, void* scratch, void* stream);
int i2v_ilaf_grad_f32(const float* a, int64_t a_stride, const float* ori, const float* adv0, int64_t D,
                      int frames, double init_norm, int mask_relu, int accumulate, float* loss_out,
                      float* grad, int64_t grad_stride, void* scratch, void* stream);
size_t i2v_ilaf_scratch_bytes(int64_t D, int frames, int frames_per_seg);
int i2v_ilaf_reduce_seg_f32(const float* a, int64_t a_stride, const float* ori, const float* adv0, int64_t D,
                            int frames, int frames_per_seg, void* scratch, void* stream);
int i2v_ilaf_grad_seg_f32(const float* a, int64_t a_stride, const float* ori, const float* adv0, int64_t D,
                          int frames, int frames_per_seg, const double* init_sq, int mask_relu, int accumulate,
                          float* loss_out, float* grad, int64_t grad_stride, void* scratch, void* stream);
int i2v_tap_distance_f32(const float* a, int64_t a_stride, const float* clean, int64_t D, int frames, int frames_per_seg,
                         double coef, int mask_relu, int accumulate, float* dist_out, float* grad, int64_t grad_stride,
                         void* scratch, void* stream);
size_t i2v_head_scratch_bytes(int C, int clips);
int i2v_head_ce_f32(const float* a, int64_t a_stride, int C, int HW, int T, int clips, const float* W, const float* bias,
                    int K, const int32_t* labels, float scale, int mask_relu, int accumulate, float* logits, float* loss_each,
                    float* grad, int64_t grad_stride, void* scratch, void* stream);
int i2v_head_pool_f32(const float* a, int64_t a_stride, int C, int HW, int T, int clips, int Ctot, int c_off, void* scratch, void* stream);
int i2v_head_logits_ce_f32(int Ctot, int clips, const float* W, const float* bias, int K, const int32_t* labels, float scale,
                           float* logits, float* loss_each, void* scratch, void* stream);
int i2v_head_grad_f32(const float* a, int64_t a_stride, int C, int HW, int T, int clips, int Ctot, int c_off, int mask_relu,
                      int accumulate, float* grad, int64_t grad_stride, void* scratch, void* stream);
int i2v_tt_grad_mix_f32(const float* grads, float* out, const float* kernel, const int32_t* moves, int D, int64_t NC, int T, int HW,
                        float weight, void* stream);
int i2v_resample_nearest_f32(const float* src, float* dst, int64_t planes, int Hs, int Ws, int Hd, int Wd, const int32_t* map_y,
                             const int32_t* map_x, void* stream);
int i2v_resample_nearest_bwd_f32(const float* g, float* gsrc, int64_t planes, int Hd, int Wd, int Hs, int Ws, const int32_t* ylo,
                                 const int32_t* yhi, const int32_t* xlo, const int32_t* xhi, void* stream);
int i2v_dwconv1d_f32(const float* src, float* dst, int64_t outer, int len, int64_t inner, const float* taps, int k, void* stream);
int64_t i2v_grad_post_scratch_bytes(int b, int c, int f, int h, int w, int mode);
int i2v_grad_post_f32(const float* g, float* momentum, float* out, int b, int c, int f, int h, int w, int frame_major, int mode, float decay,
                      void* scratch, void* stream);
int64_t i2v_tap_scratch_bytes(int64_t n);
int i2v_tap_perts_f32(const float* adv, const float* videos, float* out, int b, int c, int f, int h, int w, void* stream);
int i2v_tap_sign_abs_f32(const float* smooth, float* sign_out, float* reg, int64_t n, void* scratch, void* stream);
int i2v_tap_grad_f32(const float* gx, const float* boxsign, float* out, int b, int c, int f, int h, int w, float weight, void* stream);
int i2v_aens_coeffs_f32(const float* prev, float* coeffs, float momentum, int L, void* stream);
int i2v_aens_reduce_f32(const float* cos, const float* coeffs, int L, int frames, float* feat_sum,
                        float* weighted, void* stream);
// ... 6 lines not shown
```

Before: 747.4.

## Fuse ResNet shortcut projection conv with block's final conv into one kernel

Adds a paired implicit-GEMM kernel that computes the downsample/shortcut convolution and the following pointwise conv (which adds the shortcut as residual) in the same workgroup, keeping the shortcut tile in registers instead of writing it to and rereading it from global memory. The planner detects eligible pairs when no other launch reads the shortcut buffer, and the autotuner times paired against separate launches per frame bucket and keeps whichever is quicker. In exchange it adds register pressure and LDS reuse across two tile loops, plus more planner complexity and risk around buffer-liveness analysis.

```diff
diff --git a/__graft_entry__.py b/__graft_entry__.py
--- a/__graft_entry__.py
+++ b/__graft_entry__.py
@@ -17,17 +17,18 @@
 
 ENGINE_UNITS = ["i2v_engine.cpp", "i2v_pack.cpp", "i2v_plan.cpp", "i2v_tune.cpp", "i2v_run.cpp", "i2v_loop_api.cpp"]
 UNITS = ["i2v_kernels.hip", "i2v_conv_cfg0.hip", "i2v_conv_cfg1.hip", "i2v_conv_cfg2.hip", "i2v_conv_cfg3.hip", "i2v_conv_cfg4.hip",
-         "i2v_conv_cfg5.hip", "i2v_conv_stems.hip", "i2v_fastblock.hip", "i2v_gconv.hip", "i2v_dwconv.hip", "i2v_se.hip", "i2v_loader.hip", "i2v_vit.hip", "i2v_vit.cpp", "i2v_swin.hip", "i2v_swin.cpp",
+         "i2v_conv_cfg5.hip", "i2v_conv_scpair.hip", "i2v_conv_stems.hip", "i2v_fastblock.hip", "i2v_gconv.hip", "i2v_dwconv.hip", "i2v_se.hip", "i2v_loader.hip", "i2v_vit.hip", "i2v_vit.cpp", "i2v_swin.hip", "i2v_swin.cpp",
          "i2v_convnext.hip", "i2v_convnext.cpp", "i2v_mixer.hip", "i2v_mixer.cpp",
          ] + ENGINE_UNITS
 HEADERS = ["i2v_kernels.h", "i2v_params.h", "i2v_be.h", "i2v_conv_tile.h", "i2v_conv_launch.h", "i2v_vit_kernels.h", "i2v_swin_kernels.h", "i2v_xf.h",
            "i2v_net.h", "i2v_se_host.h", "i2v_convnext_host.h", "i2v_xf_host.h", "i2v_hip_stub.h",
-           "i2v_mixer_host.h", "i2v_gelu.h"]
+           "i2v_mixer_host.h", "i2v_gelu.h", "i2v_scpair_host.h"]
 FLAGS = ["--offload-arch=gfx950", "-O3", "-ffp-contract=off", "-std=c++20", "-fPIC", "-DI2V_SEPARATE_UNITS",
          "-DI2V_HAVE_GCONV", "-DI2V_HAVE_DWCONV",
          "-DI2V_HAVE_SE",
          "-DI2V_HAVE_CONVNEXT",
-         "-DI2V_HAVE_MIXER"]
+         "-DI2V_HAVE_MIXER",
+         "-DI2V_HAVE_SCPAIR"]
 
 
 def build_lib(experimental: bool = False) -> str:
@@ -61,7 +62,7 @@
 
 def build() -> None:
     build_lib(experimental=False)
-    deps = [os.path.join(CSRC, f) for f in ENGINE_UNITS + ["i2v_net.h", "i2v_kernels.h", "i2v_params.h", "i2v_se_host.h", "i2v_convnext_host.h", "i2v_convnext.cpp", "i2v_mixer_host.h", "i2v_mixer.cpp", "i2v_gelu.h", "i2v_xf.h", "i2v_xf_host.h", "i2v_hip_stub.h",
+    deps = [os.path.join(CSRC, f) for f in ENGINE_UNITS + ["i2v_net.h", "i2v_kernels.h", "i2v_params.h", "i2v_se_host.h", "i2v_convnext_host.h", "i2v_convnext.cpp", "i2v_mixer_host.h", "i2v_mixer.cpp", "i2v_scpair_host.h", "i2v_gelu.h", "i2v_xf.h", "i2v_xf_host.h", "i2v_hip_stub.h",
                                                                "i2v_vit_kernels.h", "i2v_swin_kernels.h"]] + [os.path.join(ROOT, "include", "i2v_hip.h")]
     hs = os.path.join(ROOT, "tests", "hostsim")
     if _stale(os.path.join(hs, "libi2v_hostsim.so"), deps + [os.path.join(hs, "hostsim_backend.cpp")]):
diff --git a/image-to-video-i2v-attack_amd/csrc/i2v_be.h b/image-to-video-i2v-attack_amd/csrc/i2v_be.h
--- a/image-to-video-i2v-attack_amd/csrc/i2v_be.h
+++ b/image-to-video-i2v-attack_amd/csrc/i2v_be.h
@@ -19,7 +19,7 @@
 int hip_fail(hipError_t e, const char* what);
 #define HIPCHK(x) do { hipError_t e_ = (x); if (e_ != hipSuccess) return hip_fail(e_, #x); } while (0)
 #define LAUNCH_CHECK(name) do { hipError_t e_ = hipGetLastError(); if (e_ != hipSuccess) return hip_fail(e_, name); } while (0)
-extern long long g_stat_conv, g_stat_pws, g_stat_bf3, g_stat_igh, g_stat_sth, g_stat_fastblock, g_stat_vfma, g_stat_igv, g_stat_gconv, g_stat_dwconv, g_stat_se, g_stat_cndw, g_stat_mixtok;
+extern long long g_stat_conv, g_stat_pws, g_stat_bf3, g_stat_igh, g_stat_sth, g_stat_fastblock, g_stat_vfma, g_stat_igv, g_stat_gconv, g_stat_dwconv, g_stat_se, g_stat_cndw, g_stat_mixtok, g_stat_scpair;
 
 __device__ __forceinline__ unsigned fastdiv(unsigned n, unsigned m, unsigned s) {
     return (unsigned)(((unsigned long long)n * m) >> s);
diff --git a/image-to-video-i2v-attack_amd/csrc/i2v_conv_scpair.hip b/image-to-video-i2v-attack_amd/csrc/i2v_conv_scpair.hip
--- /dev/null
+++ b/image-to-video-i2v-attack_amd/csrc/i2v_conv_scpair.hip
@@ -0,0 +1,72 @@
+#include "i2v_conv_tile.h"
+
+#ifndef I2V_SCPAIR_WPE
+#define I2V_SCPAIR_WPE I2V_PREF_WPE
+#endif
+
+template <int MODE_A>
+__global__ void __launch_bounds__(256) __attribute__((amdgpu_waves_per_eu(I2V_SCPAIR_WPE, I2V_SCPAIR_WPE)))
+conv_igemm_scpair(const I2VConvParams a, const I2VConvParams b, const int n_cd_tiles) {
+    constexpr int BD = 64, BP = 64, WD = 2, WP = 2, FR = 32;
+    constexpr bool PREF_A = MODE_A == 1;
+    constexpr int LA = conv_lds_floats<BD, BP, WD, false, conv_deep(MODE_A, PREF_A) ? I2V_DEEP_STAGES : 2>();
+    constexpr int LB = conv_lds_floats<BD, BP, WD, false, conv_deep(1, true) ? I2V_DEEP_STAGES : 2>();
+    __shared__ __attribute__((aligned(16))) float smem[LA > LB ? LA : LB];
+    I2V_PROBE_T probe;
+    probe.entry();
+    const int lid = conv_xcd_lid(blockIdx.x, gridDim.x);
+    const int cd0 = (lid % n_cd_tiles) * BD;
+    const int64_t px0 = (int64_t)(lid / n_cd_tiles) * BP;
+
+    constexpr int C4 = BP / 4, RSTEP = 1024 / BP, NQ = WD * FR / RSTEP;
+    float4 y[NQ];
+    {
+        f32x16 acc[1][1];
+        float4 pre_a[PREF_A ? NQ : 1]; unsigned gw_a[PREF_A ? NQ : 1];
+        conv_tile_loop<BD, BP, WD, WP, MODE_A, PREF_A>(a, cd0, px0, gridDim.x, smem, probe, blockIdx.x, I2V_PRIO_LEVELS, acc, pre_a, gw_a);
+        float (*Cs)[BP] = reinterpret_cast<float (*)[BP]>(smem);
+        conv_acc_to_rows<BP, WP, false>(acc[0], Cs);
+        const int t = threadIdx.x, c4 = t % C4, rbase = t / C4;
+        const bool pok = px0 + (int64_t)c4 * 4 < (int64_t)a.N * a.Hg * a.Wg;
+#pragma unroll
+        for (int q = 0; q < NQ; ++q) {
+            const int row = rbase + q * RSTEP, cd = cd0 + row;
+            float4 v = make_float4(0.f, 0.f, 0.f, 0.f);
+            if (pok && cd < a.Cd) {
+                v = *reinterpret_cast<const float4*>(&Cs[row][c4 * 4]);
+                if (a.shift) { const float sh = a.shift[cd]; v.x += sh; v.y += sh; v.z += sh; v.w += sh; }
+            }
+            y[q] = v;
+        }
+        __syncthreads();
+    }
+    f32x16 acc[1][1];
+    float4 pre0[NQ]; unsigned pregw[NQ];
+    conv_tile_loop<BD, BP, WD, WP, 1, true>(b, cd0, px0, gridDim.x, smem, probe, blockIdx.x, I2V_PRIO_LEVELS, acc, pre0, pregw);
+#pragma unroll
+    for (int q = 0; q < NQ; ++q) pre0[q] = y[q];
+    conv_vec_epilogue<BD, BP, WD, WP, true, false, false>(b, acc, cd0, px0, smem, pre0, pregw, nullptr);
+    probe.exit(blockIdx.x);
+}
+
+long long g_stat_scpair = 0;
+
+int k_conv_scpair_ok(const I2VConvParams& a, const I2VConvParams& b) { return i2v_conv_scpair_ok(a, b) ? 1 : 0; }
+
+int k_conv_scpair(const I2VConvParams& a_in, const I2VConvParams& b_in, i2v_stream_t s) {
+    I2VConvParams a = a_in, b = b_in;
+    if (!i2v_conv_scpair_ok(a, b)) { snprintf(g_be_err, sizeof g_be_err, "shortcut-pair launch: the two launches do not form a pair"); g_be_has_err = true; return 1; }
+    const int64_t P = (int64_t)b.N * b.Hg * b.Wg;
+    if (P + 1024 >= (1ll << 31)) { snprintf(g_be_err, sizeof g_be_err, "conv launch of more than 2^31 grid pixels"); g_be_has_err = true; return 1; }
+    conv_magics(a); conv_magics(b);
+    b.add0 = nullptr; b.add0_nstride = 0;
+    const int n_cd = (b.Cd + 63) / 64;
+    const int64_t grid = (P + 63) / 64 * n_cd;
+    if (grid <= 0) return 0;
+    if (grid > 0x7fffffff) { snprintf(g_be_err, sizeof g_be_err, "conv grid too large"); g_be_has_err = true; return 1; }
+    __atomic_fetch_add(&g_stat_scpair, 1, __ATOMIC_RELAXED);
+    if (a.pointwise) hipLaunchKernelGGL((conv_igemm_scpair<1>), dim3((unsigned)grid), dim3(256), 0, (hipStream_t)s, a, b, n_cd);
+    else hipLaunchKernelGGL((conv_igemm_scpair<2>), dim3((unsigned)grid), dim3(256), 0, (hipStream_t)s, a, b, n_cd);
+    LAUNCH_CHECK("conv_scpair");
+    return 0;
+}
diff --git a/image-to-video-i2v-attack_amd/csrc/i2v_conv_tile.h b/image-to-video-i2v-attack_amd/csrc/i2v_conv_tile.h
--- a/image-to-video-i2v-attack_amd/csrc/i2v_conv_tile.h
+++ b/image-to-video-i2v-attack_amd/csrc/i2v_conv_tile.h
@@ -148,33 +148,45 @@
 }
 
 #define I2V_FROW(r) (MF16 ? 4 * lk + (r) : ((r) & 3) + 8 * ((r) >> 2) + 4 * lk)
+template <int BP, int WP, bool MF16, int TP, typename ACC>
+__device__ __forceinline__ void conv_acc_to_rows(ACC (&acc)[TP], float (*const Cs)[BP]) {
+    constexpr int FR = MF16 ? 16 : 32, NR = MF16 ? 4 : 16;
+    const int lane = threadIdx.x & 63, wave = threadIdx.x >> 6;
+    const int wd = wave / WP, wpx = wave % WP;
+    const int l31 = MF16 ? (lane & 15) : (lane & 31), lk = MF16 ? (lane >> 4) : (lane >> 5);
+    __syncthreads();
+#pragma unroll
+    for (int j = 0; j < TP; ++j)
+#pragma unroll
+        for (int r = 0; r < NR; ++r)
+            Cs[wd * FR + I2V_FROW(r)][wpx * (BP / WP) + j * FR + l31] = acc[j][r];
+    __syncthreads();
+}
 template <int BD, int BP, int WD, int WP, bool PREF, bool MF16, bool FUSE, typename ACC, typename PT>
 __device__ __forceinline__ void conv_vec_epilogue(const PT& p, ACC (&acc)[BD / WD / (MF16 ? 16 : 32)][BP / WP / (MF16 ? 16 : 32)], const int cd0,
                                                   const int64_t px0, float* const smem, const float4* const pre0, const unsigned* const pregw,
                                                   float* const mid) {
-    constexpr int FR = MF16 ? 16 : 32, NR = MF16 ? 4 : 16, TD = BD / WD / FR, TP = BP / WP / FR;
-    const int t = threadIdx.x, lane = t & 63, wave = t >> 6;
-    const int wd = wave / WP, wpx = wave % WP;
-    const int l31 = MF16 ? (lane & 15) : (lane & 31), lk = MF16 ? (lane >> 4) : (lane >> 5);
+    constexpr int FR = MF16 ? 16 : 32, TD = BD / WD / FR;
+    const int t = threadIdx.x;
     float (*Cs)[BP] = reinterpret_cast<float (*)[BP]>(smem);
 #pragma unroll
     for (int i = 0; i < TD; ++i) {
-        __syncthreads();
-#pragma unroll
-        for (int j = 0; j < TP; ++j)
-#pragma unroll
-            for (int r = 0; r < NR; ++r)
-                Cs[wd * FR + I2V_FROW(r)][wpx * (BP / WP) + j * FR + l31] = acc[i][j][r];
-        __syncthreads();
+        conv_acc_to_rows<BP, WP, MF16>(acc[i], Cs);
         conv_vec_rows<BD, BP, WD, PREF, MF16, FUSE>(p, i, cd0, px0, Cs, t, pre0, pregw, mid);
     }
 }
 #undef I2V_FROW
 
+__device__ __forceinline__ int conv_xcd_lid(const int bid, const int nwg) {
+    const int q8 = nwg >> 3, r8 = nwg & 7, xcd = bid & 7;
+    return (xcd < r8 ? xcd * (q8 + 1) : r8 * (q8 + 1) + (xcd - r8) * q8) + (bid >> 3);
+}
+
 template <int BD, int BP, int WD, int WP, int MODE, bool PREF, bool PRE = false, bool VID = false, bool MF16 = false, int HWM = 0, int CPB = 1, int FUSE = 0, int BF3 = 0>
-__device__ __forceinline__ void conv_tile(const I2VConvParams& p, const int n_cd_tiles, const int bid, const int nwg, const int64_t px_base,
-                                          float* const smem, I2V_PROBE_T& probe, const int probe_slot, const int prio_arg = I2V_PRIO_LEVELS,
-                                          float* const mid = nullptr) {
+__device__ __forceinline__ void conv_tile_loop(const I2VConvParams& p, const int cd0, const int64_t px0, const int nwg, float* const smem, I2V_PROBE_T& probe,
+                                               const int probe_slot, const int prio_arg,
+                                               typename std::conditional<MF16, f32x4, f32x16>::type (&acc)[BD / WD / (MF16 ? 16 : 32)][BP / WP / (MF16 ? 16 : 32)],
+                                               float4 (&pre0)[PREF ? WD * (MF16 ? 16 : 32) / (1024 / BP) : 1], unsigned (&pregw)[PREF ? WD * (MF16 ? 16 : 32) / (1024 / BP) : 1]) {
 #if defined(__HIP_DEVICE_COMPILE__)
     constexpr int KC = I2V_KC;
     constexpr int FR = MF16 ? 16 : 32;
@@ -196,12 +208,6 @@
 
     const int t = threadIdx.x, lane = t & 63, wave = t >> 6;
     const int wd = wave / WP, wpx = wave % WP;
-
-    const int q8 = nwg >> 3, r8 = nwg & 7, xcd = bid & 7;
-    const int lid = (xcd < r8 ? xcd * (q8 + 1) : r8 * (q8 + 1) + (xcd - r8) * q8) + (bid >> 3);
-    const int cd_tile = lid % n_cd_tiles;
-    const int64_t px0 = px_base + (int64_t)(lid / n_cd_tiles) * BP;
-    const int cd0 = cd_tile * BD;
 
     const int HWg = p.Hg * p.Wg;
     const int64_t P = (int64_t)p.N * HWg;
@@ -311,8 +317,7 @@
 
     constexpr int E_C4 = BP / 4, E_RSTEP = 1024 / BP, E_NQ = WD * FR / E_RSTEP;
     static_assert(!PREF || TD == 1, "PREF needs a single epilogue pass");
-    float4 pre0[PREF ? E_NQ : 1];
-    unsigned pregw[PREF ? E_NQ : 1];
+    static_assert(!PREF || E_NQ == WD * (MF16 ? 16 : 32) / (1024 / BP), "pre0 / pregw (the caller's): one entry per row a lane owns");
     if (PREF) {
         const int e_c4 = t % E_C4, e_rbase = t / E_C4;
         const int64_t e_pp = px0 + (int64_t)e_c4 * 4;
@@ -373,8 +378,6 @@
         out[2] = __builtin_bit_cast(bf8, (u4){q3[0], q3[1], q3[2], q3[3]});
     };
     (void)bf3_split_frag;
-    typedef typename std::conditional<MF16, f32x4, f32x16>::type acc_t;
-    acc_t acc[TD][TP];
 #pragma unroll
     for (int a = 0; a < TD; ++a)
 #pragma unroll
@@ -384,7 +387,6 @@
 
     const int nchunks = p.Kpad / KC;
     const int l31 = MF16 ? (lane & 15) : (lane & 31), lk = MF16 ? (lane >> 4) : (lane >> 5);
-#define I2V_FROW(r) (MF16 ? 4 * lk + (r) : ((r) & 3) + 8 * ((r) >> 2) + 4 * lk)
     constexpr int NL = NAQ + NBQ;
     constexpr int KR = MF16 ? 4 : 2;
     constexpr int KS = KC / KR;
@@ -743,7 +745,32 @@
 #undef I2V_CHUNK_VB
     if (prio_hi > 0) __builtin_amdgcn_s_setprio(0);
     probe.loop_end(probe_slot);
-
+#endif
+}
+
+template <int BD, int BP, int WD, int WP, int MODE, bool PREF, bool PRE = false, bool VID = false, bool MF16 = false, int HWM = 0, int CPB = 1, int FUSE = 0, int BF3 = 0>
+__device__ __forceinline__ void conv_tile(const I2VConvParams& p, const int n_cd_tiles, const int bid, const int nwg, const int64_t px_base,
+                                          float* const smem, I2V_PROBE_T& probe, const int probe_slot, const int prio_arg = I2V_PRIO_LEVELS,
+                                          float* const mid = nullptr) {
+#if defined(__HIP_DEVICE_COMPILE__)
+    constexpr int FR = MF16 ? 16 : 32, NR = MF16 ? 4 : 16, TD = BD / WD / FR, TP = BP / WP / FR;
+    const int lid = conv_xcd_lid(bid, nwg);
+    const int cd_tile = lid % n_cd_tiles;
+    const int64_t px0 = px_base + (int64_t)(lid / n_cd_tiles) * BP;
+    const int cd0 = cd_tile * BD;
+
+    constexpr int E_NQ = WD * FR / (1024 / BP);
+    float4 pre0[PREF ? E_NQ : 1];
+    unsigned pregw[PREF ? E_NQ : 1];
+    typename std::conditional<MF16, f32x4, f32x16>::type acc[TD][TP];
+    conv_tile_loop<BD, BP, WD, WP, MODE, PREF, PRE, VID, MF16, HWM, CPB, FUSE, BF3>(p, cd0, px0, nwg, smem, probe, probe_slot, prio_arg, acc, pre0, pregw);
+
+    const int lane = threadIdx.x & 63, wave = threadIdx.x >> 6;
+    const int wd = wave / WP, wpx = wave % WP;
+    const int l31 = MF16 ? (lane & 15) : (lane & 31), lk = MF16 ? (lane >> 4) : (lane >> 5);
+    const int HWg = p.Hg * p.Wg;
+    const int64_t P = (int64_t)p.N * HWg;
+#define I2V_FROW(r) (MF16 ? 4 * lk + (r) : ((r) & 3) + 8 * ((r) >> 2) + 4 * lk)
     const int HoWo = p.Ho * p.Wo;
     if (p.vec_epilogue) {
         conv_vec_epilogue<BD, BP, WD, WP, PREF, MF16, FUSE != 0>(p, acc, cd0, px0, smem, pre0, pregw, mid);
diff --git a/image-to-video-i2v-attack_amd/csrc/i2v_engine.cpp b/image-to-video-i2v-attack_amd/csrc/i2v_engine.cpp
--- a/image-to-video-i2v-attack_amd/csrc/i2v_engine.cpp
+++ b/image-to-video-i2v-attack_amd/csrc/i2v_engine.cpp
@@ -437,6 +437,18 @@
     return 0;
 }
 
+extern "C" int i2v_net_scpair_info(i2v_handle h, int net, int32_t out[4]) {
+    Net* n = get_net(h, net); if (!n) return 1;
+    if (!n->planned || !out) return fail("i2v_net_scpair_info: net not planned");
+    out[0] = out[1] = out[2] = out[3] = 0;
+    int k = 0;
+    for (const std::vector<Launch>* L : {&n->fwd, &n->bwd}) {
+        for (const Launch& l : *L) { out[k] += l.sc_ok ? 1 : 0; out[2 + k] += (l.sc_ok && l.sc_b[0]) ? 1 : 0; }
+        ++k;
+    }
+    return 0;
+}
+
 extern "C" size_t i2v_net_workspace_bytes(i2v_handle h, int net) {
     Net* n = get_net(h, net); if (!n) return 0;
     return n->arena_floats * sizeof(float) + n->weight_bytes;
diff --git a/image-to-video-i2v-attack_amd/csrc/i2v_kernels.h b/image-to-video-i2v-attack_amd/csrc/i2v_kernels.h
--- a/image-to-video-i2v-attack_amd/csrc/i2v_kernels.h
+++ b/image-to-video-i2v-attack_amd/csrc/i2v_kernels.h
@@ -40,6 +40,18 @@
     return true;
 }
 int k_conv_fused(const I2VConvParams& a, const I2VConvParams& b, int halo, i2v_stream_t s);
+inline bool i2v_conv_scpair_ok(const I2VConvParams& a, const I2VConvParams& b) {
+    for (const I2VConvParams* q : {&a, &b})
+        if (q->temporal || q->quad || q->pre_scale || q->gate_scale || q->blk > 1 || q->blkt > 1 || q->bf3) return false;
+    if (!(a.pointwise || (a.tap_uniform && a.K == a.Cs && a.Kpad == a.K))) return false;
+    if (a.relu || a.mask || a.gate || a.gate_out || a.add0 || a.add1) return false;
+    if (a.osh != 1 || a.osw != 1 || a.oh0 || a.ow0 || a.Hg != a.Ho || a.Wg != a.Wo) return false;
+    if (!b.pointwise || !b.vec_epilogue) return false;
+    if (a.N != b.N || a.Hg != b.Hg || a.Wg != b.Wg || a.Cd != b.Cd || a.Ho != b.Ho || a.Wo != b.Wo) return false;
+    return a.dst && b.add0 == a.dst && b.add0_stride == 1 && b.add0_nstride == a.dst_nstride;
+}
+int k_conv_scpair_ok(const I2VConvParams& a, const I2VConvParams& b);
+int k_conv_scpair(const I2VConvParams& a, const I2VConvParams& b, i2v_stream_t s);
 int k_conv_candidates(const I2VConvParams& p, int* out);
 inline int i2v_fastblock_rows(const I2VConvParams& a, const I2VConvParams& b, const I2VConvParams* c, const I2VConvParams* d) {
     auto plain = [](const I2VConvParams& q) {
diff --git a/image-to-video-i2v-attack_amd/csrc/i2v_kernels.hip b/image-to-video-i2v-attack_amd/csrc/i2v_kernels.hip
--- a/image-to-video-i2v-attack_amd/csrc/i2v_kernels.hip
+++ b/image-to-video-i2v-attack_amd/csrc/i2v_kernels.hip
@@ -25,6 +25,7 @@
     if (!strcmp(name, "se_launches")) return __atomic_load_n(&g_stat_se, __ATOMIC_RELAXED);
     if (!strcmp(name, "convnext_dw_launches")) return __atomic_load_n(&g_stat_cndw, __ATOMIC_RELAXED);
     if (!strcmp(name, "mixer_tokens_launches")) return __atomic_load_n(&g_stat_mixtok, __ATOMIC_RELAXED);
+    if (!strcmp(name, "scpair_launches")) return __atomic_load_n(&g_stat_scpair, __ATOMIC_RELAXED);
 #ifdef I2V_EXPERIMENTAL
     if (!strcmp(name, "experimental")) return 1;
 #else
diff --git a/image-to-video-i2v-attack_amd/csrc/i2v_net.h b/image-to-video-i2v-attack_amd/csrc/i2v_net.h
--- a/image-to-video-i2v-attack_amd/csrc/i2v_net.h
+++ b/image-to-video-i2v-attack_amd/csrc/i2v_net.h
@@ -91,6 +91,9 @@
     int node = -1;
     int fb_ok = 0;
     int fb_b[4] = {0, 0, 0, 0};
+    int sc_ok = 0;
+    int sc_b[4] = {0, 0, 0, 0};
+    bool sc_private = false;
     int ov_after = -2, ov_join = -1;
 };
 inline int cfg_bucket(int clips, int max_clips) {
@@ -169,6 +172,9 @@
 bool fused_fits(const Launch& a, const Launch& b, int frames);
 int fused_run(const Launch& a, const Launch& b, int frames, const float* x, int halo, i2v_stream_t s);
 int fast_run(const std::vector<Launch>& L, size_t li, int frames, const float* x, i2v_stream_t s);
+bool sc_pair_ok(const Launch& a, const Launch& b);
+bool sc_fits(const Launch& a, const Launch& b, int frames);
+int sc_run(const Launch& a, const Launch& b, int frames, i2v_stream_t s);
 extern long long g_overlap_launches;
 
 #pragma GCC visibility pop
diff --git a/image-to-video-i2v-attack_amd/csrc/i2v_run.cpp b/image-to-video-i2v-attack_amd/csrc/i2v_run.cpp
--- a/image-to-video-i2v-attack_amd/csrc/i2v_run.cpp
+++ b/image-to-video-i2v-attack_amd/csrc/i2v_run.cpp
@@ -1,6 +1,9 @@
 #include "i2v_net.h"
 #ifndef I2V_HAVE_SE
 #include "i2v_se_host.h"
+#endif
+#ifndef I2V_HAVE_SCPAIR
+#include "i2v_scpair_host.h"
 #endif
 
 #include <stdio.h>
@@ -46,6 +49,35 @@
     return 0;
 }
 
+static void sc_prep(const Launch& a, const Launch& b, int frames, I2VConvParams* pa, I2VConvParams* pb) {
+    *pa = conv_prep(a, nullptr, nullptr, 0); *pb = conv_prep(b, nullptr, nullptr, 0);
+    for (I2VConvParams* p : {pa, pb}) {
+        p->N = frames;
+        p->src_span_bytes = (int32_t)(((int64_t)frames * p->Ts / p->Tg - 1) * p->src_nstride * 4 + (int64_t)p->Cs * p->Hs * p->Ws * 4);
+    }
+}
+bool sc_pair_ok(const Launch& a, const Launch& b) {
+    if (a.kind != L_CONV || b.kind != L_CONV || a.src_is_input || b.src_is_input || a.T != b.T) return false;
+    I2VConvParams pa, pb;
+    sc_prep(a, b, a.T, &pa, &pb);
+#ifdef I2V_HAVE_SCPAIR
+    return k_conv_scpair_ok(pa, pb) != 0;
+#else
+    return scpair_host::ok(pa, pb) != 0;
+#endif
+}
+bool sc_fits(const Launch& a, const Launch& b, int frames) { return fused_fits(a, b, frames); }
+int sc_run(const Launch& a, const Launch& b, int frames, i2v_stream_t s) {
+    I2VConvParams pa, pb;
+    sc_prep(a, b, frames, &pa, &pb);
+#ifdef I2V_HAVE_SCPAIR
+    CHECK_BE(k_conv_scpair(pa, pb, s));
+#else
+    if (scpair_host::run(pa, pb, s)) return fail("shortcut pair: the two launches do not form a pair");
+#endif
+    return 0;
+}
+
 int fast_run(const std::vector<Launch>& L, size_t li, int frames, const float* x, i2v_stream_t s) {
     const int g = L[li].fb_ok;
     I2VConvParams q[4];
@@ -106,9 +138,10 @@
     return t;
 }
 
-static double launch_flops(const std::vector<Launch>& L, size_t li, int fb, int fuse, int frames, int clips) {
+static double launch_flops(const std::vector<Launch>& L, size_t li, int fb, int fuse, int sc, int frames, int clips) {
     const Launch& l = L[li];
     double flops = 0.0;
+    if (sc >= 0) return 2.0 * frames * l.conv.Hg * l.conv.Wg * ((double)l.conv.Cd * l.conv.K + (double)L[sc].conv.Cd * L[sc].conv.K);
     if (fb) { for (int j = 0; j < fb; ++j) { const Launch& m = L[li + j]; flops += m.alg_flops_per_frame > 0 ? m.alg_flops_per_frame * frames : 2.0 * frames * m.conv.Hg * m.conv.Wg * (double)m.conv.Cd * m.conv.K; } }
     else if ((l.kind == L_CONV || l.kind == L_GCONV || l.kind == L_DWCONV) && l.alg_flops_per_frame > 0) flops = l.alg_flops_per_frame * frames;
     else if (l.kind == L_CONV) flops = 2.0 * frames * l.conv.Hg * l.conv.Wg * ((double)l.conv.Cd * l.conv.K + (fuse ? (double)L[li + 1].conv.Cd * L[li + 1].conv.K : 0.0));
@@ -130,7 +163,7 @@
     return 4;
 }
 
-static double launch_bytes(const std::vector<Launch>& L, size_t li, int fb, int fuse, int frames, int clips, int accumulate) {
+static double launch_bytes(const std::vector<Launch>& L, size_t li, int fb, int fuse, int sc, int frames, int clips, int accumulate) {
     const Launch& l = L[li];
     const I2VConvParams& q = l.conv;
     const double out = (double)frames * q.Hg * q.Wg * q.Cd;
@@ -162,6 +195,10 @@
         if (r.gate) b += out2 / 8.0;
         if (r.gate_out) b += out2 / 8.0;
     }
+    if (sc >= 0) {
+        const I2VConvParams& r = L[sc].conv;
+        b += 4.0 * ((double)clips * r.Ts * r.Cs * r.Hs * r.Ws + (double)r.K * r.Cd) - 4.0 * out;
+    }
     return b;
 }
 
@@ -172,10 +209,10 @@
     TimedLaunch* prev = nullptr;
     TimedLaunch* seg = nullptr;
 
-    TimedLaunch* open(const std::vector<Launch>& L, size_t li, int fb, int fuse, int frames, int clips, int accumulate) {
+    TimedLaunch* open(const std::vector<Launch>& L, size_t li, int fb, int fuse, int sc, int frames, int clips, int accumulate) {
         const Launch& l = L[li];
         const int kind = launch_timing_kind(l, backward_pass);
-        const double flops = launch_flops(L, li, fb, fuse, frames, clips);
+        const double flops = launch_flops(L, li, fb, fuse, sc, frames, clips);
         const bool conv = l.kind == L_CONV || l.kind == L_IMGGRAD || l.kind == L_GCONV || l.kind == L_DWCONV;
         if (h->timing == 2) {
             if (!seg || seg->kind != kind) {
@@ -183,13 +220,13 @@
                 seg = timing_begin(h, kind, 0.0, s, seg);
                 if (seg) seg->count = 0;
             }
-            if (seg) { seg->flops += flops; seg->count += 1; if (conv) seg->bytes += launch_bytes(L, li, fb, fuse, frames, clips, accumulate); else seg->bytes += l.se_bytes_per_frame * frames; }
+            if (seg) { seg->flops += flops; seg->count += 1; if (conv) seg->bytes += launch_bytes(L, li, fb, fuse, sc, frames, clips, accumulate); else seg->bytes += l.se_bytes_per_frame * frames; }
             return prev = nullptr;
         }
         TimedLaunch* const tl = prev = timing_begin(h, kind, flops, s, prev);
         if (tl && conv) {
             tl->Cd = l.conv.Cd; tl->K = l.conv.K; tl->HWg = l.conv.Hg * l.conv.Wg; tl->frames = frames; tl->pw = l.conv.pointwise;
-            tl->bytes = launch_bytes(L, li, fb, fuse, frames, clips, accumulate);
+            tl->bytes = launch_bytes(L, li, fb, fuse, sc, frames, clips, accumulate);
         }
         if (tl && l.kind == L_AGEMM) {
             const I2VAttnGemm& q = l.ag;
@@ -254,21 +291,36 @@
     const bool overlap = !h->timing && n.side && !side.at.empty() && in_frames <= n.ov_max_frames;
     if (overlap) n.ov_used = 0;
     if (overlap && side.issue(-1)) return 1;
+    auto leads_group = [&](size_t k) { return L[k].kind == L_CONV && ((L[k].fuse_ok && L[k].fuse_b[bucket]) || (L[k].fb_ok && L[k].fb_b[bucket])); };
+    int sc_from = -1; size_t sc_at = 0;
     for (size_t li = 0; li < L.size(); ++li) {
         Launch& l = L[li];
         const int frames = clips * l.T;
         const size_t li0 = li;
         if (overlap && l.ov_after != -2) continue;
+        if (l.kind == L_CONV && l.sc_ok && l.sc_b[bucket] && !overlap && sc_from < 0 && li + l.sc_ok < L.size() && frames * l.conv.Hg * l.conv.Wg > 0 &&
+            sc_fits(l, L[li + l.sc_ok], frames)) {
+            bool clear = !leads_group(li);
+            for (size_t k = li + 1; k <= li + l.sc_ok && clear; ++k) clear = !leads_group(k);
+            if (clear) { sc_from = (int)li; sc_at = li + l.sc_ok; continue; }
+        }
+        const int sc = (sc_from >= 0 && li == sc_at) ? sc_from : -1;
+        if (sc >= 0) sc_from = -1;
         const int fuse = (l.kind == L_CONV && l.fuse_ok && li + 1 < L.size() && frames * l.conv.Hg * l.conv.Wg > 0 && fused_fits(l, L[li + 1], frames))
                              ? l.fuse_b[bucket] : 0;
         const int fb = (l.kind == L_CONV && l.fb_ok && li + l.fb_ok <= L.size() && frames * l.conv.Hg * l.conv.Wg > 0) ? l.fb_b[bucket] * l.fb_ok : 0;
         if (overlap && side.join((int)li + (fb ? fb - 1 : fuse ? 1 : 0))) return 1;
-        TimedLaunch* const tl = h->timing ? timing.open(L, li, fb, fuse, frames, clips, accumulate) : nullptr;
+        TimedLaunch* const tl = h->timing ? timing.open(L, li, fb, fuse, sc, frames, clips, accumulate) : nullptr;
         struct Stop { TimedLaunch* t; i2v_stream_t s; ~Stop() { if (t) be_event_record(t->stop, s); } } stop{tl, s};
         switch (l.kind) {
             case L_CONV:
             case L_IMGGRAD: {
                 if (frames * l.conv.Hg * l.conv.Wg == 0) break;
+                if (sc >= 0) {
+                    if (l.cfg_b[bucket]) l.conv.cfg = l.cfg_b[bucket];
+                    if (sc_run(L[sc], l, frames, s)) return 1;
+                    break;
+                }
                 if (fuse) { if (fused_run(l, L[li + 1], frames, x, fuse == 2, s)) return 1; ++li; break; }
                 if (fb) {
                     const int rc = fast_run(L, li, frames, x, s);
@@ -451,6 +503,18 @@
                                 "(plan with I2V_FASTBLOCK=0 to read it)");
             }
         }
+    for (const std::vector<Launch>* L : {&n->fwd, &n->bwd})
+        for (const Launch& l : *L) {
+            if (l.kind != L_CONV || !l.sc_ok || !(l.sc_b[0] | l.sc_b[1] | l.sc_b[2] | l.sc_b[3])) continue;
+            if ((&l)[l.sc_ok].conv.dst == l.conv.dst) continue;
+            const float* lo = l.conv.dst; const float* hi = lo + (int64_t)(n->maxN / n->Tin() * std::max(1, l.conv.To) - 1) * l.conv.dst_nstride + (int64_t)l.conv.Cd * l.conv.Ho * l.conv.Wo;
+            const float* vlo = v.p; const float* vhi = v.p + (int64_t)(frames - 1) * v.nstride + (int64_t)v.C * v.H * v.W;
+            if (!(vlo < hi && lo < vhi)) continue;
+            if (L == &n->bwd || which != 0 || !l.sc_private)
+                return fail("i2v_net_read_tensor: this tensor is the shortcut output of a fused first bottleneck (shortcut pair) and is never stored "
+                            "(plan with I2V_SCPAIR=0 to read it)");
+            if (conv_run(l, frames / std::max(1, v.T) * l.T, nullptr, nullptr, 0, stream)) return 1;
+        }
     size_t row = (size_t)v.C * v.H * v.W * sizeof(float);
     CHECK_BE(be_d2d_2d(out, row, v.p, (size_t)v.nstride * sizeof(float), row, frames, stream));
     return 0;
diff --git a/image-to-video-i2v-attack_amd/csrc/i2v_scpair_host.h b/image-to-video-i2v-attack_amd/csrc/i2v_scpair_host.h
--- /dev/null
+++ b/image-to-video-i2v-attack_amd/csrc/i2v_scpair_host.h
@@ -0,0 +1,22 @@
+#pragma once
+#include <algorithm>
+#include <limits>
+
+#include "i2v_kernels.h"
+
+namespace eng {
+namespace scpair_host {
+
+inline int ok(const I2VConvParams& a, const I2VConvParams& b) { return i2v_conv_scpair_ok(a, b) ? 1 : 0; }
+
+inline int run(const I2VConvParams& a, const I2VConvParams& b, i2v_stream_t s) {
+    if (!i2v_conv_scpair_ok(a, b)) return 1;
+    if (k_conv(a, s) || k_conv(b, s)) return 1;
+    if (b.dst == a.dst) return 0;
+    for (int64_t f = 0; f < (int64_t)a.N; ++f)
+        std::fill(a.dst + f * a.dst_nstride, a.dst + f * a.dst_nstride + (int64_t)a.Cd * a.Ho * a.Wo, std::numeric_limits<float>::quiet_NaN());
+    return 0;
+}
+
+}
+}
diff --git a/image-to-video-i2v-attack_amd/csrc/i2v_tune.cpp b/image-to-video-i2v-attack_amd/csrc/i2v_tune.cpp
--- a/image-to-video-i2v-attack_amd/csrc/i2v_tune.cpp
+++ b/image-to-video-i2v-attack_amd/csrc/i2v_tune.cpp
@@ -145,6 +145,49 @@
                 for (size_t i = 0; i < L->size(); ++i)
                     if ((*L)[i].fb_ok) fprintf(stderr, "[i2v fastblock] %s launch %zu: group of %d (Cs %d -> %d mid channels, %dx%d)\n", L == &n.fwd ? "fwd" : "bwd", i, (*L)[i].fb_ok,
                                                (*L)[i].conv.Cs, (*L)[i].conv.Cd, (*L)[i].conv.Hg, (*L)[i].conv.Wg);
+    }
+    {
+        const bool sc_off = [] { const char* e = getenv("I2V_SCPAIR"); return e && e[0] == '0'; }();
+        for (std::vector<Launch>* L : {&n.fwd, &n.bwd}) {
+            for (Launch& l : *L) { l.sc_ok = 0; l.sc_private = false; for (int bk = 0; bk < 4; ++bk) l.sc_b[bk] = 0; }
+            for (size_t i = 0; !sc_off && i + 1 < L->size(); ++i) {
+                Launch& a = (*L)[i];
+                if (a.kind != L_CONV || a.src_is_input || a.conv.add0 || a.conv.relu) continue;
+                for (size_t j = i + 1; j < L->size() && j <= i + 3; ++j) {
+                    const Launch& b = (*L)[j];
+                    if (b.kind != L_CONV || b.conv.add0 != a.conv.dst) continue;
+                    if (!sc_pair_ok(a, b)) break;
+                    const Range w = dst_of(a);
+                    auto conv_kind = [](const Launch& c) { return c.kind == L_CONV || c.kind == L_IMGGRAD || c.kind == L_GCONV || c.kind == L_DWCONV; };
+                    auto reads = [&](const Launch& c) { return touches(c, w, false, conv_kind(c)); };
+                    auto covers = [&](const Launch& c) { return conv_kind(c) && c.conv.dst && dst_of(c).first <= w.first && dst_of(c).second >= w.second; };
+                    Launch b_rest = b; b_rest.conv.add0 = nullptr;
+                    bool other = reads(b_rest), dead = covers(b);
+                    for (size_t k = i + 1; k < j && !other; ++k) other |= touches((*L)[k], w, false, false);
+                    for (size_t k = j + 1; k < L->size() && !other && !dead; ++k) {
+                        if (reads((*L)[k])) other = true;
+                        else if (covers((*L)[k])) dead = true;
+                        else other = touches((*L)[k], w, false, false);
+                    }
+                    if (!dead) {
+                        for (auto& hk : hooked) other |= meet(hk, w);
+                        for (const Launch& c : (L == &n.fwd ? n.bwd : n.fwd)) other = other || touches(c, w, false, false);
+                    }
+                    bool dep = false;
+                    for (size_t k = i + 1; k < j && !dep; ++k) {
+                        const Launch& m = (*L)[k];
+                        const I2VConvParams& pa = a.conv; const I2VConvParams& pm = m.conv;
+                        dep = (m.kind != L_CONV && m.kind != L_GCONV && m.kind != L_DWCONV) || m.src_is_input || touches(a, dst_of(m), false, false) ||
+                              (pm.gate_out && (pm.gate_out == pa.gate || pm.gate_out == pa.gate_out)) || (pa.gate_out && (pa.gate_out == pm.gate || pa.gate_out == pm.gate_out));
+                    }
+                    if (!other && !dep) { a.sc_ok = (int)(j - i); a.sc_private = !dead; for (int bk = 0; bk < 4; ++bk) a.sc_b[bk] = 1; }
+                    if (getenv("I2V_FUSE_DEBUG"))
+                        fprintf(stderr, "[i2v scpair] %s launches %zu + %zu (K %d + %d -> Cd %d, %dx%d): other_reader=%d dependent=%d\n", L == &n.fwd ? "fwd" : "bwd", i, j,
+                                a.conv.K, b.conv.K, b.conv.Cd, b.conv.Hg, b.conv.Wg, (int)other, (int)dep);
+                    break;
+                }
+            }
+        }
     }
     const char* force = getenv("I2V_FORCE_FUSE");
     const int f = force ? atoi(force) : 0;
@@ -396,6 +439,33 @@
     return 0;
 }
 
+int tune_scpairs(Net& n, Probe& pr, int max_clips) {
+    for (std::vector<Launch>* L : {&n.fwd, &n.bwd})
+        for (size_t i = 0; i < L->size(); ++i) {
+            Launch& a = (*L)[i];
+            if (!a.sc_ok || i + a.sc_ok >= L->size()) continue;
+            Launch& b = (*L)[i + a.sc_ok];
+            const int rc = for_each_bucket(max_clips, a.conv.Tg, [&](int bk, int lf) -> int {
+                if (lf * a.conv.Hg * a.conv.Wg == 0 || !sc_fits(a, b, lf)) return 0;
+                const int ca = a.conv.cfg, cb = b.conv.cfg;
+                if (a.cfg_b[bk]) a.conv.cfg = a.cfg_b[bk];
+                if (b.cfg_b[bk]) b.conv.cfg = b.cfg_b[bk];
+                float t_sep = 0.f, t_pair = 0.f;
+                const int rc = pr.time([&] { return conv_run(a, lf, pr.x, pr.gx, 0, nullptr) || conv_run(b, lf, pr.x, pr.gx, 0, nullptr); }, 3, &t_sep) ||
+                               pr.time([&] { return sc_run(a, b, lf, nullptr); }, 3, &t_pair);
+                a.conv.cfg = ca; b.conv.cfg = cb;
+                if (rc) return 1;
+                a.sc_b[bk] = t_pair < t_sep ? 1 : 0;
+                if (getenv("I2V_FUSE_DEBUG"))
+                    fprintf(stderr, "[i2v scpair] %s launches %zu + %zu (K %d + %d -> Cd %d, %dx%d) at %d frames: separate %.1f us, pair %.1f us -> %s\n", list_name(n, L), i,
+                            i + a.sc_ok, a.conv.K, b.conv.K, b.conv.Cd, b.conv.Hg, b.conv.Wg, lf, 1e3f * t_sep, 1e3f * t_pair, a.sc_b[bk] ? "pair" : "separate");
+                return 0;
+            });
+            if (rc) return 1;
+        }
+    return 0;
+}
+
 }
 
 int autotune(Net& n) {
@@ -409,6 +479,7 @@
         const bool on_device = strncmp(be_name(), "hip", 3) == 0;
         rc = tune_tiles(n, pr, max_clips);
         if (!rc && on_device) rc = tune_fastblocks(n, pr, max_clips);
+        if (!rc && on_device) rc = tune_scpairs(n, pr, max_clips);
         static const bool fuse_on = [] { const char* e = getenv("I2V_FUSE"); return e && e[0] == '1'; }();
         if (!rc && fuse_on && on_device) rc = tune_pairs(n, pr, max_clips);
     }
diff --git a/image-to-video-i2v-attack_amd/i2v_amd/engine.py b/image-to-video-i2v-attack_amd/i2v_amd/engine.py
--- a/image-to-video-i2v-attack_amd/i2v_amd/engine.py
+++ b/image-to-video-i2v-attack_amd/i2v_amd/engine.py
@@ -418,6 +418,11 @@
         _lib.check(self.eng.capi, self.eng.capi.i2v_net_fusion_info(self.eng.h, self.id, out))
         return tuple(int(v) for v in out)
 
+    def scpair_info(self):
+        out = (C.c_int32 * 4)()
+        _lib.check(self.eng.capi, self.eng.capi.i2v_net_scpair_info(self.eng.h, self.id, out))
+        return tuple(int(v) for v in out)
+
     def forward(self, x: torch.Tensor):
         _lib.check(self.eng.capi, self.eng.capi.i2v_net_forward(self.eng.h, self.id, _ptr(x, self.eng), x.shape[0], self.eng.stream()))
 
diff --git a/image-to-video-i2v-attack_amd/i2v_amd/lib.py b/image-to-video-i2v-attack_amd/i2v_amd/lib.py
--- a/image-to-video-i2v-attack_amd/i2v_amd/lib.py
+++ b/image-to-video-i2v-attack_amd/i2v_amd/lib.py
@@ -66,6 +66,7 @@
     "i2v_net_plan": ([_P, _I, C.POINTER(_I), _I, _I], _I),
     "i2v_net_workspace_bytes": ([_P, _I], C.c_size_t),
     "i2v_net_fusion_info": ([_P, _I, _P], _I),
+    "i2v_net_scpair_info": ([_P, _I, _P], _I),
     "i2v_net_forward": ([_P, _I, _P, _I, _P], _I),
     "i2v_net_hook_info": ([_P, _I, _I, C.POINTER(_P), C.POINTER(_L), C.POINTER(_P), C.POINTER(_L),
                            C.POINTER(_L), C.POINTER(C.c_int32)], _I),
diff --git a/include/i2v_hip.h b/include/i2v_hip.h
--- a/include/i2v_hip.h
+++ b/include/i2v_hip.h
@@ -73,6 +73,7 @@
 int i2v_net_plan(i2v_handle h, int net, const int* hook_tensors, int n_hooks, int max_frames);
 size_t i2v_net_workspace_bytes(i2v_handle h, int net);
 int i2v_net_fusion_info(i2v_handle h, int net, int32_t out[4]);
+int i2v_net_scpair_info(i2v_handle h, int net, int32_t out[4]);
 
 int i2v_net_forward(i2v_handle h, int net, const float* x, int frames, void* stream);
 int i2v_net_hook_info(i2v_handle h, int net, int hook, float** act, int64_t* act_stride,
```

Result: faster. 757.8 (median of 6 runs) (+1.4%).
